# AppleHolic/pytorch_sound

Hardware: AMD Instinct MI355X
Metric: audio-sec/s STFT+mel+fwd/bwd (higher is better)
Workload: dtype bf16; 1 GPU; configs[1]: Conv1d separator (4 x ResBlock1, C=256, on 513-bin magnitude), 22.05 kHz, STFT 1024/256, 80 mel, batch 32 x 2 s per GPU, Adam, bf16 autocast; global_batch=32, parallelism=dp1, model_params=5520386

## Files before the change

### include/psnd.h

```cpp
#ifndef PSND_H
#define PSND_H

#include <stdint.h>
#include <stddef.h>

#ifdef __cplusplus
extern "C" {
#endif

#define PSND_OK 0
#define PSND_E_ARG (-1)
#define PSND_E_SHAPE (-2)
#define PSND_E_HIP (-3)
#define PSND_E_UNSUPPORTED (-4)

#define PSND_FRAMING_CENTER 0
#define PSND_FRAMING_HIFIGAN 1
#define PSND_FRAMING_NONE 2

int psnd_version(void);
const char *psnd_last_error(void);
#ifdef PSND_LAB
void psnd_env_refresh(void);
#endif

void *psnd_event_create(void);
int psnd_event_destroy(void *ev);
int psnd_event_record_external(void *ev, void *stream);
int psnd_stream_wait_event(void *stream, void *ev);
int psnd_event_external_supported(void);

int64_t psnd_frame_count(int64_t T, int n_fft, int hop, int framing);
int64_t psnd_frame_sample_index(int64_t f, int m, int64_t T, int n_fft, int hop, int framing);

size_t psnd_stft_plan_bytes(int n_fft);
int psnd_stft_plan_build(int n_fft, const float *window_host, void *plan_host);

int psnd_stft_fwd(const float *wav, int64_t N, int64_t T, int n_fft, int hop, int framing,
                  const void *plan, float mag_eps,
                  float *mag, float *phase, float *re, float *im, void *stream);

int psnd_stft_mag_nfk(const float *wav, int64_t N, int64_t T, int n_fft, int hop, int framing,
                      const void *plan, float mag_eps, float *mag_nfk, void *stream);

int psnd_stft_bwd(const float *wav, int64_t N, int64_t T, int n_fft, int hop, int framing,
                  const void *plan, float mag_eps,
                  const float *gmag, const float *gre, const float *gim,
                  float *gwav, void *stream);

int psnd_polar_bwd(const float *gmag, const float *gphase, const float *mag, const float *phase, int64_t n,
                   float *gre, float *gim, void *stream);

int psnd_istft(const float *mag, const float *phase, int64_t N, int64_t F, int n_fft, int hop,
               const void *plan, float eps, float *out, void *stream);

size_t psnd_stft_mr_plan_bytes(int n_fft);
int psnd_stft_mr_plan_build(int n_fft, const float *window_host, void *plan_host);
int psnd_stft_mr_fwd(const float *wav, int64_t N, int64_t T, int n_fft, int hop, int framing, const void *plan, size_t plan_bytes,
                     float mag_eps, float *mag, float *phase, float *re, float *im, void *stream);
size_t psnd_stft_mr_bwd_scratch_bytes(int64_t N, int64_t T, int n_fft, int hop, int framing);
int psnd_stft_mr_bwd(const float *wav, int64_t N, int64_t T, int n_fft, int hop, int framing, const void *plan, size_t plan_bytes,
                     float mag_eps, const float *gmag, const float *gre, const float *gim, void *scratch, size_t scratch_bytes,
                     float *gwav, void *stream);
size_t psnd_istft_mr_scratch_bytes(int64_t N, int64_t F, int n_fft);
int psnd_istft_mr(const float *mag, const float *phase, int64_t N, int64_t F, int n_fft, int hop, const void *plan, size_t plan_bytes,
                  float eps, void *scratch, size_t scratch_bytes, float *out, void *stream);

#define PSND_LOG_NONE 0
#define PSND_LOG_E 1
#define PSND_LOG_10 2
size_t psnd_mel_plan_bytes(int M, int K);
int psnd_mel_plan_build(int M, int K, const float *mel_filter_host, void *plan_host);
int psnd_mel_fwd(const float *mag, int64_t N, int64_t F, int M, int K, const void *mel_plan,
                 int log_kind, float log_offset, float pre_clamp_min, float clamp_lo, float clamp_hi,
                 float *out, float *mel_lin, void *stream);
int psnd_mel_bwd(const float *gout, const float *mel_lin, int64_t N, int64_t F, int M, int K,
                 const void *mel_plan, int log_kind, float log_offset, float pre_clamp_min,
                 float clamp_lo, float clamp_hi, float *gmag, void *stream);

int psnd_logmel_fwd(const float *wav, int64_t N, int64_t T, int n_fft, int hop, int framing, const void *stft_plan,
                    float mag_eps, int M, const void *mel_plan, int log_kind, float log_offset, float pre_clamp_min,
                    float clamp_lo, float clamp_hi, float *out, void *stream);

int psnd_conv1d_cl(const void *A, const void *A2, const void *AM, float a2_slope, const void *W, const float *bias,
                   const void *res, const void *mask_src, int64_t N, int Lp, int L, int HP, int Ca, int Cb, int k,
                   int off0, int dstep, float act_slope, float mask_slope, void *out_raw, void *out_act,
                   void *a_eff_out, void *stream);
int psnd_conv1d_cl_wgrad_splits(int64_t N, int Lp, int Ca, int Cb, int k);
int psnd_conv1d_cl_pair_supported(int C, int k, int off1, int dstep1, int off2, int dstep2);
int psnd_conv1d_cl_pair(const void *A, const void *W1, const float *bias1, const void *M1, float m1_slope, float act1_slope,
                        void *mid_out, const void *W2, const float *bias2, const void *M2, float m2_slope, const void *res,
                        int64_t N, int Lp, int L, int HP, int C, int k, int off1, int dstep1, int off2, int dstep2,
                        float act2_slope, void *out_raw, void *out_act, void *stream);
typedef struct psnd_wgrad_desc {
    const void *g, *xa;
    float *gw_part, *gbias_part;
    int off0, dstep;
    int Ca, Cb, k, splits;
} psnd_wgrad_desc;
int psnd_conv1d_cl_wgrad_multi_splits(int64_t N, int Lp, int Ca, int Cb, int k, int n_convs);
int psnd_conv1d_cl_wgrad_multi(const psnd_wgrad_desc *d, int n, int64_t N, int Lp, void *stream);
typedef struct psnd_chain_pair {
    const void *W1;
    const float *bias1;
    float act1_slope;
    void *mid_out;
    const void *W2;
    const float *bias2;
    int off1, dstep1, off2, dstep2;
    float act2_slope;
    void *out_raw, *out_act;
    const void *M1, *M2;
    float m1_slope, m2_slope;
} psnd_chain_pair;
int psnd_conv1d_cl_chain_rows(int C, int k, int n_pairs, const int *taps);
int psnd_conv1d_cl_chain_plan(int C, int k, int n_pairs, const int *taps, int64_t R, int *mr_out);
int psnd_conv1d_cl_chain(const void *A, const void *res, const psnd_chain_pair *pairs, int n_pairs, int64_t N, int Lp, int L, int HP,
                         int C, int k, void *stream);
void psnd_conv_chain_stats(long long *out2);
int psnd_to_cl_nfk(const float *x_nfk, int64_t N, int K, int64_t F, int Lp, int HP, int Cp, int preop, void *out, void *stream);
int64_t psnd_mask_head_l1_blocks_nfk(int64_t N, int64_t F, int K);
int psnd_mask_head_l1_fwd_nfk(const void *y, const float *mag_nfk, const float *ref_nfk, int64_t N, int K, int64_t F, int Lp, int HP, int Cp,
                              float *est_nfk, double *part, void *stream);
int psnd_mask_head_l1_bwd_nfk(const float *gest_nfk, const float *mag_nfk, const void *y, const float *est_nfk, const float *ref_nfk,
                              const float *g, float coef, int64_t N, int K, int64_t F, int Lp, int HP, int Cp, void *gy, void *stream);
int psnd_mel_fwd_nfk(const float *mag_nfk, int64_t N, int64_t F, int M, int K, const void *mel_plan, int log_kind, float log_offset,
                     float pre_clamp_min, float clamp_lo, float clamp_hi, float *out, float *mel_lin, void *stream);
int psnd_mel_bwd_nfk(const float *gout, const float *mel_lin, int64_t N, int64_t F, int M, int K, const void *mel_plan, int log_kind,
                     float log_offset, float pre_clamp_min, float clamp_lo, float clamp_hi, float *gmag_nfk, void *stream);
int psnd_mel_l1_fwd_nfk(const float *mag_nfk, int64_t N, int64_t F, int M, int K, const void *mel_plan, int log_kind, float log_offset,
                        float pre_clamp_min, float clamp_lo, float clamp_hi, const float *ref, float *mel_lin, double *part, void *stream);
int psnd_mel_l1_bwd_nfk(const float *ref, const float *mel_lin, const float *g, float coef, int64_t N, int64_t F, int M, int K,
                        const void *mel_plan, int log_kind, float log_offset, float pre_clamp_min, float clamp_lo, float clamp_hi,
                        float *gmag_nfk, void *stream);
int64_t psnd_mask_head_l1_blocks(int64_t N, int64_t T, int Cp);
int psnd_mask_head_l1_fwd(const void *y, const float *mag, const float *ref, int64_t N, int C, int64_t T, int Lp, int HP, int Cp,
                          float *est, double *part, void *stream);
int psnd_mask_head_l1_bwd(const float *gest, const float *mag, const void *y, const float *est, const float *ref, const float *g,
                          float coef, int64_t N, int C, int64_t T, int Lp, int HP, int Cp, void *gy, void *stream);
int64_t psnd_mel_l1_blocks(int64_t N, int64_t F, int M);
int psnd_mel_l1_fwd(const float *mag, int64_t N, int64_t F, int M, int K, const void *mel_plan, int log_kind, float log_offset,
                    float pre_clamp_min, float clamp_lo, float clamp_hi, const float *ref, float *mel_lin, double *part, void *stream);
int psnd_mel_l1_bwd(const float *ref, const float *mel_lin, const float *g, float coef, int64_t N, int64_t F, int M, int K,
                    const void *mel_plan, int log_kind, float log_offset, float pre_clamp_min, float clamp_lo, float clamp_hi,
                    float *gmag, void *stream);
int psnd_nan_flag(const float *x, int64_t n, float *flag, void *stream);
int psnd_l1_loss_combine(const double *const *parts, const int64_t *nb, const double *scale, int terms, float *out, float *nan_flag, void *stream);
int psnd_conv_stats(int64_t *out4, int reset);
int psnd_conv_pair_stats(int64_t *out4, int reset);
int psnd_conv1d_cl_wgrad(const void *G1, const void *G2, const void *GM, float g2_slope, const void *xa, int64_t N,
                         int Lp, int Ca, int Cb, int k, int off0, int dstep, float *gw_part, float *gbias_part,
                         void *g_out, void *stream);
int psnd_conv1d_prep(const float *v, const float *g, const float *bias, int Cout, int Cin, int k, int Cb, int Ca,
                     void *wf, void *wb, float *bias_padded, void *stream);
int psnd_convtr1d_prep(const float *v, const float *g, const float *bias, int Cin, int Cout, int K, int stride, int Cr, int Cip,
                       void *wf, void *wb, float *bias_rep, void *stream);
int psnd_convtr1d_prep_multi(const void *descs_dev, int n, int total_blocks, void *stream);
int psnd_convtr1d_cl_fwd(const void *xa, const void *wf, const float *bias_rep, int64_t N, int Lp, int L, int HP, int Cip, int Cr,
                         int stride, int padding, int LpO, int HPO, float act_slope, void *out_raw, void *out_act, void *stream);
int psnd_convtr1d_cl_wgrad_splits(int64_t N, int Lp, int Cip, int Cr, int stride);
int psnd_convtr1d_cl_bwd(const void *g_raw, const void *g_act, const void *act, float act_slope, const void *wb, const void *xa,
                         int64_t N, int Lp, int L, int HP, int Cip, int Cr, int stride, int padding, int LpO, int HPO, void *gx,
                         void *g_eff, float *gw_part, void *stream);
int psnd_convtr1d_wnorm_bwd(const float *gw_part, int splits, const float *v, const float *g, int Cin, int Cout, int K, int stride,
                            int Cr, int Cip, float *gv, float *gg, void *stream);
int psnd_cl_mean_act_fwd(const void *a, const void *b, const void *c, const void *d, int count, float slope, void *out, int64_t n,
                         void *stream);
int psnd_cl_mean_act_bwd(const void *g, const void *y, int count, float slope, void *gin, int64_t n, void *stream);
int psnd_cl_sum2(const void *const *a, int na, void *out_a, const void *const *b, int nb, void *out_b, int64_t n, void *stream);
int psnd_cl_colsum_splits(int64_t rows, int C);
int psnd_cl_colsum(const void *g, int64_t rows, int C, int Lp, int lo, int hi, float *part, float *out, void *stream);
int psnd_conv1d_prep_multi(const void *descs_dev, int n, int total_blocks, int max_row, int which, void *stream);
#define PSND_WNORM_MAX 32
typedef struct psnd_wnorm_desc {
    const float *gw_part, *gbias_part;
    const float *v, *g;
    float *gv, *gg, *gbias;
    int splits, Cout, Cin, k, Cb, Ca;
} psnd_wnorm_desc;
int psnd_conv1d_wnorm_bwd_multi(const psnd_wnorm_desc *descs, int n, void *stream);
int psnd_conv1d_cl_bwd(const void *G1, const void *G2, const void *GM, float g2_slope, const void *wb, const void *xa,
                       int64_t N, int Lp, int L, int HP, int Ca, int Cb, int k, int pad, int dil, void *gx, void *g_out,
                       const void *gx_mask, float gx_mask_slope, const void *gx_res, float *gw_part, float *gbias_part,
                       void *stream);
int psnd_conv1d_cl_pair_bwd_supported(int C, int k, int pad2, int dil2, int pad1, int dil1);
int psnd_conv1d_cl_pair_bwd_splits(int64_t N, int Lp, int C, int k);
int psnd_conv1d_cl_pair_bwd(const void *G, const void *wb2, const void *M1, float m1_slope, void *g_mid, const void *wb1, const void *M2,
                            float m2_slope, const void *res, int64_t N, int Lp, int L, int HP, int C, int k, int pad2, int dil2,
                            int pad1, int dil1, void *gx, const void *xa_a, float *gw_a, float *gb_a, const void *G_b,
                            const void *xa_b, int off_b, int dstep_b, float *gw_b, float *gb_b, void *stream);
int psnd_conv1d_wnorm_bwd(const float *gw_part, const float *gbias_part, int splits, const float *v, const float *g,
                          int Cout, int Cin, int k, int Cb, int Ca, float *gv, float *gg, float *gbias, void *stream);
int psnd_to_cl(const float *x, int64_t N, int C, int64_t T, int Lp, int HP, int Cp, int preop, void *out, void *stream);
int psnd_from_cl_tanh(const void *x, int64_t N, int C, int64_t T, int Lp, int HP, int Cp, float *out, void *stream);
int psnd_to_cl_tanh_bwd(const float *g, const float *out_fwd, int64_t N, int C, int64_t T, int Lp, int HP, int Cp, void *gx, void *stream);
int psnd_from_cl(const void *x, int64_t N, int C, int64_t T, int Lp, int HP, int Cp, float *out, void *stream);
int psnd_mask_head_fwd(const void *y, const float *mag, int64_t N, int C, int64_t T, int Lp, int HP, int Cp, float *est,
                       void *stream);
int psnd_mask_head_bwd(const float *gest, const float *mag, const void *y, int64_t N, int C, int64_t T, int Lp, int HP, int Cp,
                       void *gy, void *stream);

int psnd_linear1x1_fwd(const float *x, const float *w, const float *bias, int64_t N, int Cin, int Cout, int64_t T, int relu, int bf16,
                       float *y, void *stream);
int64_t psnd_linear1x1_wgrad_slabs(int64_t N, int Cin, int Cout, int64_t T);
int psnd_linear1x1_bwd(const float *gy, const float *ymask, const float *x, const float *w, int64_t N, int Cin, int Cout, int64_t T,
                       int bf16, float *gx, float *gw, float *gw_part, float *gbias, void *stream);
int psnd_linear1x1_bwd_acc(const float *gy, const float *ymask, const float *x, const float *w, int64_t N, int Cin, int Cout, int64_t T,
                           int bf16, const float *gx_addend, float *gx, float *gw, float *gw_part, float *gbias, void *stream);
int psnd_linear1x1_bwd_ex(const void *gy, const float *ymask, const void *x, const float *w, int64_t N, int Cin, int Cout, int64_t T, int bf16,
                          int io_h, int64_t ld_h, const float *gx_addend, const void *gx_mask, void *gx, float *gw, float *gw_part, float *gbias,
                          void *stream);
int psnd_linear1x1_fwd_ex(const void *x, const float *w, const float *bias, int64_t N, int Cin, int Cout, int64_t T, int relu, int bf16, int io_h,
                          int64_t ld_h, void *y, void *stream);
int psnd_mha_fwd(const float *kvq, const unsigned char *mask, int64_t N, int H, int C, int64_t T, float *out, float *att, float *stats,
                 int bf16, void *stream);
int psnd_mha_bwd(const float *kvq, const unsigned char *mask, const float *out, const float *att, const float *stats, const float *gout,
                 const float *gatt, int64_t N, int H, int C, int64_t T, float *delta, float *gkvq, int bf16, void *stream);
int psnd_mha_bwd_parts(const float *kvq, const unsigned char *mask, const float *out, const float *att, const float *stats, const float *gout,
                       const float *gatt, int64_t N, int H, int C, int64_t T, float *delta, float *gkvq, int bf16, int parts, void *stream);

#define PSND_GN_WS_DOUBLES(C) (2 * (size_t)(C))
int psnd_posenc(const float *x, const float *pe, float scale, int64_t N, int C, int64_t T, int64_t pe_len, float *y, void *stream);
int psnd_groupnorm1_fwd(const float *x, const float *res, const float *gamma, const float *beta, int64_t N, int C,
                        int64_t T, float eps, int relu, float *y, float *stats, double *ws, void *stream);
int psnd_groupnorm1_bwd(const float *gy, const float *x, const float *res, const float *gamma, const float *y,
                        const float *stats, int64_t N, int C, int64_t T, int relu, float *gx, float *ggamma,
                        float *gbeta, double *ws, void *stream);
int psnd_groupnorm1_drop_fwd(const float *x, const float *res, const float *gamma, const float *beta, int64_t N, int C,
                             int64_t T, float eps, int relu, float *y, float *stats, double *ws, const uint64_t *key,
                             uint32_t thr, float scale, void *stream);
int psnd_groupnorm1_drop_bwd(const float *gy, const float *x, const float *res, const float *gamma, const float *y,
                             const float *stats, int64_t N, int C, int64_t T, int relu, float *gx, float *gres, float *ggamma,
                             float *gbeta, double *ws, const uint64_t *key, uint32_t thr, float scale, void *stream);
int psnd_rng_seed(uint64_t *state, uint64_t seed, uint64_t call, void *stream);
int psnd_rng_next(uint64_t *state, uint64_t *key_out, void *stream);
int psnd_softmax_keys_fwd(float *scores, const uint8_t *mask, int64_t B, int64_t T, float scale, void *stream);
int psnd_softmax_keys_bwd(const float *att, const float *gatt, int64_t B, int64_t T, float scale, float *gscores,
                          void *stream);

int psnd_preemphasis_fwd(const float *x, int64_t N, int64_t T, float coef, float *y, void *stream);
int psnd_preemphasis_bwd(const float *gy, int64_t N, int64_t T, float coef, float *gx, void *stream);
int64_t psnd_stft_loss_blocks(int64_t KF);
int psnd_stft_loss_partial(const float *p_mag, const float *t_mag, int64_t N, int64_t KF, float eps, double *part,
                           void *stream);
int psnd_stft_loss_final(const double *const *parts, const int64_t *KF, int L, int64_t N, float *norms, float *out3,
                         void *stream);
int psnd_stft_loss_bwd(const float *p_mag, const float *t_mag, int64_t N, int64_t KF, float eps, const float *norms,
                       const float *g3, int L, float *gp, float *gt, void *stream);
int64_t psnd_stft_fwd_msl_blocks(int64_t T, int n_fft, int hop);
int psnd_stft_fwd_msl(const float *wav, int64_t N, int64_t T, int n_fft, int hop, const void *plan, float mag_eps,
                      const float *t_mag, float eps, double *part, void *stream);
int psnd_stft_loss_final_blocks(const double *const *parts, const int64_t *KF, const int64_t *blocks, int L, int64_t N,
                                float *norms, float *out3, void *stream);
int psnd_stft_bwd_msl_supported(int n_fft, int hop);
int psnd_stft_bwd_msl(const float *wav, int64_t N, int64_t T, int n_fft, int hop, int framing, const void *plan,
                      float mag_eps, const float *t_mag, const float *norms, const float *g3, int L, float eps,
                      int accumulate, float *gwav, void *stream);

#define PSND_IPREEMPH_SPAN 8192
#define PSND_IPREEMPH_WARM_MAX 2048
#define PSND_IPREEMPH_SEQ (-1)
#define PSND_IPREEMPH_AUTO (-2)
int psnd_ipreemph_fwd(const float *x, int64_t N, int64_t T, const float *w_ih, const float *w_hh, int warm, float *y,
                      void *stream);
int psnd_ipreemph_bwd(const float *gy, const float *y, const float *x, int64_t N, int64_t T, const float *w_ih,
                      const float *w_hh, int warm, float *gx, double *partial, float *gw, void *stream);
int psnd_volnorm_fwd(const float *wav, int64_t B, int64_t L, int window, int hop, float inv_gain, float *out,
                     int64_t out_len, float *std, void *stream);
int psnd_volnorm_reverse(const float *wav, int64_t B, int64_t L, int window, int hop, float gain, const float *std,
                         float *out, int64_t out_len, void *stream);

int psnd_im2col_f32(const float *x, int64_t N, int C, int64_t T, int k, int dil, int pad, int stride, int up, int64_t To, float slope,
                    float *col, void *stream);
int psnd_col2im_f32(const float *gcol, const float *x, int64_t N, int C, int64_t T, int k, int dil, int pad, int stride, int up, int64_t To,
                    float slope, float *gx, void *stream);

int psnd_pad_collate(const float *flat, const int64_t *offs, const int64_t *lens, int64_t N, int64_t Tmax, float *out,
                     float *mask, void *stream);

int64_t psnd_frame_mask_frames(int64_t T, int win, int hop);
int psnd_frame_mask(const float *mask, int64_t N, int64_t T, int win, int hop, float *out, void *stream);

int psnd_grad_pack_bf16(const float *src, void *dst, int64_t n, float scale, void *stream);
int psnd_grad_unpack_bf16(const void *src, float *dst, int64_t n, float scale, void *stream);
int64_t psnd_adam_chunk(void);
int64_t psnd_adam_table_bytes(void);
int psnd_adam_step(const void *table, int n_tensors, const int *chunk_tensor, const int64_t *chunk_off, int64_t n_chunks,
                   double lr, double beta1, double beta2, double eps, double weight_decay, int decoupled,
                   const float *found_inf, const float *grad_scale, float *corr, float clip_value, const float *clip_coef,
                   void *stream);
int psnd_adam_step_logged(const void *table, int n_tensors, const int *chunk_tensor, const int64_t *chunk_off, int64_t n_chunks,
                          double lr, double beta1, double beta2, double eps, double weight_decay, int decoupled,
                          const float *found_inf, const float *grad_scale, float *corr, float clip_value, const float *clip_coef,
                          int *flag_log, int log_slot, int log_seq, void *stream);
int psnd_grad_sumsq(const void *table, int n_tensors, const int *chunk_tensor, const int64_t *chunk_off, int64_t n_chunks,
                    float clip_value, const float *grad_scale, int accumulate, float max_norm, double *partial, double *sumsq,
                    float *coef, void *stream);

int psnd_pqmf_analysis(const float *x, const float *filt, int64_t B, int64_t T, int subbands, int taps, int flip, float scale,
                       float *out, void *stream);
int psnd_pqmf_synthesis(const float *x, const float *filt, int64_t B, int64_t M, int64_t T_out, int subbands, int taps, int flip,
                        float scale, float *y, void *stream);

int psnd_lstft_analysis(const float *x, const float *basis, const float *window, int64_t N, int64_t Lx, int C, int n, int hop, float *spec,
                        float *mag, float *phase, void *stream);
int psnd_lstft_mag_bwd(const float *spec, const float *mag, const float *gmag, int64_t N, int C, int64_t F, float *gspec, void *stream);
int psnd_lstft_synthesis(const float *g, const float *basis, const float *window, const float *mult, int64_t N, int C, int64_t F, int n,
                         int hop, int64_t Ly, float *y, void *stream);
int64_t psnd_lstft_wgrad_slabs(int64_t N, int C, int n, int64_t F);
int psnd_lstft_basis_grad(const float *g, const float *x, const float *window, int64_t N, int64_t Lx, int C, int n, int hop, int64_t F,
                          float *gb_part, float *gb, void *stream);

int64_t psnd_l1_loss_blocks(int64_t n);
int64_t psnd_masked_l1_blocks(int64_t n);
int psnd_masked_l1_fwd(const float *a, const float *b, const float *frame_weight, int64_t N, int C, int64_t T, double *part, float *out,
                       float *inv_den, void *stream);
int psnd_masked_l1_bwd(const float *a, const float *b, const float *frame_weight, int64_t N, int C, int64_t T, const float *g,
                       const float *inv_den, float *ga, float *gb, void *stream);
int psnd_l1_loss_fwd(const float *a, const float *b, int64_t n, double *part, float *out, void *stream);
int psnd_l1_loss_bwd(const float *a, const float *b, int64_t n, const float *g, float *ga, float *gb, void *stream);
int psnd_l1_loss_sum_fwd(const float *const *a, const float *const *b, const int64_t *n, const double *w, int terms, double *part,
                         float *out, void *stream);
int psnd_l1_loss_bwd_w(const float *a, const float *b, int64_t n, const float *g, double weight, float *ga, float *gb, void *stream);

#ifdef __cplusplus
// ... 4 lines not shown
```

### pytorch_sound_amd/_lib.py

```python
import ctypes
import os
import numpy as np

_HERE = os.path.dirname(os.path.abspath(__file__))
LIB_PATH = os.environ.get('PSND_LIB', os.path.join(_HERE, 'libpsnd_hip.so'))

PSND_OK = 0
FRAMING_CENTER = 0
FRAMING_HIFIGAN = 1
FRAMING_NONE = 2
LOG_NONE, LOG_E, LOG_10 = 0, 1, 2

_c = ctypes
_P = _c.c_void_p
_I64 = _c.c_int64
_INT = _c.c_int
_F = _c.c_float
_D = _c.c_double
_U32 = _c.c_uint32
_U64 = _c.c_uint64

SIGNATURES = {
    'psnd_version': (_INT, []),
    'psnd_last_error': (_c.c_char_p, []),
    'psnd_event_create': (_P, []),
    'psnd_event_destroy': (_INT, [_P]),
    'psnd_event_record_external': (_INT, [_P, _P]),
    'psnd_stream_wait_event': (_INT, [_P, _P]),
    'psnd_event_external_supported': (_INT, []),
    'psnd_frame_count': (_I64, [_I64, _INT, _INT, _INT]),
    'psnd_frame_sample_index': (_I64, [_I64, _INT, _I64, _INT, _INT, _INT]),
    'psnd_stft_plan_bytes': (_c.c_size_t, [_INT]),
    'psnd_stft_plan_build': (_INT, [_INT, _P, _P]),
    'psnd_stft_fwd': (_INT, [_P, _I64, _I64, _INT, _INT, _INT, _P, _F, _P, _P, _P, _P, _P]),
    'psnd_stft_mag_nfk': (_INT, [_P, _I64, _I64, _INT, _INT, _INT, _P, _F, _P, _P]),
    'psnd_stft_bwd': (_INT, [_P, _I64, _I64, _INT, _INT, _INT, _P, _F, _P, _P, _P, _P, _P]),
    'psnd_istft': (_INT, [_P, _P, _I64, _I64, _INT, _INT, _P, _F, _P, _P]),
    'psnd_stft_mr_plan_bytes': (_c.c_size_t, [_INT]),
    'psnd_stft_mr_plan_build': (_INT, [_INT, _P, _P]),
    'psnd_stft_mr_fwd': (_INT, [_P, _I64, _I64, _INT, _INT, _INT, _P, _c.c_size_t, _F, _P, _P, _P, _P, _P]),
    'psnd_stft_mr_bwd_scratch_bytes': (_c.c_size_t, [_I64, _I64, _INT, _INT, _INT]),
    'psnd_stft_mr_bwd': (_INT, [_P, _I64, _I64, _INT, _INT, _INT, _P, _c.c_size_t, _F, _P, _P, _P, _P, _c.c_size_t, _P, _P]),
    'psnd_istft_mr_scratch_bytes': (_c.c_size_t, [_I64, _I64, _INT]),
    'psnd_istft_mr': (_INT, [_P, _P, _I64, _I64, _INT, _INT, _P, _c.c_size_t, _F, _P, _c.c_size_t, _P, _P]),
    'psnd_mel_plan_bytes': (_c.c_size_t, [_INT, _INT]),
    'psnd_mel_plan_build': (_INT, [_INT, _INT, _P, _P]),
    'psnd_mel_fwd': (_INT, [_P, _I64, _I64, _INT, _INT, _P, _INT, _F, _F, _F, _F, _P, _P, _P]),
    'psnd_mel_bwd': (_INT, [_P, _P, _I64, _I64, _INT, _INT, _P, _INT, _F, _F, _F, _F, _P, _P]),
    'psnd_logmel_fwd': (_INT, [_P, _I64, _I64, _INT, _INT, _INT, _P, _F, _INT, _P, _INT, _F, _F, _F, _F, _P, _P]),
    'psnd_conv1d_cl': (_INT, [_P, _P, _P, _F, _P, _P, _P, _P, _I64, _INT, _INT, _INT, _INT, _INT, _INT, _INT, _INT, _F, _F, _P, _P, _P, _P]),
    'psnd_conv1d_cl_pair_supported': (_INT, [_INT, _INT, _INT, _INT, _INT, _INT]),
    'psnd_conv1d_cl_pair': (_INT, [_P, _P, _P, _P, _F, _F, _P, _P, _P, _P, _F, _P, _I64, _INT, _INT, _INT, _INT, _INT, _INT, _INT, _INT, _INT, _F, _P, _P, _P]),
    'psnd_conv1d_cl_wgrad': (_INT, [_P, _P, _P, _F, _P, _I64, _INT, _INT, _INT, _INT, _INT, _INT, _P, _P, _P, _P]),
    'psnd_conv1d_prep': (_INT, [_P, _P, _P, _INT, _INT, _INT, _INT, _INT, _P, _P, _P, _P]),
    'psnd_conv1d_wnorm_bwd': (_INT, [_P, _P, _INT, _P, _P, _INT, _INT, _INT, _INT, _INT, _P, _P, _P, _P]),
    'psnd_conv1d_cl_bwd': (_INT, [_P, _P, _P, _F, _P, _P, _I64, _INT, _INT, _INT, _INT, _INT, _INT, _INT, _INT, _P, _P, _P, _F, _P, _P, _P, _P]),
    'psnd_conv1d_cl_wgrad_multi_splits': (_INT, [_I64, _INT, _INT, _INT, _INT, _INT]),
    'psnd_conv1d_cl_wgrad_multi': (_INT, [_P, _INT, _I64, _INT, _P]),
    'psnd_nan_flag': (_INT, [_P, _I64, _P, _P]),
    'psnd_conv1d_cl_chain_rows': (_INT, [_INT, _INT, _INT, _P]),
    'psnd_conv1d_cl_chain_plan': (_INT, [_INT, _INT, _INT, _P, _I64, _P]),
    'psnd_conv1d_cl_chain': (_INT, [_P, _P, _P, _INT, _I64, _INT, _INT, _INT, _INT, _INT, _P]),
    'psnd_conv_chain_stats': (None, [_P]),
    'psnd_conv1d_cl_pair_bwd_supported': (_INT, [_INT, _INT, _INT, _INT, _INT, _INT]),
    'psnd_conv1d_cl_pair_bwd_splits': (_INT, [_I64, _INT, _INT, _INT]),
    'psnd_conv1d_cl_pair_bwd': (_INT, [_P, _P, _P, _F, _P, _P, _P, _F, _P, _I64, _INT, _INT, _INT, _INT, _INT, _INT, _INT, _INT, _INT, _P, _P, _P, _P,
                                       _P, _P, _INT, _INT, _P, _P, _P]),
    'psnd_conv1d_wnorm_bwd_multi': (_INT, [_P, _INT, _P]),
    'psnd_conv1d_prep_multi': (_INT, [_P, _INT, _INT, _INT, _INT, _P]),
    'psnd_conv1d_cl_wgrad_splits': (_INT, [_I64, _INT, _INT, _INT, _INT]),
    'psnd_mask_head_l1_blocks': (_I64, [_I64, _I64, _INT]),
    'psnd_masked_l1_blocks': (_I64, [_I64]),
    'psnd_masked_l1_fwd': (_INT, [_P, _P, _P, _I64, _INT, _I64, _P, _P, _P, _P]),
    'psnd_masked_l1_bwd': (_INT, [_P, _P, _P, _I64, _INT, _I64, _P, _P, _P, _P, _P]),
    'psnd_to_cl_nfk': (_INT, [_P, _I64, _INT, _I64, _INT, _INT, _INT, _INT, _P, _P]),
    'psnd_mask_head_l1_blocks_nfk': (_I64, [_I64, _I64, _INT]),
    'psnd_mask_head_l1_fwd_nfk': (_INT, [_P, _P, _P, _I64, _INT, _I64, _INT, _INT, _INT, _P, _P, _P]),
    'psnd_mask_head_l1_bwd_nfk': (_INT, [_P, _P, _P, _P, _P, _P, _F, _I64, _INT, _I64, _INT, _INT, _INT, _P, _P]),
    'psnd_mel_fwd_nfk': (_INT, [_P, _I64, _I64, _INT, _INT, _P, _INT, _F, _F, _F, _F, _P, _P, _P]),
    'psnd_mel_bwd_nfk': (_INT, [_P, _P, _I64, _I64, _INT, _INT, _P, _INT, _F, _F, _F, _F, _P, _P]),
    'psnd_mel_l1_fwd_nfk': (_INT, [_P, _I64, _I64, _INT, _INT, _P, _INT, _F, _F, _F, _F, _P, _P, _P, _P]),
    'psnd_mel_l1_bwd_nfk': (_INT, [_P, _P, _P, _F, _I64, _I64, _INT, _INT, _P, _INT, _F, _F, _F, _F, _P, _P]),
    'psnd_mask_head_l1_fwd': (_INT, [_P, _P, _P, _I64, _INT, _I64, _INT, _INT, _INT, _P, _P, _P]),
    'psnd_mask_head_l1_bwd': (_INT, [_P, _P, _P, _P, _P, _P, _F, _I64, _INT, _I64, _INT, _INT, _INT, _P, _P]),
    'psnd_mel_l1_blocks': (_I64, [_I64, _I64, _INT]),
    'psnd_mel_l1_fwd': (_INT, [_P, _I64, _I64, _INT, _INT, _P, _INT, _F, _F, _F, _F, _P, _P, _P, _P]),
    'psnd_mel_l1_bwd': (_INT, [_P, _P, _P, _F, _I64, _I64, _INT, _INT, _P, _INT, _F, _F, _F, _F, _P, _P]),
    'psnd_l1_loss_combine': (_INT, [_P, _P, _P, _INT, _P, _P, _P]),
    'psnd_conv_stats': (_INT, [_P, _INT]),
    'psnd_conv_pair_stats': (_INT, [_P, _INT]),
    'psnd_convtr1d_prep_multi': (_INT, [_P, _INT, _INT, _P]),
    'psnd_convtr1d_prep': (_INT, [_P, _P, _P, _INT, _INT, _INT, _INT, _INT, _INT, _P, _P, _P, _P]),
    'psnd_convtr1d_cl_fwd': (_INT, [_P, _P, _P, _I64, _INT, _INT, _INT, _INT, _INT, _INT, _INT, _INT, _INT, _F, _P, _P, _P]),
    'psnd_convtr1d_cl_wgrad_splits': (_INT, [_I64, _INT, _INT, _INT, _INT]),
    'psnd_convtr1d_cl_bwd': (_INT, [_P, _P, _P, _F, _P, _P, _I64, _INT, _INT, _INT, _INT, _INT, _INT, _INT, _INT, _INT, _P, _P, _P, _P]),
    'psnd_convtr1d_wnorm_bwd': (_INT, [_P, _INT, _P, _P, _INT, _INT, _INT, _INT, _INT, _INT, _P, _P, _P]),
    'psnd_cl_mean_act_fwd': (_INT, [_P, _P, _P, _P, _INT, _F, _P, _I64, _P]),
    'psnd_cl_mean_act_bwd': (_INT, [_P, _P, _INT, _F, _P, _I64, _P]),
    'psnd_cl_sum2': (_INT, [_P, _INT, _P, _P, _INT, _P, _I64, _P]),
    'psnd_grad_pack_bf16': (_INT, [_P, _P, _I64, _F, _P]),
    'psnd_grad_unpack_bf16': (_INT, [_P, _P, _I64, _F, _P]),
    'psnd_cl_colsum_splits': (_INT, [_I64, _INT]),
    'psnd_cl_colsum': (_INT, [_P, _I64, _INT, _INT, _INT, _INT, _P, _P, _P]),
    'psnd_posenc': (_INT, [_P, _P, _F, _I64, _INT, _I64, _I64, _P, _P]),
    'psnd_groupnorm1_fwd': (_INT, [_P, _P, _P, _P, _I64, _INT, _I64, _F, _INT, _P, _P, _P, _P]),
    'psnd_groupnorm1_bwd': (_INT, [_P, _P, _P, _P, _P, _P, _I64, _INT, _I64, _INT, _P, _P, _P, _P, _P]),
    'psnd_groupnorm1_drop_fwd': (_INT, [_P, _P, _P, _P, _I64, _INT, _I64, _F, _INT, _P, _P, _P, _P, _U32, _F, _P]),
    'psnd_groupnorm1_drop_bwd': (_INT, [_P, _P, _P, _P, _P, _P, _I64, _INT, _I64, _INT, _P, _P, _P, _P, _P, _P, _U32, _F, _P]),
    'psnd_rng_seed': (_INT, [_P, _U64, _U64, _P]),
    'psnd_rng_next': (_INT, [_P, _P, _P]),
    'psnd_linear1x1_fwd': (_INT, [_P, _P, _P, _I64, _INT, _INT, _I64, _INT, _INT, _P, _P]),
    'psnd_linear1x1_wgrad_slabs': (_I64, [_I64, _INT, _INT, _I64]),
    'psnd_linear1x1_bwd': (_INT, [_P, _P, _P, _P, _I64, _INT, _INT, _I64, _INT, _P, _P, _P, _P, _P]),
    'psnd_linear1x1_bwd_acc': (_INT, [_P, _P, _P, _P, _I64, _INT, _INT, _I64, _INT, _P, _P, _P, _P, _P, _P]),
    'psnd_linear1x1_bwd_ex': (_INT, [_P, _P, _P, _P, _I64, _INT, _INT, _I64, _INT, _INT, _I64, _P, _P, _P, _P, _P, _P, _P]),
    'psnd_linear1x1_fwd_ex': (_INT, [_P, _P, _P, _I64, _INT, _INT, _I64, _INT, _INT, _INT, _I64, _P, _P]),
    'psnd_mha_fwd': (_INT, [_P, _P, _I64, _INT, _INT, _I64, _P, _P, _P, _INT, _P]),
    'psnd_mha_bwd': (_INT, [_P, _P, _P, _P, _P, _P, _P, _I64, _INT, _INT, _I64, _P, _P, _INT, _P]),
    'psnd_mha_bwd_parts': (_INT, [_P, _P, _P, _P, _P, _P, _P, _I64, _INT, _INT, _I64, _P, _P, _INT, _INT, _P]),
    'psnd_softmax_keys_fwd': (_INT, [_P, _P, _I64, _I64, _F, _P]),
    'psnd_softmax_keys_bwd': (_INT, [_P, _P, _I64, _I64, _F, _P, _P]),
    'psnd_polar_bwd': (_INT, [_P, _P, _P, _P, _I64, _P, _P, _P]),
    'psnd_preemphasis_fwd': (_INT, [_P, _I64, _I64, _F, _P, _P]),
    'psnd_preemphasis_bwd': (_INT, [_P, _I64, _I64, _F, _P, _P]),
    'psnd_ipreemph_fwd': (_INT, [_P, _I64, _I64, _P, _P, _INT, _P, _P]),
    'psnd_ipreemph_bwd': (_INT, [_P, _P, _P, _I64, _I64, _P, _P, _INT, _P, _P, _P, _P]),
    'psnd_volnorm_fwd': (_INT, [_P, _I64, _I64, _INT, _INT, _F, _P, _I64, _P, _P]),
    'psnd_volnorm_reverse': (_INT, [_P, _I64, _I64, _INT, _INT, _F, _P, _P, _I64, _P]),
    'psnd_stft_loss_blocks': (_I64, [_I64]),
    'psnd_stft_loss_partial': (_INT, [_P, _P, _I64, _I64, _F, _P, _P]),
    'psnd_stft_loss_final': (_INT, [_P, _P, _INT, _I64, _P, _P, _P]),
    'psnd_stft_loss_bwd': (_INT, [_P, _P, _I64, _I64, _F, _P, _P, _INT, _P, _P, _P]),
    'psnd_stft_bwd_msl_supported': (_INT, [_INT, _INT]),
    'psnd_stft_fwd_msl_blocks': (_I64, [_I64, _INT, _INT]),
    'psnd_stft_fwd_msl': (_INT, [_P, _I64, _I64, _INT, _INT, _P, _F, _P, _F, _P, _P]),
    'psnd_stft_loss_final_blocks': (_INT, [_P, _P, _P, _INT, _I64, _P, _P, _P]),
    'psnd_stft_bwd_msl': (_INT, [_P, _I64, _I64, _INT, _INT, _INT, _P, _F, _P, _P, _P, _INT, _F, _INT, _P, _P]),
    'psnd_frame_mask_frames': (_I64, [_I64, _INT, _INT]),
    'psnd_frame_mask': (_INT, [_P, _I64, _I64, _INT, _INT, _P, _P]),
    'psnd_pad_collate': (_INT, [_P, _P, _P, _I64, _I64, _P, _P, _P]),
    'psnd_im2col_f32': (_INT, [_P, _I64, _INT, _I64, _INT, _INT, _INT, _INT, _INT, _I64, _F, _P, _P]),
    'psnd_col2im_f32': (_INT, [_P, _P, _I64, _INT, _I64, _INT, _INT, _INT, _INT, _INT, _I64, _F, _P, _P]),
    'psnd_adam_chunk': (_I64, []),
    'psnd_adam_table_bytes': (_I64, []),
    'psnd_adam_step': (_INT, [_P, _INT, _P, _P, _I64, _D, _D, _D, _D, _D, _INT, _P, _P, _P, _F, _P, _P]),
    'psnd_adam_step_logged': (_INT, [_P, _INT, _P, _P, _I64, _D, _D, _D, _D, _D, _INT, _P, _P, _P, _F, _P, _P, _INT, _INT, _P]),
    'psnd_grad_sumsq': (_INT, [_P, _INT, _P, _P, _I64, _F, _P, _INT, _F, _P, _P, _P, _P]),
    'psnd_mask_head_fwd': (_INT, [_P, _P, _I64, _INT, _I64, _INT, _INT, _INT, _P, _P]),
    'psnd_mask_head_bwd': (_INT, [_P, _P, _P, _I64, _INT, _I64, _INT, _INT, _INT, _P, _P]),
    'psnd_pqmf_analysis': (_INT, [_P, _P, _I64, _I64, _INT, _INT, _INT, _F, _P, _P]),
    'psnd_pqmf_synthesis': (_INT, [_P, _P, _I64, _I64, _I64, _INT, _INT, _INT, _F, _P, _P]),
    'psnd_lstft_analysis': (_INT, [_P, _P, _P, _I64, _I64, _INT, _INT, _INT, _P, _P, _P, _P]),
    'psnd_lstft_mag_bwd': (_INT, [_P, _P, _P, _I64, _INT, _I64, _P, _P]),
    'psnd_lstft_synthesis': (_INT, [_P, _P, _P, _P, _I64, _INT, _I64, _INT, _INT, _I64, _P, _P]),
    'psnd_lstft_wgrad_slabs': (_I64, [_I64, _INT, _INT, _I64]),
    'psnd_lstft_basis_grad': (_INT, [_P, _P, _P, _I64, _I64, _INT, _INT, _INT, _I64, _P, _P, _P]),
    'psnd_l1_loss_blocks': (_I64, [_I64]),
    'psnd_l1_loss_fwd': (_INT, [_P, _P, _I64, _P, _P, _P]),
    'psnd_l1_loss_bwd': (_INT, [_P, _P, _I64, _P, _P, _P, _P]),
    'psnd_l1_loss_sum_fwd': (_INT, [_P, _P, _P, _P, _INT, _P, _P, _P]),
    'psnd_l1_loss_bwd_w': (_INT, [_P, _P, _I64, _P, _D, _P, _P, _P]),
    'psnd_to_cl': (_INT, [_P, _I64, _INT, _I64, _INT, _INT, _INT, _INT, _P, _P]),
    'psnd_from_cl': (_INT, [_P, _I64, _INT, _I64, _INT, _INT, _INT, _P, _P]),
    'psnd_from_cl_tanh': (_INT, [_P, _I64, _INT, _I64, _INT, _INT, _INT, _P, _P]),
    'psnd_to_cl_tanh_bwd': (_INT, [_P, _P, _I64, _INT, _I64, _INT, _INT, _INT, _P, _P]),
}

_lib = None


class PsndError(RuntimeError):
    pass


class WgradDesc(ctypes.Structure):
    _fields_ = [('g', _P), ('xa', _P), ('gw_part', _P), ('gbias_part', _P), ('off0', _INT), ('dstep', _INT),
                ('Ca', _INT), ('Cb', _INT), ('k', _INT), ('splits', _INT)]


class ChainPair(ctypes.Structure):
    _fields_ = [('W1', _P), ('bias1', _P), ('act1_slope', _F), ('mid_out', _P), ('W2', _P), ('bias2', _P),
                ('off1', _INT), ('dstep1', _INT), ('off2', _INT), ('dstep2', _INT), ('act2_slope', _F), ('out_raw', _P), ('out_act', _P),
                ('M1', _P), ('M2', _P), ('m1_slope', _F), ('m2_slope', _F)]


def lib():
    global _lib
    if _lib is None:
        import torch
        if not os.path.exists(LIB_PATH):
            raise PsndError('libpsnd_hip.so not found at %s - run `python -m pytorch_sound_amd._build` '
                            '(there is no CPU / eager fallback)' % LIB_PATH)
        _lib = _load(LIB_PATH)
    return _lib


def _load(path):
    h = ctypes.CDLL(path)
    for name, (res, args) in SIGNATURES.items():
        fn = getattr(h, name)
        fn.restype = res
        fn.argtypes = args
    for name, (res, args) in LAB_SIGNATURES.items():
        fn = getattr(h, name, None)
        if fn is not None:
            fn.restype = res
            fn.argtypes = args
    return h


LAB_LIB_PATH = os.path.join(_HERE, 'libpsnd_hip_lab.so')
LAB_SIGNATURES = {'psnd_env_refresh': (None, [])}


def is_lab() -> bool:
    return hasattr(lib(), 'psnd_env_refresh')


def refresh_switches():
    if _lib is not None and hasattr(_lib, 'psnd_env_refresh'):
        _lib.psnd_env_refresh()

# ... 84 lines not shown
```

### pytorch_sound_amd/cl.py

```python
import ctypes
import os
from pytorch_sound_amd import _switches as _sw
import weakref

import torch

from . import _lib
from ._lib import lib, check, ptr, stream_ptr

ALIGN_C = 32


def round_up(x, m):
    return (x + m - 1) // m * m


class CLShape:

    def __init__(self, N, L, HP):
        self.N, self.L, self.HP = int(N), int(L), int(HP)
        self.Lp = round_up(self.L + 2 * self.HP, 8)

    @property
    def R(self):
# ... 33 lines not shown
        return gx, None, None


def from_cl_raw(buf, C, T, shape):
    _need(buf, torch.bfloat16)
    N, Lp, Cp = buf.shape
    out = torch.empty((N, C, T), dtype=torch.float32, device=buf.device)
    with torch.cuda.device(buf.device):
        check(lib().psnd_from_cl(ptr(buf), N, C, T, Lp, shape.HP, Cp, ptr(out), stream_ptr(buf.device)), 'psnd_from_cl')
    return out


class FromCL(torch.autograd.Function):
    @staticmethod
    def forward(ctx, buf, C, T, shape):
        ctx.shape, ctx.Cp = shape, buf.shape[2]
        return from_cl_raw(buf.contiguous(), C, T, shape)

    @staticmethod
    def backward(ctx, g):
        g = g.contiguous()
        N, C, T = g.shape
        out = torch.empty((N, ctx.shape.Lp, ctx.Cp), dtype=torch.bfloat16, device=g.device)
        with torch.cuda.device(g.device):
            check(lib().psnd_to_cl(ptr(g), N, C, T, ctx.shape.Lp, ctx.shape.HP, ctx.Cp, 0, ptr(out), stream_ptr(g.device)),
                  'psnd_to_cl')
        return out, None, None, None


class FromCLTanh(torch.autograd.Function):

    @staticmethod
    def forward(ctx, buf, C, T, shape):
        buf = buf.contiguous()
        _need(buf, torch.bfloat16)
        N, Lp, Cp = buf.shape
        out = torch.empty((N, C, T), dtype=torch.float32, device=buf.device)
        with torch.cuda.device(buf.device):
            check(lib().psnd_from_cl_tanh(ptr(buf), N, C, T, Lp, shape.HP, Cp, ptr(out), stream_ptr(buf.device)), 'psnd_from_cl_tanh')
        ctx.shape, ctx.Cp = shape, Cp
        ctx.save_for_backward(out)
        return out

    @staticmethod
    def backward(ctx, g):
        (out,) = ctx.saved_tensors
        g = g.contiguous().float()
        N, C, T = g.shape
        gx = torch.empty((N, ctx.shape.Lp, ctx.Cp), dtype=torch.bfloat16, device=g.device)
        with torch.cuda.device(g.device):
            check(lib().psnd_to_cl_tanh_bwd(ptr(g), ptr(out), N, C, T, ctx.shape.Lp, ctx.shape.HP, ctx.Cp, ptr(gx), stream_ptr(g.device)),
                  'psnd_to_cl_tanh_bwd')
        return gx, None, None, None


class MaskHeadCL(torch.autograd.Function):

    @staticmethod
    def forward(ctx, y, mag, shape):
        _need(y, torch.bfloat16)
        _need(mag, torch.float32)
        y, mag = y.contiguous(), mag.contiguous()
        N, C, T = mag.shape
        est = torch.empty_like(mag)
        with torch.cuda.device(y.device):
            check(lib().psnd_mask_head_fwd(ptr(y), ptr(mag), N, C, T, shape.Lp, shape.HP, y.shape[2], ptr(est), stream_ptr(y.device)),
                  'psnd_mask_head_fwd')
        ctx.shape = shape
        ctx.save_for_backward(y, mag)
        return est

    @staticmethod
    def backward(ctx, g):
        y, mag = ctx.saved_tensors
        g = g.contiguous().float()
        N, C, T = mag.shape
        gy = torch.empty_like(y)
        with torch.cuda.device(y.device):
            check(lib().psnd_mask_head_bwd(ptr(g), ptr(mag), ptr(y), N, C, T, ctx.shape.Lp, ctx.shape.HP, y.shape[2], ptr(gy),
                                           stream_ptr(y.device)), 'psnd_mask_head_bwd')
        return gy, None, None


LAST_LOSS_NAN_FLAG = [None]
NAN_FLAG_DEST = [None]


def _nan_flag_tensor(dev):
    dest = NAN_FLAG_DEST[0]
    if dest is not None and dest.device == dev and dest.dtype == torch.float32 and dest.numel() == 1:
        return dest.view(())
    return torch.empty((), dtype=torch.float32, device=dev)


class MaskHeadSpectralL1CL(torch.autograd.Function):

    @staticmethod
    def forward(ctx, y, mag, mag_ref, mel_ref, mel_plan, shape, M, log_kind, log_offset, pre_clamp_min, clamp_lo, clamp_hi, w1, w2):
        import ctypes
        from .kernels import _clamp_args
        ctx.set_materialize_grads(False)
        _need(y, torch.bfloat16)
        for t in (mag, mag_ref, mel_ref):
            _need(t, torch.float32)
        N, C, T = mag.shape
        if mag_ref.shape != mag.shape or tuple(mel_ref.shape) != (N, M, T):
            raise _lib.PsndError('mask_head_spectral_l1: mag_ref %s / mel_ref %s do not match mag %s and %d mel bands'
                                 % (tuple(mag_ref.shape), tuple(mel_ref.shape), tuple(mag.shape), M))
        dev = y.device
        lo, hi, pre = _clamp_args(clamp_lo, clamp_hi, pre_clamp_min)
        est = torch.empty_like(mag)
        lin = torch.empty((N, M, T), dtype=torch.float32, device=dev)
        nb1 = int(lib().psnd_mask_head_l1_blocks(N, T, y.shape[2]))
        nb2 = int(lib().psnd_mel_l1_blocks(N, T, M))
        part = torch.empty(nb1 + nb2, dtype=torch.float64, device=dev)
        out = torch.empty((), dtype=torch.float32, device=dev)
        st = stream_ptr(dev)
        with torch.cuda.device(dev):
            check(lib().psnd_mask_head_l1_fwd(ptr(y), ptr(mag), ptr(mag_ref), N, C, T, shape.Lp, shape.HP, y.shape[2], ptr(est),
                                              ptr(part), st), 'psnd_mask_head_l1_fwd')
            p2 = ctypes.c_void_p(part.data_ptr() + 8 * nb1)
            check(lib().psnd_mel_l1_fwd(ptr(est), N, T, M, C, ptr(mel_plan), log_kind, float(log_offset), pre, lo, hi, ptr(mel_ref),
                                        ptr(lin), p2, st), 'psnd_mel_l1_fwd')
            parts = (ctypes.c_void_p * 2)(part.data_ptr(), part.data_ptr() + 8 * nb1)
            nbs = (ctypes.c_int64 * 2)(nb1, nb2)
            sc = (ctypes.c_double * 2)(float(w1) / mag.numel(), float(w2) / mel_ref.numel())
            nan_flag = _nan_flag_tensor(dev)
            check(lib().psnd_l1_loss_combine(parts, nbs, sc, 2, ptr(out), ptr(nan_flag), st), 'psnd_l1_loss_combine')
        LAST_LOSS_NAN_FLAG[0] = nan_flag
        ctx.cfg = (shape, M, log_kind, float(log_offset), pre, lo, hi, float(w1) / mag.numel(), float(w2) / mel_ref.numel())
        ctx.save_for_backward(y, mag, mag_ref, mel_ref, mel_plan, est, lin)
        ctx.mark_non_differentiable(est)
        return out, est

    @staticmethod
    def backward(ctx, g, _gest):
        y, mag, mag_ref, mel_ref, mel_plan, est, lin = ctx.saved_tensors
        shape, M, log_kind, log_offset, pre, lo, hi, c1, c2 = ctx.cfg
        N, C, T = mag.shape
        if g is None:
            return (None,) * 14
        g = g.contiguous().float()
        gest = torch.empty_like(mag)
        gy = torch.empty_like(y)
        st = stream_ptr(y.device)
        with torch.cuda.device(y.device):
            check(lib().psnd_mel_l1_bwd(ptr(mel_ref), ptr(lin), ptr(g), c2, N, T, M, C, ptr(mel_plan), log_kind, log_offset, pre, lo, hi,
                                        ptr(gest), st), 'psnd_mel_l1_bwd')
            check(lib().psnd_mask_head_l1_bwd(ptr(gest), ptr(mag), ptr(y), ptr(est), ptr(mag_ref), ptr(g), c1, N, C, T, shape.Lp, shape.HP,
                                              y.shape[2], ptr(gy), st), 'psnd_mask_head_l1_bwd')
        return (gy,) + (None,) * 13


def to_cl_nfk(x_nfk, shape, preop=0):
    _need(x_nfk, torch.float32)
    if x_nfk.requires_grad and torch.is_grad_enabled():
        raise _lib.PsndError('to_cl_nfk carries no gradient (feature tensors are inputs); use ToCL on an (N, K, F) tensor')
    N, F, K = x_nfk.shape
    if F != shape.L or N != shape.N:
        raise _lib.PsndError('to_cl_nfk: tensor %s does not match the CL geometry (N=%d, L=%d)' % (tuple(x_nfk.shape), shape.N, shape.L))
    Cp = round_up(K, ALIGN_C)
    out = torch.empty((N, shape.Lp, Cp), dtype=torch.bfloat16, device=x_nfk.device)
    with torch.cuda.device(x_nfk.device):
        check(lib().psnd_to_cl_nfk(ptr(x_nfk), N, K, F, shape.Lp, shape.HP, Cp, int(preop), ptr(out), stream_ptr(x_nfk.device)),
              'psnd_to_cl_nfk')
    return out


class MaskHeadSpectralL1NFK(torch.autograd.Function):

    @staticmethod
    def forward(ctx, y, mag, mag_ref, mel_ref, mel_plan, shape, M, log_kind, log_offset, pre_clamp_min, clamp_lo, clamp_hi, w1, w2):
        from .kernels import _clamp_args
        ctx.set_materialize_grads(False)
        _need(y, torch.bfloat16)
        for t in (mag, mag_ref, mel_ref):
            _need(t, torch.float32)
        N, F, K = mag.shape
        if mag_ref.shape != mag.shape or tuple(mel_ref.shape) != (N, M, F):
            raise _lib.PsndError('mask_head_spectral_l1 (nfk): mag_ref %s / mel_ref %s do not match mag %s and %d mel bands'
                                 % (tuple(mag_ref.shape), tuple(mel_ref.shape), tuple(mag.shape), M))
        dev = y.device
        lo, hi, pre = _clamp_args(clamp_lo, clamp_hi, pre_clamp_min)
        est = torch.empty_like(mag)
        lin = torch.empty((N, M, F), dtype=torch.float32, device=dev)
        nb1 = int(lib().psnd_mask_head_l1_blocks_nfk(N, F, K))
        nb2 = int(lib().psnd_mel_l1_blocks(N, F, M))
        part = torch.empty(nb1 + nb2, dtype=torch.float64, device=dev)
        out = torch.empty((), dtype=torch.float32, device=dev)
        st = stream_ptr(dev)
        with torch.cuda.device(dev):
            check(lib().psnd_mask_head_l1_fwd_nfk(ptr(y), ptr(mag), ptr(mag_ref), N, K, F, shape.Lp, shape.HP, y.shape[2], ptr(est),
                                                  ptr(part), st), 'psnd_mask_head_l1_fwd_nfk')
            p2 = ctypes.c_void_p(part.data_ptr() + 8 * nb1)
            check(lib().psnd_mel_l1_fwd_nfk(ptr(est), N, F, M, K, ptr(mel_plan), log_kind, float(log_offset), pre, lo, hi, ptr(mel_ref),
                                            ptr(lin), p2, st), 'psnd_mel_l1_fwd_nfk')
            parts = (ctypes.c_void_p * 2)(part.data_ptr(), part.data_ptr() + 8 * nb1)
            nbs = (ctypes.c_int64 * 2)(nb1, nb2)
            sc = (ctypes.c_double * 2)(float(w1) / mag.numel(), float(w2) / mel_ref.numel())
            nan_flag = _nan_flag_tensor(dev)
            check(lib().psnd_l1_loss_combine(parts, nbs, sc, 2, ptr(out), ptr(nan_flag), st), 'psnd_l1_loss_combine')
        LAST_LOSS_NAN_FLAG[0] = nan_flag
        ctx.cfg = (shape, M, log_kind, float(log_offset), pre, lo, hi, float(w1) / mag.numel(), float(w2) / mel_ref.numel())
        ctx.save_for_backward(y, mag, mag_ref, mel_ref, mel_plan, est, lin)
        ctx.mark_non_differentiable(est)
        return out, est

    @staticmethod
    def backward(ctx, g, _gest):
        y, mag, mag_ref, mel_ref, mel_plan, est, lin = ctx.saved_tensors
        shape, M, log_kind, log_offset, pre, lo, hi, c1, c2 = ctx.cfg
        N, F, K = mag.shape
        if g is None:
            return (None,) * 14
        g = g.contiguous().float()
        gest = torch.empty_like(mag)
        gy = torch.empty_like(y)
        st = stream_ptr(y.device)
        with torch.cuda.device(y.device):
            check(lib().psnd_mel_l1_bwd_nfk(ptr(mel_ref), ptr(lin), ptr(g), c2, N, F, M, K, ptr(mel_plan), log_kind, log_offset, pre, lo, hi,
                                            ptr(gest), st), 'psnd_mel_l1_bwd_nfk')
            check(lib().psnd_mask_head_l1_bwd_nfk(ptr(gest), ptr(mag), ptr(y), ptr(est), ptr(mag_ref), ptr(g), c1, N, K, F, shape.Lp,
                                                  shape.HP, y.shape[2], ptr(gy), st), 'psnd_mask_head_l1_bwd_nfk')
        return (gy,) + (None,) * 13


def _launch_conv(A, A2, AM, a2_slope, W, bias, res, mask_src, shape, Ca, Cb, k, off0, dstep, act_slope, mask_slope,
                 want_raw, want_act, a_eff_out=None):
    dev = W.device
    raw = torch.empty((shape.N, shape.Lp, Cb), dtype=torch.bfloat16, device=dev) if want_raw else None
    act = torch.empty((shape.N, shape.Lp, Cb), dtype=torch.bfloat16, device=dev) if want_act else None
    with torch.cuda.device(dev):
        check(lib().psnd_conv1d_cl(ptr(A), ptr(A2), ptr(AM), float(a2_slope), ptr(W), ptr(bias), ptr(res), ptr(mask_src),
                                   shape.N, shape.Lp, shape.L, shape.HP, Ca, Cb, k, off0, dstep, float(act_slope),
                                   float(mask_slope), ptr(raw), ptr(act), ptr(a_eff_out), stream_ptr(dev)), 'psnd_conv1d_cl')
    return raw, act


_JOIN_PENDING = {}


def _join_side_at_end_of_backward(dev, side):
    target = torch.cuda.current_stream(dev)
    pending = _JOIN_PENDING.setdefault(dev.index, [])
    if not any(t == target and sd == side for t, sd in pending):
        pending.append((target, side))

    def join():
        for t, sd in _JOIN_PENDING.pop(dev.index, []):
            t.wait_stream(sd)

    torch.autograd.Variable._execution_engine.queue_callback(join)

_SECTION_STREAMS = {}
AUTO_SECTIONS = True
NODE_GRANULARITY = 'body'

GRAD_SINK = None

_PARAM_NOTES = {}
_PARAM_MULTI_TASK = {}
_PARAM_FORCED_MULTI = set()


def _graph_task_id():
    return torch._C._current_graph_task_id()


def _drop_notes(cid, pids):
    for pid in pids:
        live = _PARAM_NOTES.get(pid)
        if live is not None:
            live.discard(cid)
            if not live:
                del _PARAM_NOTES[pid]


def note_param_use(ctx, *params):
    if not any(ctx.needs_input_grad):
        return
    pids = tuple(id(p) for p in params if p is not None)
    if not pids:
        return
    cid = id(ctx)
    in_backward = _graph_task_id() != -1
    for pid in pids:
        _PARAM_NOTES.setdefault(pid, set()).add(cid)
        if in_backward:
            _PARAM_FORCED_MULTI.add(pid)
    ctx._psnd_noted = pids
    weakref.finalize(ctx, _drop_notes, cid, pids)


def single_use(p) -> bool:
    if p is None:
        return True
    pid = id(p)
    if pid in _PARAM_FORCED_MULTI:
        return False
    task = _graph_task_id()
    if task != -1 and _PARAM_MULTI_TASK.get(pid) == task:
        return False
    n = len(_PARAM_NOTES.get(pid, ()))
    if n > 1 and task != -1:
        _PARAM_MULTI_TASK[pid] = task
    return n == 1


def consume_param_use(ctx):
    pids = getattr(ctx, '_psnd_noted', None)
    if pids:
        task = _graph_task_id()
        for pid in pids:
            if len(_PARAM_NOTES.get(pid, ())) > 1 and task != -1:
                _PARAM_MULTI_TASK[pid] = task
        _drop_notes(id(ctx), pids)


def reset_param_uses():
    _PARAM_NOTES.clear()
    _PARAM_MULTI_TASK.clear()
    _PARAM_FORCED_MULTI.clear()


HANDOVER_CHUNKS = 3


def _sections(dev, N, rows):
    import os
    e = _sw.lab('PSND_CL_SECTIONS', 'auto')
    n = 1 if e == 'auto' else int(e)
    if n <= 1 or N % n != 0 or N // n < 1 or (e == 'auto' and not AUTO_SECTIONS):
        return 1, []
    pool = _SECTION_STREAMS.setdefault(dev.index, [])
    while len(pool) < n - 1:
        pool.append(torch.cuda.Stream(device=dev))
    return n, pool[:n - 1]


def _run_sections(dev, nsec, sides, fn):
    if nsec == 1:
        fn(0)
        return
    main = torch.cuda.current_stream(dev)
    for sd in sides:
        sd.wait_stream(main)
    fn(0)
    for h, sd in enumerate(sides, 1):
        with torch.cuda.stream(sd):
            fn(h)
    for sd in sides:
        main.wait_stream(sd)


BRANCH_PARAM_GRADS = _sw.lab('PSND_BRANCH_PARAM_GRADS', '1') == '1'
_BRANCH_STREAMS = {}
_PARAM_STREAM = {}


def param_stream(dev):
    s = _PARAM_STREAM.get(dev.index)
    if s is None:
        s = _PARAM_STREAM[dev.index] = torch.cuda.Stream(device=dev)
    return s



def branch_streams(dev, n):
    pool = _BRANCH_STREAMS.setdefault(dev.index, [])
    while len(pool) < n:
        pool.append(torch.cuda.Stream(device=dev))
    return pool[:n]


_WGRAD_STREAMS = {}

# ... 208 lines not shown
            if GRAD_SINK is not None:
                GRAD_SINK.note_producer(ctx.params, side)
        main = torch.cuda.current_stream(dev)

        def param_side(st):
            check(lib().psnd_convtr1d_cl_bwd(ptr(g_raw), ptr(g_act), ptr(act if g_act is not None else None), slope, ptr(wb), ptr(xa),
                                             shape.N, shape.Lp, shape.L, shape.HP, Cip, Cr, stride, padding, out_shape.Lp, out_shape.HP,
                                             None, ptr(g_eff), ptr(gw), st), 'psnd_convtr1d_cl_bwd')
            check(lib().psnd_convtr1d_wnorm_bwd(ptr(gw), S, ptr(v32), ptr(g32), Cin, Cout, K, stride, Cr, Cip, ptr(gv), ptr(gg), st),
                  'psnd_convtr1d_wnorm_bwd')
            if ctx.has_bias:
                gsrc = (g_eff if g_eff is not None else g_raw).view(-1, Cr)
                if Cr > 256:
                    return torch.sum(gsrc, 0, dtype=torch.float32)[:Cout]
                rows = gsrc.shape[0]
                part = torch.empty(lib().psnd_cl_colsum_splits(rows, Cr) * Cr, dtype=torch.float32, device=dev)
                gb_full = torch.empty(Cr, dtype=torch.float32, device=dev)
                win = (out_shape.Lp, out_shape.HP, out_shape.HP + out_shape.L) if (g_eff is not None and clip_rows) else (0, 0, 0)
                check(lib().psnd_cl_colsum(ptr(gsrc), rows, Cr, win[0], win[1], win[2], ptr(part), ptr(gb_full), st), 'psnd_cl_colsum')
                return gb_full[:Cout]
            return None

        with torch.cuda.device(dev):
            check(lib().psnd_convtr1d_cl_bwd(ptr(g_raw), ptr(g_act), ptr(act if g_act is not None else None), slope, ptr(wb), ptr(xa),
                                             shape.N, shape.Lp, shape.L, shape.HP, Cip, Cr, stride, padding, out_shape.Lp, out_shape.HP,
                                             ptr(gx), ptr(g_eff), None, stream_ptr(dev)), 'psnd_convtr1d_cl_bwd')
            if side is None:
                g_bias = param_side(stream_ptr(dev))
            else:
                side.wait_stream(main)
                with torch.cuda.stream(side):
                    gw = torch.empty_like(gw)
                    gv, gg = torch.empty_like(gv), torch.empty_like(gg)
                    g_bias = param_side(stream_ptr(dev))
                for t in (g_raw, g_act, g_eff, act, xa, v32, g32, wb):
                    if t is not None:
                        t.record_stream(side)
                _join_side_at_end_of_backward(dev, side)
        consume_param_use(ctx)
        return gx, gv, gg, g_bias, None, None, None, None, None, None


def prep_all_convtr(owner, ups):
    import struct
    key = tuple((u.weight_v.data_ptr(), u.weight_g.data_ptr(), 0 if u.bias is None else u.bias.data_ptr(), tuple(u.weight_v.shape), u.stride)
                for u in ups)
    cache = getattr(owner, '_cl_prep_convtr_cache', None)
    if cache is None or cache['key'] != key:
        dev = ups[0].weight_v.device
        packs, recs, blk0 = {}, [], 0
        for u in ups:
            Cin, Cout, K = u.weight_v.shape
            Cip, Cr = round_up(Cin, ALIGN_C), round_up(Cout, ALIGN_C)
            wf = torch.zeros(2 * u.stride * Cr * Cip, dtype=torch.bfloat16, device=dev)
            wb = torch.zeros(2 * u.stride * Cr * Cip, dtype=torch.bfloat16, device=dev)
            bp = torch.zeros(u.stride * Cr, dtype=torch.float32, device=dev)
            packs[id(u)] = (wf, wb, bp)
            recs.append(struct.pack('<6Q8i', u.weight_v.data_ptr(), u.weight_g.data_ptr(), 0 if u.bias is None else u.bias.data_ptr(),
                                    wf.data_ptr(), wb.data_ptr(), bp.data_ptr(), Cin, Cout, K, u.stride, Cr, Cip, blk0, 0))
            blk0 += Cin
        table = torch.frombuffer(bytearray(b''.join(recs)), dtype=torch.uint8).to(dev)
        cache = {'key': key, 'packs': packs, 'table': table, 'n': len(ups), 'blocks': blk0, 'dev': dev}
        owner._cl_prep_convtr_cache = cache
    for u in ups:
        if not (u.weight_v.is_contiguous() and u.weight_g.is_contiguous() and u.weight_v.dtype == torch.float32):
            raise _lib.PsndError('prep_all_convtr: fp32 contiguous weight_v / weight_g expected')
    with torch.cuda.device(cache['dev']):
        check(lib().psnd_convtr1d_prep_multi(ptr(cache['table']), cache['n'], cache['blocks'], stream_ptr(cache['dev'])),
              'psnd_convtr1d_prep_multi')
    return cache['packs']


class FanOutCL(torch.autograd.Function):

    @staticmethod
    def forward(ctx, x_raw, x_act, count):
        ctx.set_materialize_grads(False)
        ctx.count = count
        ctx.meta = (x_raw.shape, x_raw.device)
        outs = []
        for _ in range(count):
            outs += [x_raw.detach(), x_act.detach()]
        return tuple(outs)

    @staticmethod
    def backward(ctx, *gs):
        g_raw = [g.contiguous() for g in gs[0::2] if g is not None]
        g_act = [g.contiguous() for g in gs[1::2] if g is not None]
        shape, dev = ctx.meta

        def single(lst):
            return lst[0] if len(lst) == 1 else None

        if len(g_raw) <= 1 and len(g_act) <= 1:
            return single(g_raw), single(g_act), None
        out_r = single(g_raw) if len(g_raw) <= 1 else torch.empty(shape, dtype=torch.bfloat16, device=dev)
        out_a = single(g_act) if len(g_act) <= 1 else torch.empty(shape, dtype=torch.bfloat16, device=dev)
        for g in g_raw + g_act:
            _need(g, torch.bfloat16)
        ra = g_raw if len(g_raw) > 1 else []
        aa = g_act if len(g_act) > 1 else []
        pa = (ctypes.c_void_p * max(1, len(ra)))(*[g.data_ptr() for g in ra])
        pb = (ctypes.c_void_p * max(1, len(aa)))(*[g.data_ptr() for g in aa])
        n = (ra or aa)[0].numel()
        with torch.cuda.device(dev):
            check(lib().psnd_cl_sum2(pa, len(ra), ptr(out_r) if ra else None, pb, len(aa), ptr(out_a) if aa else None, n, stream_ptr(dev)),
                  'psnd_cl_sum2')
        return out_r, out_a, None


class MeanActCL(torch.autograd.Function):

    @staticmethod
    def forward(ctx, slope, *rs):
        n = len(rs)
        if not 1 <= n <= 4:
            raise _lib.PsndError('MeanActCL: 1..4 branches, got %d' % n)
        rs = [r.contiguous() for r in rs]
        for r in rs:
            _need(r, torch.bfloat16)
        out = torch.empty_like(rs[0])
        ps = [ptr(r) for r in rs] + [None] * (4 - n)
        with torch.cuda.device(out.device):
            check(lib().psnd_cl_mean_act_fwd(ps[0], ps[1], ps[2], ps[3], n, float(slope), ptr(out), out.numel(), stream_ptr(out.device)),
                  'psnd_cl_mean_act_fwd')
        ctx.n, ctx.slope = n, float(slope)
        ctx.save_for_backward(out)
        return out

    @staticmethod
    def backward(ctx, g):
        (out,) = ctx.saved_tensors
        g = g.contiguous()
        gin = torch.empty_like(out)
        with torch.cuda.device(out.device):
            check(lib().psnd_cl_mean_act_bwd(ptr(g), ptr(out), ctx.n, ctx.slope, ptr(gin), out.numel(), stream_ptr(out.device)),
                  'psnd_cl_mean_act_bwd')
        return (None,) + (gin,) * ctx.n


class PrepPacks(dict):
    deferred = None

    def write_backward_packs(self):
        cache = self.deferred
        if cache is None or cache['wb_done']:
            return
        cache['wb_done'] = True
        with torch.cuda.device(cache['dev']):
            check(lib().psnd_conv1d_prep_multi(ptr(cache['table']), cache['n'], cache['blocks'], cache['max_row'], 2, stream_ptr(cache['dev'])),
                  'psnd_conv1d_prep_multi')


def prep_all(owner, convs, defer_backward_packs=False):
    import struct
    import os
    if _sw.lab('PSND_NO_PREP_ALL') == '1':
        return None
    if any(c.weight_v.shape[1] * c.weight_v.shape[2] > 10240 for c in convs):
        return None
    key = tuple((c.weight_v.data_ptr(), c.weight_g.data_ptr(), 0 if c.bias is None else c.bias.data_ptr(),
                 tuple(c.weight_v.shape)) for c in convs)
    cache = getattr(owner, '_cl_prep_cache', None)
    if cache is None or cache['key'] != key:
        dev = convs[0].weight_v.device
        packs, recs, blk0, max_row = PrepPacks(), [], 0, 0
        for c in convs:
            Cout, Cin, k = c.weight_v.shape
            Ca, Cb = round_up(Cin, ALIGN_C), round_up(Cout, ALIGN_C)
            wf = torch.zeros((k, Cb, Ca), dtype=torch.bfloat16, device=dev)
            wb = torch.zeros((k, Ca, Cb), dtype=torch.bfloat16, device=dev)
            bp = torch.zeros(Cb, dtype=torch.float32, device=dev)
            packs[id(c)] = (wf, wb, bp)
            recs.append(struct.pack('<6Q6i', c.weight_v.data_ptr(), c.weight_g.data_ptr(),
                                    0 if c.bias is None else c.bias.data_ptr(), wf.data_ptr(), wb.data_ptr(), bp.data_ptr(),
                                    Cout, Cin, k, Cb, Ca, blk0))
            blk0 += (Cout + 7) // 8
            max_row = max(max_row, Cin * k)
        table = torch.frombuffer(bytearray(b''.join(recs)), dtype=torch.uint8).to(dev)
        cache = {'key': key, 'packs': packs, 'table': table, 'n': len(convs), 'blocks': blk0, 'max_row': max_row, 'dev': dev,
                 'wb_done': True}
        owner._cl_prep_cache = cache
    for c in convs:
        if not (c.weight_v.is_contiguous() and c.weight_g.is_contiguous() and c.weight_v.dtype == torch.float32):
            raise _lib.PsndError('prep_all: fp32 contiguous weight_v / weight_g expected')
    defer = bool(defer_backward_packs) and torch.is_grad_enabled() and _sw.lab('PSND_PREP_NO_DEFER') != '1'
    with torch.cuda.device(cache['dev']):
        check(lib().psnd_conv1d_prep_multi(ptr(cache['table']), cache['n'], cache['blocks'], cache['max_row'], 1 if defer else 3,
                                           stream_ptr(cache['dev'])), 'psnd_conv1d_prep_multi')
    cache['wb_done'] = not defer
    cache['packs'].deferred = cache if defer else None
    return cache['packs']


def fused_conv(xa, conv, shape, res=None, want_raw=False, want_act=True, act_slope=0.1, prep=None):
    return FusedConvCL.apply(xa, conv.weight_v, conv.weight_g, conv.bias, res, shape, conv.dilation, want_raw, want_act,
                             act_slope, None if prep is None else prep[id(conv)])


class ResBlockCL(torch.autograd.Function):

    @staticmethod
    def forward(ctx, x, xa, shape, roles, dils, last_act_slope, want_raw, packs, *params):
        ctx.set_materialize_grads(False)
        _need(xa, torch.bfloat16)
        dev = xa.device
        n = len(dils)
        ctx.pack_owner = getattr(packs, 'owner', None)
        steps, saved, plan = [], [], []
        cur_x, cur_xa, pending = x, xa, None
        for i in range(n):
            wv, wg, b = params[3 * i:3 * i + 3]
            Cout, Cin, k = wv.shape
            role = roles[i]
            src = pending if role == 'c2' else cur_xa
            Ca, Cb = src.shape[2], round_up(Cout, ALIGN_C)
            if Ca != round_up(Cin, ALIGN_C) or (role in ('c2', 'r2') and Cb != cur_x.shape[2]):
                raise _lib.PsndError('CL conv chain: %s conv %d -> %d channels on a %d-channel buffer' % (role, Cin, Cout, Ca))
            dil = dils[i]
            pad = (k * dil - dil) // 2
            v32, g32 = wv.detach().contiguous(), wg.detach().contiguous()
            if packs is not None and packs[i] is not None:
                wf, wb, bp = packs[i]
            else:
                wf = torch.empty((k, Cb, Ca), dtype=torch.bfloat16, device=dev)
                wb = torch.empty((k, Ca, Cb), dtype=torch.bfloat16, device=dev)
                bp = torch.empty(Cb, dtype=torch.float32, device=dev)
                b32 = None if b is None else b.detach().contiguous()
                with torch.cuda.device(dev):
                    check(lib().psnd_conv1d_prep(ptr(v32), ptr(g32), ptr(b32), Cout, Cin, k, Cb, Ca, ptr(wf), ptr(wb), ptr(bp),
                                                 stream_ptr(dev)), 'psnd_conv1d_prep')
            last = i == n - 1
            inp, slope, has_res = src, (last_act_slope if last else 0.1), role in ('c2', 'r2')
            mk = lambda: torch.empty((shape.N, shape.Lp, Cb), dtype=torch.bfloat16, device=dev)
            if role == 'c1':
                raw, act, res, oslope = None, mk(), None, slope
                pending = act
            elif role == 'tail':
                raw, act, res, oslope = mk(), None, None, 1.0
                cur_x, cur_xa = raw, None
            else:
                raw, act, res, oslope = (mk() if (not last) or want_raw else None), mk(), (cur_x if has_res else None), slope
                cur_x, cur_xa = raw, act
            if (role == 'c2' and _pair_enabled() and plan and plan[-1][0] == 'conv' and steps[-1][10] == 'c1' and plan[-1][5] == Ca == Cb
                    and plan[-1][7] == k and lib().psnd_conv1d_cl_pair_supported(Ca, k, plan[-1][8], plan[-1][9], -pad, dil)):
                _, inp1, wf1, bp1, _, _, _, _, off1, dil1, slope1, _, mid = plan.pop()
                plan.append(('pair', inp1, wf1, bp1, slope1, mid, wf, bp, res, Ca, k, off1, dil1, -pad, dil, oslope, raw, act))
            else:
                plan.append(('conv', inp, wf, bp, res, Ca, Cb, k, -pad, dil, oslope, raw, act))
            steps.append((Cout, Cin, k, Ca, Cb, dil, pad, slope, has_res, b is not None, role))
            saved += [inp, act if act is not None else inp, wb, v32, g32]
        nsec, sides = _sections(dev, shape.N, shape.N * shape.Lp)
        Nh = shape.N // nsec
        plan = _chain_pairs(plan, Nh * shape.Lp)

        def run(h):
            st = stream_ptr(dev)
            q = lambda t: ptr(_sec(t, h, nsec))
            for e in plan:
                if e[0] == 'chain':
                    _, inp1, res0, C, k, pairs = e
                    arr = (_lib.ChainPair * len(pairs))()
                    for d, (_, _, wf1, bp1, slope1, mid, wf2, bp2, _, _, _, off1, dil1, off2, dil2, oslope, raw, act) in zip(arr, pairs):
                        d.W1, d.bias1, d.act1_slope, d.mid_out = wf1.data_ptr(), bp1.data_ptr(), float(slope1), q(mid)
                        d.W2, d.bias2, d.off1, d.dstep1, d.off2, d.dstep2 = wf2.data_ptr(), bp2.data_ptr(), off1, dil1, off2, dil2
                        d.act2_slope, d.out_raw, d.out_act = float(oslope), (q(raw) if raw is pairs[-1][16] else None), q(act)
                    check(lib().psnd_conv1d_cl_chain(q(inp1), q(res0), ctypes.addressof(arr), len(pairs), Nh, shape.Lp, shape.L, shape.HP,
                                                     C, k, st), 'psnd_conv1d_cl_chain')
                    continue
                if e[0] == 'pair':
                    _, inp1, wf1, bp1, slope1, mid, wf2, bp2, res, C, k, off1, dil1, off2, dil2, oslope, raw, act = e
                    check(lib().psnd_conv1d_cl_pair(q(inp1), ptr(wf1), ptr(bp1), None, 1.0, float(slope1), q(mid), ptr(wf2), ptr(bp2),
                                                    None, 1.0, q(res), Nh, shape.Lp, shape.L, shape.HP, C, k, off1, dil1, off2, dil2,
                                                    float(oslope), q(raw), q(act), st), 'psnd_conv1d_cl_pair')
                    continue
                _, inp, wf, bp, res, Ca, Cb, k, off0, dil, oslope, raw, act = e
                check(lib().psnd_conv1d_cl(q(inp), None, None, 1.0, ptr(wf), ptr(bp), q(res), None,
                                           Nh, shape.Lp, shape.L, shape.HP, Ca, Cb, k, off0, dil, float(oslope), 1.0,
                                           q(raw), q(act), None, st), 'psnd_conv1d_cl')

        with torch.cuda.device(dev):
            _run_sections(dev, nsec, sides, run)
        ctx.steps, ctx.shape = steps, shape
        ctx.param_refs = params
        note_param_use(ctx, *params)
        ctx.save_for_backward(*saved)
        return cur_x, cur_xa

    @staticmethod
    def backward(ctx, g_raw, g_act):
        import os
        import struct
        import ctypes
        saved, steps, shape = ctx.saved_tensors, ctx.steps, ctx.shape
        dev = saved[0].device
        n = len(steps)
        if ctx.pack_owner is not None:
            ctx.pack_owner.write_backward_packs()
        g_raw = None if g_raw is None else g_raw.contiguous()
        g_act = None if g_act is None else g_act.contiguous()
        grads = [None] * (3 * n)
        descs, keep = [None] * n, []
        res_pending = None
        sink = GRAD_SINK if (GRAD_SINK is not None and GRAD_SINK.sink_active()) else None
        prefs = getattr(ctx, 'param_refs', None)
        early = {}

        def grad_out(i, v32, g32, Cb):
            gv = gg = gb = None
            if sink is not None and prefs is not None:
                pv, pg, pb = prefs[3 * i:3 * i + 3]
                gv, gg = sink.dest(pv, pv.numel()), sink.dest(pg, pg.numel())
                gb = sink.dest(pb, Cb) if pb is not None else None
                early[i] = [(0, pv) if gv is not None else None, (1, pg) if gg is not None else None,
                            (2, pb) if gb is not None else None]
            gv = torch.empty_like(v32) if gv is None else gv.view_as(v32)
            gg = torch.empty_like(g32) if gg is None else gg.view_as(g32)
            gb = torch.empty(Cb, dtype=torch.float32, device=dev) if gb is None else gb
            return gv, gg, gb

        nsec, sides = _sections(dev, shape.N, shape.N * shape.Lp)
        wstreams = _wgrad_streams(dev) if shape.N * shape.Lp <= 8192 else []
        if wstreams:
            nsec, sides = 1, []
        Nh = shape.N // nsec
        plan = []
        skip = -1
        batch = (nsec == 1 and not wstreams and _pair_enabled() and _sw.lab('PSND_CL_BWD_BATCH', '1') == '1'
                 and shape.N * shape.Lp <= 8192)
        wbatch = []
        own_launch = []
        flush_after = {}
        pair_bwd = (nsec == 1 and not wstreams and not batch and _pair_enabled() and _sw.lab('PSND_CL_PAIR_BWD', '1') != '0'
                    and shape.N * shape.Lp <= 8192)
        lag = None
        with torch.cuda.device(dev):
            g_comb = None
            res_pending = None
            def slabs(i, G1, G2, am, inp, S=None):
                Cout, Cin, k, Ca, Cb, dil, pad, slope = steps[i][:8]
                v32, g32 = saved[5 * i + 3], saved[5 * i + 4]
                if S is None:
                    S = lib().psnd_conv1d_cl_wgrad_splits(Nh, shape.Lp, Ca, Cb, k)
                gw = torch.empty((nsec * S, k, Cb, Ca), dtype=torch.float32, device=dev)
                gbp = torch.empty((nsec * S, Cb), dtype=torch.float32, device=dev)
# ... 341 lines not shown
```

### pytorch_sound_amd/csrc/psnd_conv.hip

```cpp
#include "psnd_common.h"
#include "psnd_conv_pair.h"
#include <stdlib.h>
#include <string.h>
#include <algorithm>
#include <atomic>

namespace {

typedef __attribute__((ext_vector_type(8))) short bf16x8;
typedef __attribute__((ext_vector_type(16))) float f32x16;
typedef unsigned short bf16_t;

__device__ __forceinline__ float bf2f(bf16_t v) { return __builtin_bit_cast(float, (unsigned)v << 16); }
__device__ __forceinline__ bf16_t f2bf(float f) {
    unsigned u = __builtin_bit_cast(unsigned, f);
    if ((u & 0x7fffffffu) > 0x7f800000u) return (bf16_t)((u >> 16) | 0x40);
    u += 0x7fffu + ((u >> 16) & 1u);
    return (bf16_t)(u >> 16);
}

typedef __bf16 hwbf16x2 __attribute__((ext_vector_type(2)));
typedef float f32x2_t __attribute__((ext_vector_type(2)));
__device__ __forceinline__ unsigned pack_bf16(float lo, float hi) {
    const f32x2_t v = {lo, hi};
    return __builtin_bit_cast(unsigned, __builtin_convertvector(v, hwbf16x2));
}

struct ConvParams {
    const bf16_t *A;
    const bf16_t *A2;
    const bf16_t *AM;
    const bf16_t *W;
    const float *bias;
    const bf16_t *res;
    const bf16_t *mask_src;
    bf16_t *out_raw;
    bf16_t *out_act;
    bf16_t *a_eff_out;
    long long R;
    int Lp, L, HP, Ca, Cb, k, off0, dstep, hm;
    float act_slope, mask_slope, a2_slope;
    int up_role, up_u, up_p, up_LpO, up_HPO, up_LO, up_Cr;
    int res_is_a_eff;
#ifdef PSND_TRACE
    long long *trace;
#endif
};
__device__ __forceinline__ long long up_row_base(int Lp, int HP, int u, int pp, int LpO, int HPO, long long r) {
    const long long n = r / Lp;
    const int l = (int)(r - n * Lp);
    const int b = HPO - pp + (l - HP) * u;
    return (b >= 0 && b + u <= LpO) ? n * (long long)LpO + b : -1;
}
#ifdef PSND_TRACE
#define PSND_CSTAMP(i_)                                                                                         \
    do {                                                                                                        \
        if ((threadIdx.x & 63) == 0 && p.trace)                                                                 \
            p.trace[(tblk * 4 + (threadIdx.x >> 6)) * 8 + (i_)] = __builtin_amdgcn_s_memtime(); \
    } while (0)
#else
#define PSND_CSTAMP(i_)
#endif

constexpr int BM = 64, BN = 64, RS = 40;

__device__ __forceinline__ uint4 load_combined(const bf16_t *G1, const bf16_t *G2, const bf16_t *M, float slope, size_t o) {
    uint4 v = make_uint4(0, 0, 0, 0);
    if (G1) v = *reinterpret_cast<const uint4 *>(G1 + o);
    if (G2) {
        const uint4 g2 = *reinterpret_cast<const uint4 *>(G2 + o);
        const uint4 m = *reinterpret_cast<const uint4 *>(M + o);
        const unsigned *pv = reinterpret_cast<const unsigned *>(&v), *pg = reinterpret_cast<const unsigned *>(&g2),
                       *pm = reinterpret_cast<const unsigned *>(&m);
        unsigned out[4];
#pragma unroll
        for (int i = 0; i < 4; ++i) {
            const float a0 = bf2f((bf16_t)(pv[i] & 0xffff)), a1 = bf2f((bf16_t)(pv[i] >> 16));
            const float b0 = bf2f((bf16_t)(pg[i] & 0xffff)), b1 = bf2f((bf16_t)(pg[i] >> 16));
            const float m0 = bf2f((bf16_t)(pm[i] & 0xffff)), m1 = bf2f((bf16_t)(pm[i] >> 16));
            const float r0 = a0 + b0 * (m0 > 0.f ? 1.f : slope), r1 = a1 + b1 * (m1 > 0.f ? 1.f : slope);
            out[i] = pack_bf16(r0, r1);
        }
        v = make_uint4(out[0], out[1], out[2], out[3]);
    }
    return v;
}

constexpr int KFRAG = 16;
#ifndef PSND_DB_PLAIN
#define PSND_DB_PLAIN 4
#endif
#ifndef PSND_DB_COMBINE
#define PSND_DB_COMBINE 2
#endif
__device__ __host__ __forceinline__ size_t pack_index(int , int j, int n, int c, int Nn, int Nc) {
    return ((((size_t)j * (Nn >> 5) + (n >> 5)) * (Nc >> 4) + (c >> 4)) * 64 + (((c & 15) >> 3) << 5) + (n & 31)) * 8 + (c & 7);
}

constexpr int MAXK = 16;
constexpr int KC = 32;
constexpr int PCS = KC / 8;
constexpr int NA = (BM + 2 * 25) * PCS / 256 + 1;

template <int KT, int D, bool COMBINE, int NBUF, int MT, int HMX = 25, bool UPM = false, int KCT = 32, int WNC = 2>
__device__ __forceinline__ void conv_cl_body(const ConvParams &p, const int bx, const int by, bf16_t *smem_c, const size_t tblk) {
    static_assert(KCT == 32, "only 32-channel stages are validated");
    static_assert(WNC == 1 || WNC == 2, "waves across the channels");
    constexpr int KC = KCT, PCS = KCT / 8, KS = KCT / 16;
    constexpr int RS = KC + 8;
    constexpr int BNt = 32 * WNC, BMt = 32 * (4 / WNC) * MT, NAt = (BMt + 2 * HMX) * PCS / 256 + 1;
    const int rowsA = BMt + 2 * p.hm;
    const int buf_elems = rowsA * RS;
    const int tid = threadIdx.x, wave = tid >> 6, lane = tid & 63;
    const int wm = WNC == 2 ? wave >> 1 : wave, wn = WNC == 2 ? wave & 1 : 0;
    const long long r0 = (long long)bx * BMt;
    const int n0 = by * BNt;
    const int li = lane & 31, kg = lane >> 5;

    f32x16 acc[MT];
#pragma unroll
    for (int m = 0; m < MT; ++m)
#pragma unroll
        for (int i = 0; i < 16; ++i) acc[m][i] = 0.f;
    PSND_CSTAMP(0);

    constexpr int TC = 3, NCH = (KT + TC - 1) / TC, UNITS = D * NCH;
    constexpr int DB = D == 1 ? (UNITS % 2 == 0 ? 2 : (UNITS % 3 == 0 ? 3 : 1))
                     : KCT == 64 ? (UNITS % 2 == 0 ? 2 : 1)
                     : KT <= 3 ? (COMBINE ? PSND_DB_COMBINE : PSND_DB_PLAIN) : (UNITS % 4 == 0 ? 4 : (UNITS % 3 == 0 ? 3 : 2));
    static_assert(UNITS % DB == 0, "B ring depth must divide the units of a ring turn (slots are static inside a turn)");
    uint4 ra[D][NAt], ra2[COMBINE ? D : 1][NAt], ram[COMBINE ? D : 1][NAt], rbf[DB][KS * TC];
    const int nA = rowsA * PCS;
    constexpr unsigned OOB = 0xffffffffu;
    const bool upA = UPM && p.up_role == 2;
    const unsigned a_bytes = upA ? (unsigned)((size_t)(p.R / p.Lp) * p.up_LpO * p.up_Cr * sizeof(bf16_t))
                                 : (unsigned)((size_t)p.R * p.Ca * sizeof(bf16_t));
    const unsigned w_bytes = (unsigned)((size_t)p.k * p.Cb * p.Ca * sizeof(bf16_t));
    const __amdgpu_buffer_rsrc_t rA = make_uniform_rsrc(p.A ? p.A : p.A2, (int)a_bytes);
    __amdgpu_buffer_rsrc_t rA2 = rA, rAM = rA;
    if constexpr (COMBINE) rA2 = make_uniform_rsrc(p.A2, (int)a_bytes), rAM = make_uniform_rsrc(p.AM, (int)a_bytes);
    const __amdgpu_buffer_rsrc_t rW = make_uniform_rsrc(p.W, (int)w_bytes);
    const __amdgpu_buffer_rsrc_t rG = make_uniform_rsrc(p.a_eff_out ? p.a_eff_out : p.W,
                                                        (COMBINE && p.a_eff_out && by == 0) ? (int)a_bytes : 0);
    const bool haveA = p.A != nullptr;
    unsigned aoff[NAt];
#pragma unroll
    for (int u = 0; u < NAt; ++u) {
        const int idx = tid + 256 * u;
        const int rr = idx / PCS, pc = idx % PCS;
        const long long r = r0 - p.hm + rr;
        if (!upA) {
            aoff[u] = (idx < nA && r >= 0 && r < p.R) ? (unsigned)(((size_t)r * p.Ca + 8 * pc) * sizeof(bf16_t)) : OOB;
        } else {
            const long long hb = (idx < nA && r >= 0 && r < p.R) ? up_row_base(p.Lp, p.HP, p.up_u, p.up_p, p.up_LpO, p.up_HPO, r) : -1;
// ... 694 lines not shown
                }
            }
        }
    } else {
        constexpr int EP = 68;
        float *sE = reinterpret_cast<float *>(sT);
        static_assert(64 * EP * 4 <= kWgradLdsBytes, "one tap's slab tile fits the chunk buffers");
        const bool vec = (p.Ca % 4 == 0);
#pragma unroll
        for (int j = 0; j < WK; ++j)
            if (j < nt) {
                if (j > 0) __syncthreads();
#pragma unroll
                for (int rg = 0; rg < 16; ++rg) sE[(wm * 32 + (rg & 3) + 8 * (rg >> 2) + 4 * kg) * EP + wn * 32 + li] = acc[j][rg];
                __syncthreads();
                float *dst = p.gw + (((size_t)split * p.k + t0 + j) * p.Cb) * p.Ca;
#pragma unroll
                for (int u = 0; u < 4; ++u) {
                    const int idx = tid + 256 * u, row = idx >> 4, c4 = 4 * (idx & 15);
                    const int co = co0 + row, ci = ci0 + c4;
                    if (co >= p.Cb || ci >= p.Ca) continue;
                    const f32x4 v = *reinterpret_cast<const f32x4 *>(sE + row * EP + c4);
                    if (vec && ci + 3 < p.Ca) {
                        *reinterpret_cast<f32x4 *>(dst + (size_t)co * p.Ca + ci) = v;
                    } else {
                        const float e[4] = {v.x, v.y, v.z, v.w};
                        for (int q = 0; q < 4 && ci + q < p.Ca; ++q) dst[(size_t)co * p.Ca + ci + q] = e[q];
                    }
                }
            }
    }
    __syncthreads();
    PSND_WSTAMP(3);
#ifdef PSND_TRACE
    __builtin_amdgcn_s_waitcnt(0);
    PSND_WSTAMP(4);
#endif
    if (do_bias && p.gbias) {
        float *sb = reinterpret_cast<float *>(sT);
#pragma unroll
        for (int e = 0; e < 8; ++e) {
            float v = bsum[e];
#pragma unroll
            for (int m = 32; m >= 8; m >>= 1) v += __shfl_xor(v, m, 64);
            if ((lane >> 3) == 0) sb[wave * 64 + 8 * cg + e] = v;
        }
        __syncthreads();
        if (tid < 64 && co0 + tid < p.Cb) p.gbias[(size_t)split * p.Cb + co0 + tid] = (sb[tid] + sb[64 + tid]) + (sb[128 + tid] + sb[192 + tid]);
    }
#endif
}
__global__ __launch_bounds__(256, PSND_WGRAD_WAVES) void conv_wgrad_kernel(WgradParams p) {
    extern __shared__ __attribute__((aligned(16))) bf16_t smem_dyn[];
    if (p.G2) conv_wgrad_body<true>(p, blockIdx.x, blockIdx.y, blockIdx.z, smem_dyn, ((size_t)blockIdx.z * gridDim.y + blockIdx.y) * gridDim.x + blockIdx.x);
    else conv_wgrad_body<false>(p, blockIdx.x, blockIdx.y, blockIdx.z, smem_dyn, ((size_t)blockIdx.z * gridDim.y + blockIdx.y) * gridDim.x + blockIdx.x);
}

constexpr int pair_wk(int KT, int HMX) { return HMX != 25 ? WKT : (KT >= 9 ? 6 : (KT >= 5 ? 4 : WKT)); }
template <int KT, int D, int NBUF, bool COMBINE, int MT, int HMX = 25, int KCT = 32, int WNC = 2, bool WN = false>
__global__ __launch_bounds__(256, (D == 1 ? 3 : PSND_CONV_OCC)) void conv_bwd_pair_kernel(ConvParams pc, WgradParams pw, int nw, int wgx, int wgy, int cgx) {
    extern __shared__ __attribute__((aligned(16))) bf16_t smem_dyn[];
    const int b = blockIdx.x;
    if (b < nw) {
        const int bx = b % wgx, r = b / wgx;
        conv_wgrad_body<COMBINE, WN, ((WN || D == 1) ? WKT : pair_wk(KT, HMX))>(pw, bx, r % wgy, r / wgy, smem_dyn, 0);
    } else {
        const int c = b - nw;
        conv_cl_body<KT, D, COMBINE, NBUF, MT, HMX, false, KCT, WNC>(pc, c % cgx, c / cgx, smem_dyn, 0);
    }
}


#ifndef PSND_PAIRBWD_MR
#define PSND_PAIRBWD_MR 1
#endif
#ifndef PSND_PAIRBWD_RU
#define PSND_PAIRBWD_RU 6
#endif
__global__ __launch_bounds__(256, 2) void conv_pair_bwd_kernel(pairk::PairParams pp, WgradParams wa, WgradParams wb_, int nwa, int nwb, int wgx,
                                                               int wgy) {
    extern __shared__ __attribute__((aligned(16))) bf16_t smem_dyn[];
    const int b = blockIdx.x;
    if (b < nwa) {
        const int bx = b % wgx, r = b / wgx;
        conv_wgrad_body<false>(wa, bx, r % wgy, r / wgy, smem_dyn, 0);
    } else if (b < nwa + nwb) {
        const int c = b - nwa, bx = c % wgx, r = c / wgx;
        conv_wgrad_body<false>(wb_, bx, r % wgy, r / wgy, smem_dyn, 0);
    } else {
        pairk::conv_pair_body<256, PSND_PAIRBWD_MR, true, 4, PSND_PAIRBWD_RU>(pp, b - nwa - nwb, smem_dyn);
    }
}

constexpr int WGRAD_MULTI_MAX = 32;
struct WgradMultiArgs {
    WgradParams base;
    int n, linear, ci_fastest;
    struct {
        const bf16_t *g, *xa;
        float *gw, *gb;
        int off0, dstep, Ca, Cb, k, rps, wgx, wgy, splits, tiles, lab0;
    } c[WGRAD_MULTI_MAX];
};
__global__ __launch_bounds__(256, 2) void conv_wgrad_multi_kernel(WgradMultiArgs a) {
    extern __shared__ __attribute__((aligned(16))) bf16_t smem_dyn[];
    const bool lin = a.linear != 0;
    const int label = lin ? 0 : (int)(blockIdx.x & 7), sh = lin ? 0 : 3;
    int t = (int)blockIdx.x >> sh, c = 0, split = 0;
    for (; c < a.n; ++c) {
        const int first = lin ? 0 : (label - a.c[c].lab0) & 7, S = a.c[c].splits, T = a.c[c].tiles;
        const int nb = first < S ? (((S - first - 1) >> sh) + 1) * T : 0;
        if (t < nb) {
            split = first + ((t / T) << sh), t = t % T;
            break;
        }
        t -= nb;
    }
    if (c == a.n) return;
    WgradParams w = a.base;
    w.G1 = a.c[c].g, w.xa = a.c[c].xa, w.gw = a.c[c].gw, w.gbias = a.c[c].gb, w.off0 = a.c[c].off0, w.dstep = a.c[c].dstep;
    w.Ca = a.c[c].Ca, w.Cb = a.c[c].Cb, w.k = a.c[c].k, w.rows_per_split = a.c[c].rps;
    const int wgx = a.c[c].wgx, wgy = a.c[c].wgy, txy = t % (wgx * wgy), tgrp = t / (wgx * wgy);
    const int bx = a.ci_fastest ? txy / wgy : txy % wgx, by = a.ci_fastest ? txy % wgy : txy / wgx;
    conv_wgrad_body<false>(w, bx, by, split * (a.c[c].tiles / (wgx * wgy)) + tgrp, smem_dyn, 0);
}

__global__ __launch_bounds__(256) void conv_prep_kernel(const float *v, const float *g, const float *bias, int Cout, int Cin, int k,
                                                        int Cb, int Ca, bf16_t *wf, bf16_t *wb, float *bp) {
    __shared__ float red[4];
    const int co = blockIdx.x, n = Cin * k;
    const float *vr = v + (size_t)co * n;
    float ss = 0.f;
    for (int i = threadIdx.x; i < n; i += 256) ss = __builtin_fmaf(vr[i], vr[i], ss);
    for (int m = 32; m >= 1; m >>= 1) ss += __shfl_xor(ss, m, 64);
    if ((threadIdx.x & 63) == 0) red[threadIdx.x >> 6] = ss;
    __syncthreads();
    const float scale = g[co] / __builtin_sqrtf(red[0] + red[1] + red[2] + red[3]);
    for (int i = threadIdx.x; i < n; i += 256) {
        const int ci = i / k, j = i - ci * k;
        const bf16_t w = f2bf(vr[i] * scale);
        wf[pack_index(k, j, co, ci, Cb, Ca)] = w;
        wb[pack_index(k, j, ci, co, Ca, Cb)] = w;
    }
    if (threadIdx.x == 0) bp[co] = bias ? bias[co] : 0.f;
}

struct PrepDesc {
    const float *v, *g, *bias;
    bf16_t *wf, *wb;
    float *bp;
    int Cout, Cin, k, Cb, Ca, blk0;
};
constexpr int PREP_ROWS = 8;
__global__ __launch_bounds__(256) void conv_prep_multi_kernel(const PrepDesc *descs, int n, int which) {
    extern __shared__ __attribute__((aligned(16))) bf16_t s_prep[];
    int lo = 0, hi = n - 1;
    while (lo < hi) {
        const int mid = (lo + hi + 1) >> 1;
        if (descs[mid].blk0 <= (int)blockIdx.x) lo = mid;
        else hi = mid - 1;
    }
    const PrepDesc d = descs[lo];
    const int co0 = (blockIdx.x - d.blk0) * PREP_ROWS, nn = d.Cin * d.k;
    if (co0 >= d.Cout) return;
    const int tid = threadIdx.x, lane = tid & 63, w = tid >> 6;
    constexpr int NR = 32;
    if (nn <= 64 * NR) {
        float x[2][NR];
        const float *vr0 = d.v + (size_t)(co0 + 2 * w) * nn;
#pragma unroll
        for (int rr = 0; rr < 2; ++rr) {
            const bool live = co0 + 2 * w + rr < d.Cout;
#pragma unroll
            for (int q = 0; q < NR; ++q) {
                const int i = 64 * q + lane;
                x[rr][q] = (live && i < nn) ? vr0[(size_t)rr * nn + i] : 0.f;
            }
        }
#pragma unroll
        for (int rr = 0; rr < 2; ++rr) {
            const int r = 2 * w + rr, co = co0 + r;
            bf16_t *srow = s_prep + (size_t)r * nn;
            float ss[4] = {0.f, 0.f, 0.f, 0.f};
#pragma unroll
            for (int q = 0; q < NR; ++q) ss[q & 3] = __builtin_fmaf(x[rr][q], x[rr][q], ss[q & 3]);
#pragma unroll
            for (int q = 0; q < 4; ++q)
                for (int m = 32; m >= 1; m >>= 1) ss[q] += __shfl_xor(ss[q], m, 64);
            const float scale = co < d.Cout ? d.g[co] / __builtin_sqrtf(ss[0] + ss[1] + ss[2] + ss[3]) : 0.f;
#pragma unroll
            for (int q = 0; q < NR; ++q) {
                const int i = 64 * q + lane;
                if (i < nn) srow[i] = f2bf(x[rr][q] * scale);
            }
            if (lane == 0 && (which & 1) && co < d.Cout) d.bp[co] = d.bias ? d.bias[co] : 0.f;
        }
    } else {
#pragma unroll
    for (int rr = 0; rr < 2; ++rr) {
        const int r = 2 * w + rr, co = co0 + r;
        bf16_t *srow = s_prep + (size_t)r * nn;
        if (co >= d.Cout) {
            for (int i = lane; i < nn; i += 64) srow[i] = 0;
            continue;
        }
        const float *vr = d.v + (size_t)co * nn;
        float ss[4] = {0.f, 0.f, 0.f, 0.f};
        for (int i0 = 0; i0 < nn; i0 += 256) {
#pragma unroll
            for (int q = 0; q < 4; ++q) {
                const int i = i0 + 64 * q + lane;
                const float x = i < nn ? vr[i] : 0.f;
                ss[q] = __builtin_fmaf(x, x, ss[q]);
            }
        }
#pragma unroll
        for (int q = 0; q < 4; ++q)
            for (int m = 32; m >= 1; m >>= 1) ss[q] += __shfl_xor(ss[q], m, 64);
        const float scale = d.g[co] / __builtin_sqrtf(ss[0] + ss[1] + ss[2] + ss[3]);
        for (int i = lane; i < nn; i += 64) srow[i] = f2bf(vr[i] * scale);
        if (lane == 0 && (which & 1)) d.bp[co] = d.bias ? d.bias[co] : 0.f;
    }
    }
    __syncthreads();
    const int k = d.k, Ca8 = d.Ca >> 3;
    if (which & 1)
    for (int q = tid; q < k * Ca8 * PREP_ROWS; q += 256) {
        const int r = q & (PREP_ROWS - 1), rest = q >> 3;
        const int o = rest % Ca8, j = rest / Ca8;
        const bf16_t *srow = s_prep + (size_t)r * nn + j;
        bf16x8 v;
#pragma unroll
        for (int e = 0; e < 8; ++e) {
            const int ci = 8 * o + e;
            v[e] = ci < d.Cin ? (short)srow[ci * k] : (short)0;
        }
        *reinterpret_cast<bf16x8 *>(d.wf + pack_index(k, j, co0 + r, 8 * o, d.Cb, d.Ca)) = v;
    }
    if (which & 2)
    for (int q = tid; q < k * d.Cin; q += 256) {
        const int ci = q % d.Cin, j = q / d.Cin;
        const bf16_t *sp = s_prep + ci * k + j;
        bf16x8 v;
#pragma unroll
        for (int e = 0; e < 8; ++e) v[e] = (short)sp[(size_t)e * nn];
        *reinterpret_cast<bf16x8 *>(d.wb + pack_index(k, j, ci, co0, d.Ca, d.Cb)) = v;
    }
}

template <bool MANY>
__device__ __forceinline__ void conv_finish_body(const float *gw_part, const float *gb_part, int splits, const float *v,
                                                 const float *g, int Cin, int k, int Cb, int Ca, float *gv,
                                                 float *gg, float *gbias, unsigned kmagic, unsigned cmagic, const int co, float *s_gw,
                                                 float *red) {
    const int n = Cin * k, BD = blockDim.x, tid = threadIdx.x;
    const int pitch = Cin + 1;
    if constexpr (!MANY) {
        if ((Cin & 3) == 0 && (Ca & 3) == 0 && splits <= 16) {
            const int cin4 = Cin >> 2, n4 = n >> 2;
            const size_t slab4 = (size_t)k * Cb * Ca;
            const float *vrow = v + (size_t)co * n;
            float bsum = 0.f;
            if (tid < 64 && gbias && gb_part)
                for (int sp = tid; sp < splits; sp += 64) bsum += gb_part[(size_t)sp * Cb + co];
            for (int q = tid; q < n4; q += BD) {
                const int j = q / cin4, c4 = q - j * cin4;
                const float *src = gw_part + ((size_t)j * Cb + co) * Ca + 4 * c4;
                f32x4 a = {0.f, 0.f, 0.f, 0.f};
                auto add_slabs = [&](auto nc) __attribute__((always_inline)) {
                    constexpr int NS = decltype(nc)::value;
                    f32x4 t[NS];
#pragma unroll
                    for (int u = 0; u < NS; ++u) t[u] = *reinterpret_cast<const f32x4 *>(src + (size_t)(u < splits ? u : splits - 1) * slab4);
#pragma unroll
                    for (int u = 0; u < NS; ++u) {
                        const f32x4 z = {0.f, 0.f, 0.f, 0.f};
                        a += u < splits ? t[u] : z;
                    }
                };
                if (splits <= 2) add_slabs(std::integral_constant<int, 2>{});
                else if (splits <= 4) add_slabs(std::integral_constant<int, 4>{});
                else if (splits <= 8) add_slabs(std::integral_constant<int, 8>{});
                else add_slabs(std::integral_constant<int, 16>{});
                float *dst = s_gw + j * pitch + 4 * c4;
                dst[0] = a.x, dst[1] = a.y, dst[2] = a.z, dst[3] = a.w;
            }
            __syncthreads();
            float ss4 = 0.f, dot4 = 0.f;
            for (int q = tid; q < n4; q += BD) {
                const f32x4 vv = *reinterpret_cast<const f32x4 *>(vrow + 4 * q);
#pragma unroll
                for (int e = 0; e < 4; ++e) {
                    const int i = 4 * q + e, ci = (int)__umulhi((unsigned)i, kmagic), j = i - ci * k;
                    ss4 = __builtin_fmaf(vv[e], vv[e], ss4);
                    dot4 = __builtin_fmaf(vv[e], s_gw[j * pitch + ci], dot4);
                }
            }
            for (int m = 32; m >= 1; m >>= 1) {
                ss4 += __shfl_xor(ss4, m, 64);
                dot4 += __shfl_xor(dot4, m, 64);
            }
            const int nw4 = BD >> 6;
            if ((tid & 63) == 0) red[tid >> 6] = ss4, red[16 + (tid >> 6)] = dot4;
            __syncthreads();
            float sst = 0.f, dott = 0.f;
            for (int w = 0; w < nw4; ++w) sst += red[w], dott += red[16 + w];
            const float inv = 1.f / __builtin_sqrtf(sst);
            const float dd = dott * inv;
            const float gs = g[co] * inv;
            for (int q = tid; q < n4; q += BD) {
                const f32x4 vv = *reinterpret_cast<const f32x4 *>(vrow + 4 * q);
                f32x4 o;
#pragma unroll
                for (int e = 0; e < 4; ++e) {
                    const int i = 4 * q + e, ci = (int)__umulhi((unsigned)i, kmagic), j = i - ci * k;
                    o[e] = gs * (s_gw[j * pitch + ci] - vv[e] * inv * dd);
                }
                *reinterpret_cast<f32x4 *>(gv + (size_t)co * n + 4 * q) = o;
            }
            if (tid == 0) gg[co] = dd;
            if (tid < 64 && gbias && gb_part) {
                float b = bsum;
                for (int m = 32; m >= 1; m >>= 1) b += __shfl_xor(b, m, 64);
                if (tid == 0) gbias[co] = b;
            }
            return;
        }
    }
    const size_t slab = (size_t)k * Cb * Ca;
    const float *vr = v + (size_t)co * n;
    float ss = 0.f, dot = 0.f;
    if constexpr (MANY) {
        int EP = 64;
        while (EP < n && EP < BD) EP <<= 1;
        const int NSG = BD / EP, e = tid & (EP - 1), sg = tid / EP;
        float *s_part = s_gw + pitch * k;
        for (int e0 = 0; e0 < n; e0 += EP) {
            const int ee = e0 + e;
            const bool ok = ee < n;
            const int j = (int)__umulhi((unsigned)ee, cmagic), c = ee - j * Cin;
            const float *src = gw_part + ((size_t)j * Cb + co) * Ca + c;
            float acc = 0.f;
            for (int sp0 = sg; sp0 < splits; sp0 += 8 * NSG) {
                float t[8];
#pragma unroll
                for (int u = 0; u < 8; ++u) t[u] = (ok && sp0 + u * NSG < splits) ? src[(size_t)(sp0 + u * NSG) * slab] : 0.f;
                acc += ((t[0] + t[1]) + (t[2] + t[3])) + ((t[4] + t[5]) + (t[6] + t[7]));
            }
            if (NSG > 1) {
                s_part[sg * EP + e] = acc;
                __syncthreads();
                if (sg == 0 && ok) {
                    float a2 = 0.f;
                    for (int q = 0; q < NSG; ++q) a2 += s_part[q * EP + e];
                    s_gw[j * pitch + c] = a2;
                }
                __syncthreads();
            } else if (ok) {
                s_gw[j * pitch + c] = acc;
            }
        }
    } else
    for (int e0 = tid; e0 < n; e0 += 4 * BD) {
        int jj[4], cc[4];
        float gsum[4] = {0.f, 0.f, 0.f, 0.f};
#pragma unroll
        for (int q = 0; q < 4; ++q) {
            const int e = e0 + BD * q;
            jj[q] = (int)__umulhi((unsigned)e, cmagic);
            cc[q] = e - jj[q] * Cin;
        }
        {
            float t[4][16];
#pragma unroll
            for (int q = 0; q < 4; ++q) {
                const float *src = gw_part + ((size_t)jj[q] * Cb + co) * Ca + cc[q];
#pragma unroll
                for (int u = 0; u < 16; ++u) t[q][u] = (e0 + BD * q < n && u < splits) ? src[(size_t)u * slab] : 0.f;
            }
#pragma unroll
            for (int q = 0; q < 4; ++q)
                gsum[q] += ((t[q][0] + t[q][1]) + (t[q][2] + t[q][3])) + ((t[q][4] + t[q][5]) + (t[q][6] + t[q][7])) +
                           (((t[q][8] + t[q][9]) + (t[q][10] + t[q][11])) + ((t[q][12] + t[q][13]) + (t[q][14] + t[q][15])));
        }
#pragma unroll
        for (int q = 0; q < 4; ++q)
            if (e0 + BD * q < n) s_gw[jj[q] * pitch + cc[q]] = gsum[q];
    }
    __syncthreads();
    for (int i = tid; i < n; i += BD) {
        const int ci = (int)__umulhi((unsigned)i, kmagic), j = i - ci * k;
        const float vv = vr[i];
        ss += vv * vv;
        dot += vv * s_gw[j * pitch + ci];
    }
    for (int m = 32; m >= 1; m >>= 1) {
        ss += __shfl_xor(ss, m, 64);
        dot += __shfl_xor(dot, m, 64);
    }
    const int nw = BD >> 6;
// ... 466 lines not shown
    fill(wa, G, xa_a, -pad2, dil2, gw_a, gb_a);
    fill(wb_, G_b, xa_b, off_b, dstep_b, gw_b, gb_b);
    pairk::PairParams pp;
    memset(&pp, 0, sizeof(pp));
    int tiles = 0;
    size_t lds = kWgradLdsBytes;
    if (have_pair) {
        pp.A = static_cast<const pairk::bf16_t *>(G), pp.W1 = static_cast<const pairk::bf16_t *>(wb2), pp.W2 = static_cast<const pairk::bf16_t *>(wb1);
        pp.bias1 = nullptr, pp.bias2 = nullptr;
        pp.M1 = static_cast<const pairk::bf16_t *>(M1), pp.M2 = static_cast<const pairk::bf16_t *>(M2), pp.res = static_cast<const pairk::bf16_t *>(res);
        pp.mid_out = static_cast<pairk::bf16_t *>(g_mid), pp.out_raw = static_cast<pairk::bf16_t *>(gx), pp.out_act = nullptr;
        pp.R = R, pp.Lp = Lp, pp.L = L, pp.HP = HP;
        pp.off1 = pad2, pp.dstep1 = -dil2, pp.h1 = pairk::reach3(pad2, -dil2);
        pp.off2 = pad1, pp.dstep2 = -dil1, pp.h2 = pairk::reach3(pad1, -dil1);
        pp.m1_slope = m1_slope, pp.m2_slope = m2_slope, pp.act1_slope = 1.f, pp.act2_slope = 1.f, pp.trace = nullptr;
        const int MRW = 32 * PSND_PAIRBWD_MR, TS = MRW - 2 * pp.h2;
        tiles = (int)((R + TS - 1) / TS);
        const size_t lp = (size_t)(MRW + 2 * pp.h1 + MRW + 2 * pp.h2) * (C + 8) * 2, lo = (size_t)MRW * (C + 8) * 4;
        if (lds < lp) lds = lp;
        if (lds < lo) lds = lo;
    }
    const int nwa = have_pair ? wgx * wgy * wgz : 0, nwb = have_b ? wgx * wgy * wgz : 0;
    hipLaunchKernelGGL(conv_pair_bwd_kernel, dim3((unsigned)(nwa + nwb + tiles)), dim3(256), lds, static_cast<hipStream_t>(stream), pp, wa, wb_, nwa,
                       nwb, wgx, wgy);
    PSND_CHECK_LAUNCH("conv1d_cl_pair_bwd");
    if (have_pair) g_conv_pair_stats[2]++;
    g_conv_pair_stats[3].store(splits);
    return PSND_OK;
}

extern "C" int psnd_conv1d_cl_bwd(const void *G1, const void *G2, const void *GM, float g2_slope, const void *wb, const void *xa,
                                  int64_t N, int Lp, int L, int HP, int Ca, int Cb, int k, int pad, int dil, void *gx, void *g_out,
                                  const void *gx_mask, float gx_mask_slope, const void *gx_res, float *gw_part, float *gbias_part,
                                  void *stream) {
    static const bool no_pair = PSND_ENV("PSND_NO_BWD_PAIR") != nullptr;
    if (gw_part && (k < WKT ? k - 1 : WKT - 1) * (dil < 0 ? -dil : dil) > WXR - 32)
        PSND_FAIL(PSND_E_UNSUPPORTED, "conv1d_cl_bwd: dilation %d: a tap group spans more than %d rows", dil, WXR - 32);
    int hm = 0;
    for (int j = 0; j < k; ++j) {
        const int o = pad - j * dil;
        hm = (o < 0 ? -o : o) > hm ? (o < 0 ? -o : o) : hm;
    }
    const size_t buf = sizeof(bf16_t) * 40 * (size_t)(BM + 2 * hm);
    const bool pairable = !no_pair && (G1 || G2) && (!G2 || GM) && gx && wb && xa && gw_part && k >= 1 && k <= 16 && (hm <= 25 || (hm <= 40 && k <= 7)) && hm <= HP && N > 0 &&
                          Ca % 32 == 0 && Cb % 32 == 0 && L > 0 && Lp >= L + 2 * HP &&
                          (size_t)N * Lp * (Ca > Cb ? Ca : Cb) * 2 < ((size_t)1 << 32) && (size_t)k * Cb * Ca * 2 < ((size_t)1 << 32);
    if (!pairable) {
        if (gw_part) {
            int rc = psnd_conv1d_cl_wgrad(G1, G2, GM, g2_slope, xa, N, Lp, Ca, Cb, k, -pad, dil, gw_part, gbias_part, nullptr, stream);
            if (rc != PSND_OK) return rc;
        }
        if (gx_res && gx_res == g_out) PSND_FAIL(PSND_E_UNSUPPORTED, "conv1d_cl_bwd: residual = combined gradient outside the paired launch");
        return psnd_conv1d_cl(G1, G2, GM, g2_slope, wb, nullptr, gx_res, gx_mask, N, Lp, L, HP, Cb, Ca, k, pad, -dil, 1.f, gx_mask_slope, gx,
                              nullptr, g_out, stream);
    }
    ConvParams pc;
    conv_params_plain(pc);
    pc.A = static_cast<const bf16_t *>(G1), pc.A2 = static_cast<const bf16_t *>(G2), pc.AM = static_cast<const bf16_t *>(GM);
    pc.a2_slope = g2_slope;
    pc.W = static_cast<const bf16_t *>(wb), pc.bias = nullptr;
    pc.res = static_cast<const bf16_t *>(gx_res), pc.mask_src = static_cast<const bf16_t *>(gx_mask);
    pc.out_raw = static_cast<bf16_t *>(gx), pc.out_act = nullptr, pc.a_eff_out = static_cast<bf16_t *>(g_out);
    if (gx_res && gx_res == g_out) {
        if (Ca != Cb) PSND_FAIL(PSND_E_SHAPE, "conv1d_cl_bwd: gx_res == g_out needs Ca == Cb");
        pc.res = nullptr, pc.res_is_a_eff = 1;
    }
    pc.R = N * (int64_t)Lp, pc.Lp = Lp, pc.L = L, pc.HP = HP, pc.Ca = Cb, pc.Cb = Ca, pc.k = k, pc.off0 = pad, pc.dstep = -dil, pc.hm = hm;
    pc.act_slope = 1.f, pc.mask_slope = gx_mask_slope;
    WgradParams pw;
    wgrad_params_plain(pw);
    pw.G1 = pc.A, pw.G2 = pc.A2, pw.GM = pc.AM;
    pw.xa = static_cast<const bf16_t *>(xa), pw.gw = gw_part, pw.gbias = gbias_part, pw.g_out = nullptr;
    pw.R = pc.R, pw.Ca = Ca, pw.Cb = Cb, pw.k = k, pw.off0 = -pad, pw.dstep = dil, pw.g2_slope = g2_slope;
    int64_t rps;
    const int splits = wgrad_splits(pw.R, Ca, Cb, k, &rps);
    pw.rows_per_split = (int)rps;
    const char *pe = PSND_ENV("PSND_PAIR_MT");
    const int pair_mt = pe ? atoi(pe) : 0;
    const bool can3 = !G2 && hm <= 25 && Ca > 32;
    const int mt = (pair_mt == 1 || pair_mt == 2 || (pair_mt == 3 && can3)) ? pair_mt : ((can3 && conv_row_tiles(pc.R, Ca, true) == 3) ? 3 : 2);
    const bool narrow = Ca <= 32 && mt == 2 && hm <= 25 && !G2 && (pc.R + 63) / 64 >= 1024 && !PSND_ENV("PSND_CONV_NO_NARROW");
    const int bm = narrow ? 256 : 64 * mt, bn = narrow ? 32 : BN;
    const int cgx = (int)((pc.R + bm - 1) / bm), cgy = (Ca + bn - 1) / bn;
    const bool wn = Ca <= 32 && Cb <= 32 && (pc.R + 63) / 64 >= 1024 && hm <= 25 && gw_part &&
                    ((k < 4 * WKT ? k : 4 * WKT) - 1) * (dil < 0 ? -dil : dil) <= WXRN - 32 && !PSND_ENV("PSND_CONV_NO_NARROW");
    const bool narrow1 = narrow && Cb <= 32;
    const int wk = wn ? 4 * WKT : (narrow1 ? WKT : pair_wk(k <= 3 ? 3 : (k <= 7 ? 7 : (k <= 11 ? 11 : 16)), hm > 25 ? 40 : 25));
    if (gw_part && !wn && ((k < wk ? k : wk) - 1) * (dil < 0 ? -dil : dil) > WXR - 32)
        PSND_FAIL(PSND_E_UNSUPPORTED, "conv1d_cl_bwd: dilation %d: a group of %d taps spans more than %d rows", dil, wk, WXR - 32);
    const int wgx = (Cb + 63) / 64, wgy = (Ca + 63) / 64, wgz = splits * ((k + wk - 1) / wk);
    const int nw = wgx * wgy * wgz;
    const int kct = 32;
    size_t lds = 2 * sizeof(bf16_t) * (kct + 8) * (size_t)(bm + 2 * hm);
    if (lds < sizeof(float) * bm * (bn + 8)) lds = sizeof(float) * bm * (bn + 8);
    if (lds < (size_t)kWgradLdsBytes) lds = kWgradLdsBytes;
    if (wn && lds < (size_t)kWgradNarrowLdsBytes) lds = kWgradNarrowLdsBytes;
    hipStream_t st = static_cast<hipStream_t>(stream);
#define PSND_PAIR_LAUNCH(KT_, D_, C_, H_)                                                                              \
    do {                                                                                                              \
        auto kern = mt == 2 ? conv_bwd_pair_kernel<KT_, (C_ ? 2 : (D_ > 4 ? 4 : D_)), 2, C_, 2, H_> : conv_bwd_pair_kernel<KT_, D_, 2, C_, 1, H_>;   \
        if constexpr (H_ == 25 && !C_) {                                                                              \
            if (mt == 3) kern = conv_bwd_pair_kernel<KT_, (D_ > 4 ? 4 : D_), 2, false, 3, H_>;                        \
        }                                                                                                             \
        if constexpr (H_ == 25) {                                                                                     \
            if (wn && mt == 2) kern = conv_bwd_pair_kernel<KT_, (C_ ? 2 : (D_ > 4 ? 4 : D_)), 2, C_, 2, H_, 32, 2, true>;   \
        }                                                                                                             \
        if constexpr (H_ == 25 && !C_) {                                                                              \
            if (narrow1 && wn) kern = conv_bwd_pair_kernel<KT_, 1, 2, false, 2, H_, 32, 1, true>;    \
            else if (narrow1) kern = conv_bwd_pair_kernel<KT_, 1, 2, false, 2, H_, 32, 1>;                            \
            else if (narrow) kern = conv_bwd_pair_kernel<KT_, (D_ > 4 ? 4 : D_), 2, false, 2, H_, 32, 1>;             \
        }                                                                                                             \
        if (lds > 64 * 1024) {                                                                                        \
            hipError_t e = hipFuncSetAttribute(reinterpret_cast<const void *>(kern),                                  \
                                               hipFuncAttributeMaxDynamicSharedMemorySize, (int)lds);                 \
            if (e != hipSuccess) PSND_FAIL(PSND_E_HIP, "conv1d_cl_bwd: set LDS size: %s", hipGetErrorString(e));      \
        }                                                                                                             \
        hipLaunchKernelGGL(kern, dim3((unsigned)(nw + cgx * cgy)), dim3(256), lds, st, pc, pw, nw, wgx, wgy, cgx);    \
    } while (0)
    if (hm > 25 && !G2) PSND_PAIR_LAUNCH(7, 3, false, 40);
    else if (hm > 25) PSND_PAIR_LAUNCH(7, 3, true, 40);
    else if (k <= 3 && !G2) PSND_PAIR_LAUNCH(3, 8, false, 25);
    else if (k <= 3) PSND_PAIR_LAUNCH(3, 4, true, 25);
    else if (k <= 7 && !G2) PSND_PAIR_LAUNCH(7, 3, false, 25);
    else if (k <= 7) PSND_PAIR_LAUNCH(7, 3, true, 25);
    else if (k <= 11 && !G2) PSND_PAIR_LAUNCH(11, 2, false, 25);
    else if (k <= 11) PSND_PAIR_LAUNCH(11, 2, true, 25);
    else if (!G2) PSND_PAIR_LAUNCH(16, 2, false, 25);
    else PSND_PAIR_LAUNCH(16, 2, true, 25);
#undef PSND_PAIR_LAUNCH
    PSND_CHECK_LAUNCH("conv1d_cl_bwd");
    g_conv_stats[mt == 2 ? 3 : 2]++;
    return PSND_OK;
}

extern "C" int psnd_conv1d_prep(const float *v, const float *g, const float *bias, int Cout, int Cin, int k, int Cb, int Ca,
                                void *wf, void *wb, float *bias_padded, void *stream) {
    if (!v || !g || !wf || !wb || !bias_padded) PSND_FAIL(PSND_E_ARG, "conv1d_prep: null pointer");
    if (Cb < Cout || Ca < Cin) PSND_FAIL(PSND_E_SHAPE, "conv1d_prep: padded sizes too small");
    hipStream_t s = static_cast<hipStream_t>(stream);
    const size_t nw = sizeof(bf16_t) * (size_t)k * Cb * Ca;
    hipError_t e = hipSuccess;
    if (Cb != Cout || Ca != Cin) {
        e = hipMemsetAsync(wf, 0, nw, s);
        if (e == hipSuccess) e = hipMemsetAsync(wb, 0, nw, s);
        if (e == hipSuccess) e = hipMemsetAsync(bias_padded, 0, sizeof(float) * Cb, s);
    }
    if (e != hipSuccess) PSND_FAIL(PSND_E_HIP, "conv1d_prep: memset: %s", hipGetErrorString(e));
    hipLaunchKernelGGL(conv_prep_kernel, dim3(Cout), dim3(256), 0, s, v, g, bias, Cout, Cin, k, Cb, Ca,
                       static_cast<bf16_t *>(wf), static_cast<bf16_t *>(wb), bias_padded);
    PSND_CHECK_LAUNCH("conv1d_prep");
    return PSND_OK;
}

extern "C" int psnd_conv1d_prep_multi(const void *descs_dev, int n, int total_blocks, int max_row, int which, void *stream) {
    if (!descs_dev || n <= 0 || total_blocks <= 0 || max_row <= 0 || which < 1 || which > 3) PSND_FAIL(PSND_E_ARG, "conv1d_prep_multi: bad arguments");
    const size_t lds = (size_t)PREP_ROWS * (size_t)max_row * sizeof(bf16_t);
    if (lds > 160 * 1024) PSND_FAIL(PSND_E_SHAPE, "conv1d_prep_multi: Cin * k = %d too large for the 8-row tile (use psnd_conv1d_prep)", max_row);
    if (lds > 48 * 1024) {
        hipError_t e = hipFuncSetAttribute(reinterpret_cast<const void *>(conv_prep_multi_kernel), hipFuncAttributeMaxDynamicSharedMemorySize, (int)lds);
        if (e != hipSuccess) PSND_FAIL(PSND_E_HIP, "conv1d_prep_multi: set LDS size: %s", hipGetErrorString(e));
    }
    hipLaunchKernelGGL(conv_prep_multi_kernel, dim3(total_blocks), dim3(256), lds, static_cast<hipStream_t>(stream),
                       static_cast<const PrepDesc *>(descs_dev), n, which);
    PSND_CHECK_LAUNCH("conv1d_prep_multi");
    return PSND_OK;
}

extern "C" int psnd_conv1d_wnorm_bwd(const float *gw_part, const float *gbias_part, int splits, const float *v, const float *g,
                                     int Cout, int Cin, int k, int Cb, int Ca, float *gv, float *gg, float *gbias, void *stream) {
    if (!gw_part || !v || !g || !gv || !gg || splits < 1) PSND_FAIL(PSND_E_ARG, "conv1d_wnorm_bwd: null pointer / splits");
    const size_t lds = sizeof(float) * (size_t)(Cin + 1) * k;
    if (lds > 60 * 1024) PSND_FAIL(PSND_E_SHAPE, "conv1d_wnorm_bwd: Cin*k=%d too large", Cin * k);
    const unsigned kmagic = (unsigned)((0x100000000ull + (unsigned)k - 1) / (unsigned)k);
    const unsigned cmagic = (unsigned)((0x100000000ull + (unsigned)Cin - 1) / (unsigned)Cin);
    const int threads = Cin * k >= 2048 ? 1024 : 256;
    if (splits > 16)
        hipLaunchKernelGGL(conv_finish_kernel<true>, dim3(Cout), dim3(1024), lds + 4096, static_cast<hipStream_t>(stream), gw_part,
                           gbias_part, splits, v, g, Cout, Cin, k, Cb, Ca, gv, gg, gbias, kmagic, cmagic);
    else
        hipLaunchKernelGGL(conv_finish_kernel<false>, dim3(Cout), dim3(threads), lds, static_cast<hipStream_t>(stream), gw_part,
                           gbias_part, splits, v, g, Cout, Cin, k, Cb, Ca, gv, gg, gbias, kmagic, cmagic);
    PSND_CHECK_LAUNCH("conv1d_wnorm_bwd");
    return PSND_OK;
}

extern "C" int psnd_conv1d_wnorm_bwd_multi(const psnd_wnorm_desc *descs, int n, void *stream) {
    if (!descs || n < 1 || n > PSND_WNORM_MAX) PSND_FAIL(PSND_E_ARG, "conv1d_wnorm_bwd_multi: %d descriptors (1..%d)", n, PSND_WNORM_MAX);
    FinishArgs a;
    a.n = n;
    size_t lds = 0;
    int total = 0, maxn = 0, maxsplits = 0;
    for (int i = 0; i < n; ++i) {
        const psnd_wnorm_desc &d = descs[i];
        if (!d.gw_part || !d.v || !d.g || !d.gv || !d.gg || d.splits < 1 || d.Cout < 1 || d.Cin < 1 || d.k < 1)
            PSND_FAIL(PSND_E_ARG, "conv1d_wnorm_bwd_multi: descriptor %d: null pointer / bad sizes", i);
        const size_t l = sizeof(float) * (size_t)(d.Cin + 1) * d.k;
        if (l > 60 * 1024) PSND_FAIL(PSND_E_SHAPE, "conv1d_wnorm_bwd_multi: Cin*k=%d too large", d.Cin * d.k);
        lds = l > lds ? l : lds;
        a.d[i] = d;
        a.kmagic[i] = (unsigned)((0x100000000ull + (unsigned)d.k - 1) / (unsigned)d.k);
        a.cmagic[i] = (unsigned)((0x100000000ull + (unsigned)d.Cin - 1) / (unsigned)d.Cin);
        a.blk0[i] = total;
        total += d.Cout;
        maxn = d.Cin * d.k > maxn ? d.Cin * d.k : maxn;
        maxsplits = d.splits > maxsplits ? d.splits : maxsplits;
    }
    a.blk0[n] = total;
    const int threads = maxn >= 2048 ? 1024 : 256;
    if (maxsplits > 16)
        hipLaunchKernelGGL(conv_finish_multi_kernel<true>, dim3(total), dim3(1024), lds + 4096, static_cast<hipStream_t>(stream), a);
    else
        hipLaunchKernelGGL(conv_finish_multi_kernel<false>, dim3(total), dim3(threads), lds, static_cast<hipStream_t>(stream), a);
    PSND_CHECK_LAUNCH("conv1d_wnorm_bwd_multi");
    return PSND_OK;
}

namespace {

__global__ __launch_bounds__(256) void convtr_prep_kernel(const float *v, const float *g, const float *bias, int Cin, int Cout, int K, int u,
                                                          int Cr, int Cip, bf16_t *wf, bf16_t *wb, float *bp) {
    __shared__ float red[4];
    const int ci = blockIdx.x, n = Cout * K;
    const float *vr = v + (size_t)ci * n;
    float ss = 0.f;
    for (int i = threadIdx.x; i < n; i += 256) ss += vr[i] * vr[i];
    for (int m = 32; m >= 1; m >>= 1) ss += __shfl_xor(ss, m, 64);
    if ((threadIdx.x & 63) == 0) red[threadIdx.x >> 6] = ss;
    __syncthreads();
    const float scale = g[ci] / __builtin_sqrtf(red[0] + red[1] + red[2] + red[3]);
    const int Nn = u * Cr;
    for (int i = threadIdx.x; i < n; i += 256) {
        const int co = i / K, jk = i - co * K;
        const int tap = jk / u, phi = jk - tap * u;
        const bf16_t w = f2bf(vr[i] * scale);
        wf[pack_index(2, tap, phi * Cr + co, ci, Nn, Cip)] = w;
        wb[pack_index(2, tap, ci, phi * Cr + co, Cip, Nn)] = w;
    }
    if (ci == 0)
        for (int i = threadIdx.x; i < Nn; i += 256) {
            const int co = i % Cr;
            bp[i] = (bias && co < Cout) ? bias[co] : 0.f;
        }
}

__global__ __launch_bounds__(1024) void convtr_finish_kernel(const float *gw_part, int splits, const float *v, const float *g, int Cin,
                                                             int Cout, int K, int u, int Cr, int Cip, float *gv, float *gg) {
    extern __shared__ float s_gw[];
    __shared__ float red[32];
    const int ci = blockIdx.x, n = Cout * K, Nn = u * Cr, BD = blockDim.x, tid = threadIdx.x;
    const size_t slab = (size_t)2 * Cip * Nn;
    const float *vr = v + (size_t)ci * n;
    float ss = 0.f, dot = 0.f;
    const int E = 2 * u * Cout;
    int EP = 64;
    while (EP < E && EP < BD) EP <<= 1;
    const int NSG = BD / EP, el = tid & (EP - 1), sg = tid / EP;
    float *s_part = s_gw + n;
    for (int e0 = 0; e0 < E; e0 += EP) {
        const int e = e0 + el;
        const bool ok = e < E;
        const int co = e % Cout, tp = e / Cout;
        const int tap = tp / u, phi = tp - tap * u;
        const float *src = gw_part + ((size_t)tap * Cip + ci) * Nn + phi * Cr + co;
        float a = 0.f;
        for (int sp0 = sg; sp0 < splits; sp0 += 8 * NSG) {
            float t[8];
#pragma unroll
            for (int q = 0; q < 8; ++q) t[q] = (ok && sp0 + q * NSG < splits) ? src[(size_t)(sp0 + q * NSG) * slab] : 0.f;
            a += ((t[0] + t[1]) + (t[2] + t[3])) + ((t[4] + t[5]) + (t[6] + t[7]));
        }
        if (NSG > 1) {
            s_part[sg * EP + el] = a;
            __syncthreads();
            if (sg == 0 && ok) {
                float a2 = 0.f;
                for (int q = 0; q < NSG; ++q) a2 += s_part[q * EP + el];
                s_gw[co * K + tp] = a2;
            }
            __syncthreads();
        } else if (ok) {
            s_gw[co * K + tp] = a;
        }
    }
    __syncthreads();
    for (int i = tid; i < n; i += BD) {
        const float vv = vr[i];
        ss += vv * vv;
        dot += vv * s_gw[i];
    }
    for (int m = 32; m >= 1; m >>= 1) {
        ss += __shfl_xor(ss, m, 64);
        dot += __shfl_xor(dot, m, 64);
    }
    const int nw = BD >> 6;
    if ((tid & 63) == 0) red[tid >> 6] = ss, red[16 + (tid >> 6)] = dot;
    __syncthreads();
    float sst = 0.f, dott = 0.f;
    for (int w = 0; w < nw; ++w) sst += red[w], dott += red[16 + w];
    const float inv = 1.f / __builtin_sqrtf(sst);
    const float d = dott * inv;
    const float gs = g[ci] * inv;
    for (int i = tid; i < n; i += BD) gv[(size_t)ci * n + i] = gs * (s_gw[i] - vr[i] * inv * d);
    if (tid == 0) gg[ci] = d;
}

__global__ __launch_bounds__(256) void cl_mean_act_kernel(const bf16_t *a, const bf16_t *b, const bf16_t *c, const bf16_t *d, int count,
                                                          float slope, bf16_t *out, size_t n8) {
    const size_t i = (size_t)blockIdx.x * 256 + threadIdx.x;
    if (i >= n8) return;
    const bf16_t *src[4] = {a, b, c, d};
    float acc[8] = {0.f, 0.f, 0.f, 0.f, 0.f, 0.f, 0.f, 0.f};
    for (int s = 0; s < count; ++s) {
        const uint4 q = reinterpret_cast<const uint4 *>(src[s])[i];
        const unsigned *pq = reinterpret_cast<const unsigned *>(&q);
#pragma unroll
        for (int e = 0; e < 4; ++e) acc[2 * e] += bf2f((bf16_t)(pq[e] & 0xffff)), acc[2 * e + 1] += bf2f((bf16_t)(pq[e] >> 16));
    }
    unsigned w[4];
// ... 322 lines not shown
```

### pytorch_sound_amd/csrc/psnd_core.hip

```cpp
#include "psnd_common.h"

static thread_local char g_err[512] = "";

void psnd_set_error(const char *fmt, ...) {
    va_list ap;
    va_start(ap, fmt);
    vsnprintf(g_err, sizeof(g_err), fmt, ap);
    va_end(ap);
}

extern "C" int psnd_version(void) { return 141; }

extern "C" const char *psnd_last_error(void) { return g_err; }

#ifdef PSND_LAB
std::atomic<int> g_psnd_env_gen{0};
extern "C" void psnd_env_refresh(void) { g_psnd_env_gen.fetch_add(1, std::memory_order_acq_rel); }
#endif

static inline int64_t pad_of(int n_fft, int hop, int framing) {
    if (framing == PSND_FRAMING_NONE) return 0;
    return framing == PSND_FRAMING_CENTER ? n_fft / 2 : (n_fft - hop) / 2;
}

extern "C" int64_t psnd_frame_count(int64_t T, int n_fft, int hop, int framing) {
    if (T <= 0 || n_fft <= 0 || hop <= 0) return 0;
    const int64_t L = T + 2 * pad_of(n_fft, hop, framing);
    if (L < n_fft) return 0;
    return (L - n_fft) / hop + 1;
}

extern "C" int64_t psnd_frame_sample_index(int64_t f, int m, int64_t T, int n_fft, int hop, int framing) {
    int64_t i = f * hop - pad_of(n_fft, hop, framing) + m;
    if (i < 0) i = -i;
    if (i >= T) i = 2 * (T - 1) - i;
    return i;
}

extern "C" void *psnd_event_create(void) {
    hipEvent_t ev = nullptr;
    if (hipEventCreateWithFlags(&ev, hipEventDisableTiming) != hipSuccess) {
        psnd_set_error("event_create: %s", hipGetErrorString(hipGetLastError()));
        return nullptr;
    }
    return ev;
}
extern "C" int psnd_event_destroy(void *ev) {
    if (!ev) return PSND_OK;
    if (hipEventDestroy(static_cast<hipEvent_t>(ev)) != hipSuccess) PSND_FAIL(PSND_E_HIP, "event_destroy: %s", hipGetErrorString(hipGetLastError()));
    return PSND_OK;
}
extern "C" int psnd_event_record_external(void *ev, void *stream) {
    if (!ev) PSND_FAIL(PSND_E_ARG, "event_record_external: null event");
    hipStream_t s = static_cast<hipStream_t>(stream);
    hipStreamCaptureStatus st = hipStreamCaptureStatusNone;
    if (hipStreamIsCapturing(s, &st) != hipSuccess) st = hipStreamCaptureStatusNone;
    const hipError_t e = st == hipStreamCaptureStatusActive ? hipEventRecordWithFlags(static_cast<hipEvent_t>(ev), s, hipEventRecordExternal)
                                                            : hipEventRecord(static_cast<hipEvent_t>(ev), s);
    if (e != hipSuccess) {
        (void)hipGetLastError();
        PSND_FAIL(PSND_E_HIP, "event_record_external: %s", hipGetErrorString(e));
    }
    return PSND_OK;
}
extern "C" int psnd_event_external_supported(void) {
    static int cached = -1;
    if (cached >= 0) return cached;
    int ok = 0;
    hipStream_t s = nullptr;
    hipEvent_t ev = nullptr;
    hipGraph_t g = nullptr;
    if (hipStreamCreateWithFlags(&s, hipStreamNonBlocking) == hipSuccess && hipEventCreateWithFlags(&ev, hipEventDisableTiming) == hipSuccess) {
        if (hipStreamBeginCapture(s, hipStreamCaptureModeThreadLocal) == hipSuccess) {
            const hipError_t e = hipEventRecordWithFlags(ev, s, hipEventRecordExternal);
            const hipError_t e2 = hipStreamEndCapture(s, &g);
            ok = (e == hipSuccess && e2 == hipSuccess) ? 1 : 0;
            if (g) (void)hipGraphDestroy(g);
        }
    }
    if (ev) (void)hipEventDestroy(ev);
    if (s) (void)hipStreamDestroy(s);
    (void)hipGetLastError();
    cached = ok;
    return ok;
}
extern "C" int psnd_stream_wait_event(void *stream, void *ev) {
    if (!ev) PSND_FAIL(PSND_E_ARG, "stream_wait_event: null event");
    const hipError_t e = hipStreamWaitEvent(static_cast<hipStream_t>(stream), static_cast<hipEvent_t>(ev), 0);
    if (e != hipSuccess) PSND_FAIL(PSND_E_HIP, "stream_wait_event: %s", hipGetErrorString(e));
    return PSND_OK;
}

__global__ __launch_bounds__(256) void polar_bwd_kernel(const float *__restrict__ gmag, const float *__restrict__ gphase,
                                                        const float *__restrict__ mag, const float *__restrict__ phase, long long n,
                                                        float *__restrict__ gre, float *__restrict__ gim) {
    const long long stride = (long long)gridDim.x * 256 * 4;
    for (long long i = ((long long)blockIdx.x * 256 + threadIdx.x) * 4; i < n; i += stride) {
        float gm[4] = {0.f, 0.f, 0.f, 0.f}, gp[4] = {0.f, 0.f, 0.f, 0.f}, m[4], ph[4], o_re[4], o_im[4];
        const int cnt = n - i >= 4 ? 4 : (int)(n - i);
        if (cnt == 4 && (n & 3) == 0) {
            *reinterpret_cast<float4 *>(m) = *reinterpret_cast<const float4 *>(mag + i);
            *reinterpret_cast<float4 *>(ph) = *reinterpret_cast<const float4 *>(phase + i);
            if (gmag) *reinterpret_cast<float4 *>(gm) = *reinterpret_cast<const float4 *>(gmag + i);
            if (gphase) *reinterpret_cast<float4 *>(gp) = *reinterpret_cast<const float4 *>(gphase + i);
        } else {
            for (int j = 0; j < cnt; ++j) {
                m[j] = mag[i + j], ph[j] = phase[i + j];
                if (gmag) gm[j] = gmag[i + j];
                if (gphase) gp[j] = gphase[i + j];
            }
        }
        for (int j = 0; j < 4; ++j) {
            float sn, cs;
            sn = sinf(ph[j]), cs = cosf(ph[j]);
            const float q = gphase ? gp[j] / m[j] : 0.f;
            o_re[j] = gm[j] * cs - q * sn;
            o_im[j] = gm[j] * sn + q * cs;
        }
        if (cnt == 4 && (n & 3) == 0) {
            *reinterpret_cast<float4 *>(gre + i) = *reinterpret_cast<float4 *>(o_re);
            *reinterpret_cast<float4 *>(gim + i) = *reinterpret_cast<float4 *>(o_im);
        } else {
            for (int j = 0; j < cnt; ++j) gre[i + j] = o_re[j], gim[i + j] = o_im[j];
        }
    }
}
extern "C" int psnd_polar_bwd(const float *gmag, const float *gphase, const float *mag, const float *phase, int64_t n, float *gre,
                              float *gim, void *stream) {
    if (!mag || !phase || !gre || !gim) PSND_FAIL(PSND_E_ARG, "polar_bwd: null mag/phase/gre/gim");
    if (!gmag && !gphase) PSND_FAIL(PSND_E_ARG, "polar_bwd: neither gmag nor gphase given");
    if (n < 0) PSND_FAIL(PSND_E_ARG, "polar_bwd: n=%lld", (long long)n);
    if (n == 0) return PSND_OK;
    long long blocks = (n + 1023) / 1024;
    if (blocks > 8192) blocks = 8192;
    hipLaunchKernelGGL(polar_bwd_kernel, dim3((unsigned)blocks), dim3(256), 0, static_cast<hipStream_t>(stream), gmag, gphase, mag, phase,
                       (long long)n, gre, gim);
    PSND_CHECK_LAUNCH("polar_bwd");
    return PSND_OK;
}
```

### pytorch_sound_amd/csrc/psnd_nfk.hip

```cpp
#include "psnd_common.h"

namespace {

typedef unsigned short bf16_t;
typedef __bf16 hwbf16x2 __attribute__((ext_vector_type(2)));

__device__ __forceinline__ float bf_lo(unsigned v) { return __builtin_bit_cast(float, v << 16); }
__device__ __forceinline__ float bf_hi(unsigned v) { return __builtin_bit_cast(float, v & 0xffff0000u); }
__device__ __forceinline__ unsigned pack_bf16(float lo, float hi) {
    const f32x2 v = {lo, hi};
    return __builtin_bit_cast(unsigned, __builtin_convertvector(v, hwbf16x2));
}

struct Row8 {
    float v[8];
};
__device__ __forceinline__ Row8 load8(__amdgpu_buffer_rsrc_t r, unsigned row_byte, int c0, int K, bool row_ok) {
    Row8 o;
    constexpr unsigned OOB = 0xffffffffu;
    if (c0 + 8 <= K) {
        const unsigned b = row_ok ? row_byte + 4u * (unsigned)c0 : OOB;
        const f32x4 a = __builtin_bit_cast(f32x4, __builtin_amdgcn_raw_buffer_load_b128(r, (int)b, 0, 0));
        const f32x4 c = __builtin_bit_cast(f32x4, __builtin_amdgcn_raw_buffer_load_b128(r, (int)(row_ok ? b + 16u : OOB), 0, 0));
        o.v[0] = a.x, o.v[1] = a.y, o.v[2] = a.z, o.v[3] = a.w, o.v[4] = c.x, o.v[5] = c.y, o.v[6] = c.z, o.v[7] = c.w;
    } else {
#pragma unroll
        for (int j = 0; j < 8; ++j)
            o.v[j] = __builtin_bit_cast(float, __builtin_amdgcn_raw_buffer_load_b32(r, (int)((row_ok && c0 + j < K) ? row_byte + 4u * (unsigned)(c0 + j) : OOB), 0, 0));
    }
    return o;
}
__device__ __forceinline__ void store8(__amdgpu_buffer_rsrc_t r, unsigned row_byte, int c0, int K, const float (&v)[8]) {
    if (c0 + 8 <= K) {
        __builtin_amdgcn_raw_buffer_store_b128(__builtin_bit_cast(u32x4, f32x4{v[0], v[1], v[2], v[3]}), r, (int)(row_byte + 4u * (unsigned)c0), 0, 0);
        __builtin_amdgcn_raw_buffer_store_b128(__builtin_bit_cast(u32x4, f32x4{v[4], v[5], v[6], v[7]}), r, (int)(row_byte + 4u * (unsigned)c0 + 16u), 0, 0);
    } else {
#pragma unroll
        for (int j = 0; j < 8; ++j)
            if (c0 + j < K) __builtin_amdgcn_raw_buffer_store_b32(__builtin_bit_cast(unsigned, v[j]), r, (int)(row_byte + 4u * (unsigned)(c0 + j)), 0, 0);
    }
}

struct NfkParams {
    const float *x;
    const float *ref;
    const float *est_in;
    const float *gest;
    const float *g;
    const bf16_t *y;
    bf16_t *out_cl;
    float *est;
    double *part;
    long long items;
    int N, F, K, Lp, HP, Cp, preop;
    unsigned tensor_bytes;
    float coef;
};

template <bool MASKBWD>
__global__ __launch_bounds__(256) void to_cl_nfk_kernel(NfkParams p) {
    const long long it = (long long)blockIdx.x * 256 + threadIdx.x;
    if (it >= p.items) return;
    const int cpr = p.Cp >> 3;
    const long long row = it / cpr;
    const int c0 = (int)(it - row * cpr) * 8;
    const int n = (int)(row / p.Lp), l = (int)(row - (long long)n * p.Lp), t = l - p.HP;
    const bool ok = t >= 0 && t < p.F;
    const unsigned rb = (unsigned)(((size_t)n * p.F + (size_t)(ok ? t : 0)) * p.K * 4);
    const int tb = (int)p.tensor_bytes;
    const __amdgpu_buffer_rsrc_t rx = make_uniform_rsrc(p.x, tb);
    float w[8];
    if constexpr (!MASKBWD) {
        const Row8 a = load8(rx, rb, c0, p.K, ok);
#pragma unroll
        for (int j = 0; j < 8; ++j) {
            float v = a.v[j];
            if (p.preop == 1) {
                const float u = 1.f + v;
                v = u == 1.f ? v : __logf(u) * __fdividef(v, u - 1.f);
            }
            w[j] = v;
        }
    } else {
        const __amdgpu_buffer_rsrc_t re = make_uniform_rsrc(p.est_in, tb), rr = make_uniform_rsrc(p.ref, tb);
        const __amdgpu_buffer_rsrc_t rg = make_uniform_rsrc(p.gest ? p.gest : p.x, p.gest ? tb : 0);
        const Row8 m = load8(rx, rb, c0, p.K, ok), e = load8(re, rb, c0, p.K, ok), r = load8(rr, rb, c0, p.K, ok), ge = load8(rg, rb, c0, p.K, ok);
        const u32x4 yq = *reinterpret_cast<const u32x4 *>(p.y + (size_t)row * p.Cp + c0);
        const float l1c = p.coef * p.g[0];
#pragma unroll
        for (int j = 0; j < 8; ++j) {
            const unsigned q = yq[j >> 1];
            const float yv = (j & 1) ? bf_hi(q) : bf_lo(q);
            const float sg = 1.f / (1.f + __expf(-yv));
            const float d = e.v[j] - r.v[j];
            const float gg = ge.v[j] + l1c * (d > 0.f ? 1.f : (d < 0.f ? -1.f : 0.f));
            w[j] = gg * m.v[j] * sg * (1.f - sg);
        }
    }
    const u32x4 o = {pack_bf16(w[0], w[1]), pack_bf16(w[2], w[3]), pack_bf16(w[4], w[5]), pack_bf16(w[6], w[7])};
    *reinterpret_cast<u32x4 *>(p.out_cl + (size_t)row * p.Cp + c0) = o;
}

__global__ __launch_bounds__(256) void mask_head_nfk_kernel(NfkParams p) {
    const long long it = (long long)blockIdx.x * 256 + threadIdx.x;
    const int cpr = (p.K + 7) >> 3;
    float acc = 0.f;
    if (it < p.items) {
        const long long row = it / cpr;
        const int c0 = (int)(it - row * cpr) * 8;
        const int n = (int)(row / p.F), t = (int)(row - (long long)n * p.F);
        const unsigned rb = (unsigned)((size_t)row * p.K * 4);
        const int tb = (int)p.tensor_bytes;
        const __amdgpu_buffer_rsrc_t rm = make_uniform_rsrc(p.x, tb), rr = make_uniform_rsrc(p.ref ? p.ref : p.x, p.ref ? tb : 0);
        const __amdgpu_buffer_rsrc_t ro = make_uniform_rsrc(p.est, tb);
        const Row8 m = load8(rm, rb, c0, p.K, true), r = load8(rr, rb, c0, p.K, true);
        const u32x4 yq = *reinterpret_cast<const u32x4 *>(p.y + ((size_t)n * p.Lp + p.HP + t) * p.Cp + c0);
        float v[8];
#pragma unroll
        for (int j = 0; j < 8; ++j) {
            const unsigned q = yq[j >> 1];
            const float yv = (j & 1) ? bf_hi(q) : bf_lo(q);
            v[j] = m.v[j] / (1.f + __expf(-yv));
            if (c0 + j < p.K) acc += __builtin_fabsf(v[j] - r.v[j]);
        }
        store8(ro, rb, c0, p.K, v);
    }
    if (p.part) {
        double d = (double)acc;
#pragma unroll
        for (int m = 32; m >= 1; m >>= 1) d += __shfl_xor(d, m, 64);
        __shared__ double red[4];
        if ((threadIdx.x & 63) == 0) red[threadIdx.x >> 6] = d;
        __syncthreads();
        if (threadIdx.x == 0) p.part[blockIdx.x] = red[0] + red[1] + red[2] + red[3];
    }
}

int check_shape(const char *what, int64_t N, int K, int64_t F, int Lp, int HP, int Cp) {
    if (N < 0 || K <= 0 || F <= 0 || HP < 0 || Lp < F + 2 * HP || Cp < ((K + 7) & ~7) || Cp % 8 != 0 || (size_t)N * (size_t)K * (size_t)F * 4 >= ((size_t)1 << 32) - 64 ||
        (size_t)Lp * Cp * 2 >= ((size_t)1 << 31) || N * (int64_t)Lp * (Cp / 8) >= ((int64_t)1 << 39))
        PSND_FAIL(PSND_E_SHAPE, "%s: N=%lld K=%d F=%lld Lp=%d HP=%d Cp=%d", what, (long long)N, K, (long long)F, Lp, HP, Cp);
    return PSND_OK;
}

}

extern "C" int psnd_to_cl_nfk(const float *x_nfk, int64_t N, int K, int64_t F, int Lp, int HP, int Cp, int preop, void *out, void *stream) {
    if (!x_nfk || !out) PSND_FAIL(PSND_E_ARG, "to_cl_nfk: null pointer");
    if (preop < 0 || preop > 1) PSND_FAIL(PSND_E_ARG, "to_cl_nfk: preop=%d", preop);
    if (int rc = check_shape("to_cl_nfk", N, K, F, Lp, HP, Cp)) return rc;
    if (N == 0) return PSND_OK;
    NfkParams p = {};
    p.x = x_nfk, p.out_cl = static_cast<bf16_t *>(out), p.N = (int)N, p.F = (int)F, p.K = K, p.Lp = Lp, p.HP = HP, p.Cp = Cp, p.preop = preop;
    p.items = N * (int64_t)Lp * (Cp / 8);
    p.tensor_bytes = (unsigned)((size_t)N * F * K * 4);
    hipLaunchKernelGGL(to_cl_nfk_kernel<false>, dim3((unsigned)((p.items + 255) / 256)), dim3(256), 0, static_cast<hipStream_t>(stream), p);
    PSND_CHECK_LAUNCH("to_cl_nfk");
    return PSND_OK;
}

extern "C" int64_t psnd_mask_head_l1_blocks_nfk(int64_t N, int64_t F, int K) {
    if (N <= 0 || F <= 0 || K <= 0) return 0;
    return (N * F * ((K + 7) / 8) + 255) / 256;
}

extern "C" int psnd_mask_head_l1_fwd_nfk(const void *y, const float *mag_nfk, const float *ref_nfk, int64_t N, int K, int64_t F, int Lp, int HP,
                                         int Cp, float *est_nfk, double *part, void *stream) {
    if (!y || !mag_nfk || !est_nfk) PSND_FAIL(PSND_E_ARG, "mask_head_l1_fwd_nfk: null pointer");
    if ((ref_nfk == nullptr) != (part == nullptr)) PSND_FAIL(PSND_E_ARG, "mask_head_l1_fwd_nfk: ref and part go together");
    if (int rc = check_shape("mask_head_l1_fwd_nfk", N, K, F, Lp, HP, Cp)) return rc;
    if (N == 0) return PSND_OK;
    NfkParams p = {};
    p.x = mag_nfk, p.ref = ref_nfk, p.y = static_cast<const bf16_t *>(y), p.est = est_nfk, p.part = part;
    p.N = (int)N, p.F = (int)F, p.K = K, p.Lp = Lp, p.HP = HP, p.Cp = Cp;
    p.items = N * F * ((K + 7) / 8);
    p.tensor_bytes = (unsigned)((size_t)N * F * K * 4);
    hipLaunchKernelGGL(mask_head_nfk_kernel, dim3((unsigned)((p.items + 255) / 256)), dim3(256), 0, static_cast<hipStream_t>(stream), p);
    PSND_CHECK_LAUNCH("mask_head_l1_fwd_nfk");
    return PSND_OK;
}

extern "C" int psnd_mask_head_l1_bwd_nfk(const float *gest_nfk, const float *mag_nfk, const void *y, const float *est_nfk, const float *ref_nfk,
                                         const float *g, float coef, int64_t N, int K, int64_t F, int Lp, int HP, int Cp, void *gy, void *stream) {
    if (!mag_nfk || !y || !est_nfk || !ref_nfk || !g || !gy) PSND_FAIL(PSND_E_ARG, "mask_head_l1_bwd_nfk: null pointer");
    if (int rc = check_shape("mask_head_l1_bwd_nfk", N, K, F, Lp, HP, Cp)) return rc;
    if (N == 0) return PSND_OK;
    NfkParams p = {};
    p.x = mag_nfk, p.ref = ref_nfk, p.est_in = est_nfk, p.gest = gest_nfk, p.g = g, p.coef = coef, p.y = static_cast<const bf16_t *>(y);
    p.out_cl = static_cast<bf16_t *>(gy), p.N = (int)N, p.F = (int)F, p.K = K, p.Lp = Lp, p.HP = HP, p.Cp = Cp;
    p.items = N * (int64_t)Lp * (Cp / 8);
    p.tensor_bytes = (unsigned)((size_t)N * F * K * 4);
    hipLaunchKernelGGL(to_cl_nfk_kernel<true>, dim3((unsigned)((p.items + 255) / 256)), dim3(256), 0, static_cast<hipStream_t>(stream), p);
    PSND_CHECK_LAUNCH("mask_head_l1_bwd_nfk");
    return PSND_OK;
}
```

### pytorch_sound_amd/models/separator.py

```python
import torch
import torch.nn as nn
import torch.nn.functional as F

from pytorch_sound_amd.models import register_model, register_model_architecture
from pytorch_sound_amd.models.vocoders.hifi_gan import WNConv1d, ResBlock1, LRELU_SLOPE, wants_bf16


@register_model('conv_separator')
class ConvSeparator(nn.Module):
    def __init__(self, spec_size: int = 513, channels: int = 256, num_blocks: int = 4, kernel_size: int = 3,
                 dilation=(1, 3, 5)):
        super().__init__()
        self.conv_pre = WNConv1d(spec_size, channels, 3, 1, 1)
        self.blocks = nn.ModuleList([ResBlock1(None, channels, kernel_size, tuple(dilation)) for _ in range(num_blocks)])
        self.conv_post = WNConv1d(channels, spec_size, 3, 1, 1, init_std=0.01)

    precision = 'auto'

    def forward(self, mag: torch.Tensor) -> torch.Tensor:
        from pytorch_sound_amd import deferred
        if mag.is_cuda and wants_bf16(self.precision, mag):
            node = deferred.nfk_of(mag) if deferred.ENABLED else None
            if node is not None:
                y, shape = self.logits_cl(node.nfk, 'nfk')
                return deferred.est(y, None, shape, node)
            return self.forward_cl(deferred.resolve(mag))
        mag = deferred.resolve(mag)
        if mag.is_cuda:
            with torch.autocast('cuda', enabled=False):
                return self._forward_plain(mag.float()).to(mag.dtype)
        return self._forward_plain(mag)

    def _forward_plain(self, mag):
        x = self.conv_pre(torch.log1p(mag))
        for block in self.blocks:
            x = block(x)
        mask = torch.sigmoid(self.conv_post(x, LRELU_SLOPE))
        return mask * mag


    def logits_cl(self, mag: torch.Tensor, layout: str = 'nkf'):
        from pytorch_sound_amd import cl
        if layout == 'nfk':
            N, T, C = mag.shape
        else:
            N, C, T = mag.shape
        halo = max(c.padding for b in self.blocks for c in list(b.convs1) + list(b.convs2))
        shape = cl.CLShape(N, T, max(halo, self.conv_pre.padding, self.conv_post.padding))
        convs = [self.conv_pre] + [c for b in self.blocks for c in list(b.convs1) + list(b.convs2)] + [self.conv_post]
        prep = cl.prep_all(self, convs, defer_backward_packs=True)
        x0 = cl.to_cl_nfk(mag.float(), shape, 1) if layout == 'nfk' else cl.ToCL.apply(mag.float(), shape, 1)
        return cl.conv_body_cl(self.conv_pre, list(self.blocks), self.conv_post, x0, shape, prep), shape

    def spectral_l1_loss(self, mag: torch.Tensor, mag_ref: torch.Tensor, mel_ref: torch.Tensor, mel_plan: torch.Tensor, n_mels: int,
                         w_mag: float = 1.0, w_mel: float = 0.5, log_offset: float = 1e-6, clamp_lo=None, clamp_hi=None, layout: str = 'nkf'):
        from pytorch_sound_amd import cl, kernels as K
        if not mag.is_cuda:
            raise RuntimeError('spectral_l1_loss is the fused HIP formulation; on the host compose the loss from forward()')
        if layout == 'nfk':
            y, shape = self.logits_cl(mag, 'nfk')
            loss, est = cl.MaskHeadSpectralL1NFK.apply(y, mag.float().contiguous(), mag_ref.float().contiguous(), mel_ref.float().contiguous(),
                                                       mel_plan, shape, n_mels, K.LOG_E, log_offset, None, clamp_lo, clamp_hi, w_mag, w_mel)
            loss.psnd_nan_flag = cl.LAST_LOSS_NAN_FLAG[0]
            return loss, est
        y, shape = self.logits_cl(mag)
        loss, est = cl.MaskHeadSpectralL1CL.apply(y, mag.float().contiguous(), mag_ref.float().contiguous(), mel_ref.float().contiguous(),
                                                  mel_plan, shape, n_mels, K.LOG_E, log_offset, None, clamp_lo, clamp_hi, w_mag, w_mel)
        loss.psnd_nan_flag = cl.LAST_LOSS_NAN_FLAG[0]
        return loss, est

    def forward_cl(self, mag: torch.Tensor) -> torch.Tensor:
        from pytorch_sound_amd import cl
        N, C, T = mag.shape
        halo = max(c.padding for b in self.blocks for c in list(b.convs1) + list(b.convs2))
        shape = cl.CLShape(N, T, max(halo, self.conv_pre.padding, self.conv_post.padding))
        convs = [self.conv_pre] + [c for b in self.blocks for c in list(b.convs1) + list(b.convs2)] + [self.conv_post]
        prep = cl.prep_all(self, convs, defer_backward_packs=True)
        x0 = cl.ToCL.apply(mag.float(), shape, 1)
        y = cl.conv_body_cl(self.conv_pre, list(self.blocks), self.conv_post, x0, shape, prep)
        if mag.dtype == torch.float32 and not mag.requires_grad:
            from pytorch_sound_amd import deferred
            if deferred.ENABLED:
                return deferred.est(y, mag.contiguous(), shape)
            return cl.MaskHeadCL.apply(y, mag, shape)
        logits = cl.FromCL.apply(y, C, T, shape)
        return torch.sigmoid(logits) * mag


@register_model_architecture('conv_separator', 'conv_separator_voicebank')
def conv_separator_voicebank():
    return {'spec_size': 513, 'channels': 256, 'num_blocks': 4, 'kernel_size': 3, 'dilation': (1, 3, 5)}
```

Measured before the change: 102,900 audio-s/s.

## Run weight-prep blocks alongside layout conversion and mask-head backward in one launch

Merges the conv weight-normalization prep kernel with the NFK-to-channels-last conversion kernel into a single launch. Leading workgroups run the prep and the remaining ones do the layout transform. The deferred backward weight packs are likewise launched together with the mask-head L1 backward kernel, tracked through a per-device pending-pack registry. This aims to cut kernel launches and let two small, independent kernels fill the GPU together. In exchange it adds shared-LDS sizing for the layout blocks and bookkeeping state that must stay consistent across forward and backward.

After: 104,300 audio-s/s, median of 6. 1.01x the previous value.

```diff
diff --git a/include/psnd.h b/include/psnd.h
--- a/include/psnd.h
+++ b/include/psnd.h
@@ -171,6 +171,12 @@
 int psnd_cl_colsum_splits(int64_t rows, int C);
 int psnd_cl_colsum(const void *g, int64_t rows, int C, int Lp, int lo, int hi, float *part, float *out, void *stream);
 int psnd_conv1d_prep_multi(const void *descs_dev, int n, int total_blocks, int max_row, int which, void *stream);
+int psnd_conv1d_prep_multi_to_cl_nfk(const void *descs_dev, int n, int total_blocks, int max_row, int which, const float *x_nfk, int64_t N,
+                                     int K, int64_t F, int Lp, int HP, int Cp, int preop, void *out, void *stream);
+int psnd_conv1d_prep_multi_mask_head_l1_bwd_nfk(const void *descs_dev, int n, int total_blocks, int max_row, int which, const float *gest_nfk,
+                                                const float *mag_nfk, const void *y, const float *est_nfk, const float *ref_nfk,
+                                                const float *g, float coef, int64_t N, int K, int64_t F, int Lp, int HP, int Cp, void *gy,
+                                                void *stream);
 #define PSND_WNORM_MAX 32
 typedef struct psnd_wnorm_desc {
     const float *gw_part, *gbias_part;
diff --git a/pytorch_sound_amd/_lib.py b/pytorch_sound_amd/_lib.py
--- a/pytorch_sound_amd/_lib.py
+++ b/pytorch_sound_amd/_lib.py
@@ -68,6 +68,9 @@
                                        _P, _P, _INT, _INT, _P, _P, _P]),
     'psnd_conv1d_wnorm_bwd_multi': (_INT, [_P, _INT, _P]),
     'psnd_conv1d_prep_multi': (_INT, [_P, _INT, _INT, _INT, _INT, _P]),
+    'psnd_conv1d_prep_multi_to_cl_nfk': (_INT, [_P, _INT, _INT, _INT, _INT, _P, _I64, _INT, _I64, _INT, _INT, _INT, _INT, _P, _P]),
+    'psnd_conv1d_prep_multi_mask_head_l1_bwd_nfk': (_INT, [_P, _INT, _INT, _INT, _INT, _P, _P, _P, _P, _P, _P, _F, _I64, _INT, _I64, _INT, _INT,
+                                                            _INT, _P, _P]),
     'psnd_conv1d_cl_wgrad_splits': (_INT, [_I64, _INT, _INT, _INT, _INT]),
     'psnd_mask_head_l1_blocks': (_I64, [_I64, _I64, _INT]),
     'psnd_masked_l1_blocks': (_I64, [_I64]),
diff --git a/pytorch_sound_amd/cl.py b/pytorch_sound_amd/cl.py
--- a/pytorch_sound_amd/cl.py
+++ b/pytorch_sound_amd/cl.py
@@ -209,7 +209,7 @@
         return (gy,) + (None,) * 13
 
 
-def to_cl_nfk(x_nfk, shape, preop=0):
+def _to_cl_nfk_out(x_nfk, shape):
     _need(x_nfk, torch.float32)
     if x_nfk.requires_grad and torch.is_grad_enabled():
         raise _lib.PsndError('to_cl_nfk carries no gradient (feature tensors are inputs); use ToCL on an (N, K, F) tensor')
@@ -217,7 +217,11 @@
     if F != shape.L or N != shape.N:
         raise _lib.PsndError('to_cl_nfk: tensor %s does not match the CL geometry (N=%d, L=%d)' % (tuple(x_nfk.shape), shape.N, shape.L))
     Cp = round_up(K, ALIGN_C)
-    out = torch.empty((N, shape.Lp, Cp), dtype=torch.bfloat16, device=x_nfk.device)
+    return N, F, K, Cp, torch.empty((N, shape.Lp, Cp), dtype=torch.bfloat16, device=x_nfk.device)
+
+
+def to_cl_nfk(x_nfk, shape, preop=0):
+    N, F, K, Cp, out = _to_cl_nfk_out(x_nfk, shape)
     with torch.cuda.device(x_nfk.device):
         check(lib().psnd_to_cl_nfk(ptr(x_nfk), N, K, F, shape.Lp, shape.HP, Cp, int(preop), ptr(out), stream_ptr(x_nfk.device)),
               'psnd_to_cl_nfk')
@@ -261,6 +265,7 @@
         ctx.cfg = (shape, M, log_kind, float(log_offset), pre, lo, hi, float(w1) / mag.numel(), float(w2) / mel_ref.numel())
         ctx.save_for_backward(y, mag, mag_ref, mel_ref, mel_plan, est, lin)
         ctx.mark_non_differentiable(est)
+        ctx.pending_packs = _PENDING_BACKWARD_PACKS.get(dev)
         return out, est
 
     @staticmethod
@@ -270,6 +275,7 @@
         N, F, K = mag.shape
         if g is None:
             return (None,) * 14
+        cache = _take_pending_backward_packs(y.device, ctx.pending_packs)
         g = g.contiguous().float()
         gest = torch.empty_like(mag)
         gy = torch.empty_like(y)
@@ -277,8 +283,15 @@
         with torch.cuda.device(y.device):
             check(lib().psnd_mel_l1_bwd_nfk(ptr(mel_ref), ptr(lin), ptr(g), c2, N, F, M, K, ptr(mel_plan), log_kind, log_offset, pre, lo, hi,
                                             ptr(gest), st), 'psnd_mel_l1_bwd_nfk')
-            check(lib().psnd_mask_head_l1_bwd_nfk(ptr(gest), ptr(mag), ptr(y), ptr(est), ptr(mag_ref), ptr(g), c1, N, K, F, shape.Lp,
-                                                  shape.HP, y.shape[2], ptr(gy), st), 'psnd_mask_head_l1_bwd_nfk')
+            if cache is not None:
+                cache['wb_done'] = True
+                check(lib().psnd_conv1d_prep_multi_mask_head_l1_bwd_nfk(ptr(cache['table']), cache['n'], cache['blocks'], cache['max_row'], 2,
+                                                                        ptr(gest), ptr(mag), ptr(y), ptr(est), ptr(mag_ref), ptr(g), c1, N, K, F,
+                                                                        shape.Lp, shape.HP, y.shape[2], ptr(gy), st),
+                      'psnd_conv1d_prep_multi_mask_head_l1_bwd_nfk')
+            else:
+                check(lib().psnd_mask_head_l1_bwd_nfk(ptr(gest), ptr(mag), ptr(y), ptr(est), ptr(mag_ref), ptr(g), c1, N, K, F, shape.Lp,
+                                                      shape.HP, y.shape[2], ptr(gy), st), 'psnd_mask_head_l1_bwd_nfk')
         return (gy,) + (None,) * 13
 
 
@@ -793,9 +806,26 @@
                   'psnd_conv1d_prep_multi')
 
 
-def prep_all(owner, convs, defer_backward_packs=False):
+_PENDING_BACKWARD_PACKS = {}
+
+
+def _prep_ride_enabled():
+    return _sw.lab('PSND_NO_PREP_RIDE') != '1'
+
+
+def _take_pending_backward_packs(dev, entry):
+    if entry is None or _PENDING_BACKWARD_PACKS.get(dev) is not entry:
+        return None
+    del _PENDING_BACKWARD_PACKS[dev]
+    packs = entry[1]()
+    cache = None if packs is None else packs.deferred
+    if cache is None or cache['wb_done'] or cache['key'] != entry[0] or not _prep_ride_enabled():
+        return None
+    return cache
+
+
+def _prep_cache(owner, convs):
     import struct
-    import os
     if _sw.lab('PSND_NO_PREP_ALL') == '1':
         return None
     if any(c.weight_v.shape[1] * c.weight_v.shape[2] > 10240 for c in convs):
@@ -825,13 +855,48 @@
     for c in convs:
         if not (c.weight_v.is_contiguous() and c.weight_g.is_contiguous() and c.weight_v.dtype == torch.float32):
             raise _lib.PsndError('prep_all: fp32 contiguous weight_v / weight_g expected')
-    defer = bool(defer_backward_packs) and torch.is_grad_enabled() and _sw.lab('PSND_PREP_NO_DEFER') != '1'
+    return cache
+
+
+def _prep_defer(defer_backward_packs):
+    return bool(defer_backward_packs) and torch.is_grad_enabled() and _sw.lab('PSND_PREP_NO_DEFER') != '1'
+
+
+def _prep_launched(cache, defer):
+    cache['wb_done'] = not defer
+    cache['packs'].deferred = cache if defer else None
+    _PENDING_BACKWARD_PACKS.pop(cache['dev'], None)
+    if defer:
+        _PENDING_BACKWARD_PACKS[cache['dev']] = (cache['key'], weakref.ref(cache['packs']))
+    return cache['packs']
+
+
+def prep_all(owner, convs, defer_backward_packs=False):
+    _PENDING_BACKWARD_PACKS.pop(convs[0].weight_v.device, None)
+    cache = _prep_cache(owner, convs)
+    if cache is None:
+        return None
+    defer = _prep_defer(defer_backward_packs)
     with torch.cuda.device(cache['dev']):
         check(lib().psnd_conv1d_prep_multi(ptr(cache['table']), cache['n'], cache['blocks'], cache['max_row'], 1 if defer else 3,
                                            stream_ptr(cache['dev'])), 'psnd_conv1d_prep_multi')
-    cache['wb_done'] = not defer
-    cache['packs'].deferred = cache if defer else None
-    return cache['packs']
+    return _prep_launched(cache, defer)
+
+
+def prep_all_to_cl_nfk(owner, convs, x_nfk, shape, preop=0, defer_backward_packs=False):
+    if not _prep_ride_enabled():
+        return prep_all(owner, convs, defer_backward_packs), to_cl_nfk(x_nfk, shape, preop)
+    _PENDING_BACKWARD_PACKS.pop(convs[0].weight_v.device, None)
+    cache = _prep_cache(owner, convs)
+    if cache is None or cache['dev'] != x_nfk.device:
+        return (None if cache is None else prep_all(owner, convs, defer_backward_packs)), to_cl_nfk(x_nfk, shape, preop)
+    N, F, K, Cp, out = _to_cl_nfk_out(x_nfk, shape)
+    defer = _prep_defer(defer_backward_packs)
+    with torch.cuda.device(cache['dev']):
+        check(lib().psnd_conv1d_prep_multi_to_cl_nfk(ptr(cache['table']), cache['n'], cache['blocks'], cache['max_row'], 1 if defer else 3,
+                                                     ptr(x_nfk), N, K, F, shape.Lp, shape.HP, Cp, int(preop), ptr(out),
+                                                     stream_ptr(cache['dev'])), 'psnd_conv1d_prep_multi_to_cl_nfk')
+    return _prep_launched(cache, defer), out
 
 
 def fused_conv(xa, conv, shape, res=None, want_raw=False, want_act=True, act_slope=0.1, prep=None):
diff --git a/pytorch_sound_amd/csrc/psnd_conv.hip b/pytorch_sound_amd/csrc/psnd_conv.hip
--- a/pytorch_sound_amd/csrc/psnd_conv.hip
+++ b/pytorch_sound_amd/csrc/psnd_conv.hip
@@ -1,5 +1,6 @@
 #include "psnd_common.h"
 #include "psnd_conv_pair.h"
+#include "psnd_nfk_body.h"
 #include <stdlib.h>
 #include <string.h>
 #include <algorithm>
@@ -1000,16 +1001,15 @@
     int Cout, Cin, k, Cb, Ca, blk0;
 };
 constexpr int PREP_ROWS = 8;
-__global__ __launch_bounds__(256) void conv_prep_multi_kernel(const PrepDesc *descs, int n, int which) {
-    extern __shared__ __attribute__((aligned(16))) bf16_t s_prep[];
+__device__ __forceinline__ void conv_prep_multi_body(const PrepDesc *descs, int n, int which, const unsigned block, bf16_t *s_prep) {
     int lo = 0, hi = n - 1;
     while (lo < hi) {
         const int mid = (lo + hi + 1) >> 1;
-        if (descs[mid].blk0 <= (int)blockIdx.x) lo = mid;
+        if (descs[mid].blk0 <= (int)block) lo = mid;
         else hi = mid - 1;
     }
     const PrepDesc d = descs[lo];
-    const int co0 = (blockIdx.x - d.blk0) * PREP_ROWS, nn = d.Cin * d.k;
+    const int co0 = (block - d.blk0) * PREP_ROWS, nn = d.Cin * d.k;
     if (co0 >= d.Cout) return;
     const int tid = threadIdx.x, lane = tid & 63, w = tid >> 6;
     constexpr int NR = 32;
@@ -1094,6 +1094,17 @@
         for (int e = 0; e < 8; ++e) v[e] = (short)sp[(size_t)e * nn];
         *reinterpret_cast<bf16x8 *>(d.wb + pack_index(k, j, ci, co0, d.Ca, d.Cb)) = v;
     }
+}
+__global__ __launch_bounds__(256) void conv_prep_multi_kernel(const PrepDesc *descs, int n, int which) {
+    extern __shared__ __attribute__((aligned(16))) bf16_t s_prep[];
+    conv_prep_multi_body(descs, n, which, blockIdx.x, s_prep);
+}
+
+template <bool MASKBWD>
+__global__ __launch_bounds__(256) void conv_prep_ride_kernel(const PrepDesc *descs, int n, int which, unsigned prep_blocks, nfkk::NfkParams p) {
+    extern __shared__ __attribute__((aligned(16))) bf16_t s_prep[];
+    if (blockIdx.x < prep_blocks) conv_prep_multi_body(descs, n, which, blockIdx.x, s_prep);
+    else nfkk::to_cl_nfk_body<MASKBWD>(p, blockIdx.x - prep_blocks);
 }
 
 template <bool MANY>
@@ -1866,18 +1877,59 @@
     return PSND_OK;
 }
 
+static int prep_multi_lds(const char *what, const void *kernel, const void *descs_dev, int n, int total_blocks, int max_row, int which, size_t *lds) {
+    if (!descs_dev || n <= 0 || total_blocks <= 0 || max_row <= 0 || which < 1 || which > 3) PSND_FAIL(PSND_E_ARG, "%s: bad arguments", what);
+    *lds = (size_t)PREP_ROWS * (size_t)max_row * sizeof(bf16_t);
+    if (*lds > 160 * 1024) PSND_FAIL(PSND_E_SHAPE, "%s: Cin * k = %d too large for the 8-row tile (use psnd_conv1d_prep)", what, max_row);
+    if (*lds > 48 * 1024) {
+        hipError_t e = hipFuncSetAttribute(kernel, hipFuncAttributeMaxDynamicSharedMemorySize, (int)*lds);
+        if (e != hipSuccess) PSND_FAIL(PSND_E_HIP, "%s: set LDS size: %s", what, hipGetErrorString(e));
+    }
+    return PSND_OK;
+}
+
 extern "C" int psnd_conv1d_prep_multi(const void *descs_dev, int n, int total_blocks, int max_row, int which, void *stream) {
-    if (!descs_dev || n <= 0 || total_blocks <= 0 || max_row <= 0 || which < 1 || which > 3) PSND_FAIL(PSND_E_ARG, "conv1d_prep_multi: bad arguments");
-    const size_t lds = (size_t)PREP_ROWS * (size_t)max_row * sizeof(bf16_t);
-    if (lds > 160 * 1024) PSND_FAIL(PSND_E_SHAPE, "conv1d_prep_multi: Cin * k = %d too large for the 8-row tile (use psnd_conv1d_prep)", max_row);
-    if (lds > 48 * 1024) {
-        hipError_t e = hipFuncSetAttribute(reinterpret_cast<const void *>(conv_prep_multi_kernel), hipFuncAttributeMaxDynamicSharedMemorySize, (int)lds);
-        if (e != hipSuccess) PSND_FAIL(PSND_E_HIP, "conv1d_prep_multi: set LDS size: %s", hipGetErrorString(e));
-    }
+    size_t lds = 0;
+    if (int rc = prep_multi_lds("conv1d_prep_multi", reinterpret_cast<const void *>(conv_prep_multi_kernel), descs_dev, n, total_blocks, max_row, which, &lds)) return rc;
     hipLaunchKernelGGL(conv_prep_multi_kernel, dim3(total_blocks), dim3(256), lds, static_cast<hipStream_t>(stream),
                        static_cast<const PrepDesc *>(descs_dev), n, which);
     PSND_CHECK_LAUNCH("conv1d_prep_multi");
     return PSND_OK;
+}
+
+template <bool MASKBWD>
+static int launch_prep_ride(const char *what, const void *descs_dev, int n, int total_blocks, int which, size_t lds, const nfkk::NfkParams &p,
+                            bool empty, void *stream) {
+    const long long lay = empty ? 0 : (p.items + 255) / 256;
+    if ((long long)total_blocks + lay >= (1ll << 31)) PSND_FAIL(PSND_E_SHAPE, "%s: %lld + %d workgroups", what, lay, total_blocks);
+    hipLaunchKernelGGL(conv_prep_ride_kernel<MASKBWD>, dim3((unsigned)(total_blocks + lay)), dim3(256), lds, static_cast<hipStream_t>(stream),
+                       static_cast<const PrepDesc *>(descs_dev), n, which, (unsigned)total_blocks, p);
+    PSND_CHECK_LAUNCH(what);
+    return PSND_OK;
+}
+
+extern "C" int psnd_conv1d_prep_multi_to_cl_nfk(const void *descs_dev, int n, int total_blocks, int max_row, int which, const float *x_nfk,
+                                                int64_t N, int K, int64_t F, int Lp, int HP, int Cp, int preop, void *out, void *stream) {
+    const char *what = "conv1d_prep_multi_to_cl_nfk";
+    size_t lds = 0;
+    if (int rc = prep_multi_lds(what, reinterpret_cast<const void *>(conv_prep_ride_kernel<false>), descs_dev, n, total_blocks, max_row, which, &lds)) return rc;
+    nfkk::NfkParams p;
+    bool empty = false;
+    if (int rc = nfkk::to_cl_params(what, x_nfk, N, K, F, Lp, HP, Cp, preop, out, p, &empty)) return rc;
+    return launch_prep_ride<false>(what, descs_dev, n, total_blocks, which, lds, p, empty, stream);
+}
+
+extern "C" int psnd_conv1d_prep_multi_mask_head_l1_bwd_nfk(const void *descs_dev, int n, int total_blocks, int max_row, int which,
+                                                           const float *gest_nfk, const float *mag_nfk, const void *y, const float *est_nfk,
+                                                           const float *ref_nfk, const float *g, float coef, int64_t N, int K, int64_t F, int Lp,
+                                                           int HP, int Cp, void *gy, void *stream) {
+    const char *what = "conv1d_prep_multi_mask_head_l1_bwd_nfk";
+    size_t lds = 0;
+    if (int rc = prep_multi_lds(what, reinterpret_cast<const void *>(conv_prep_ride_kernel<true>), descs_dev, n, total_blocks, max_row, which, &lds)) return rc;
+    nfkk::NfkParams p;
+    bool empty = false;
+    if (int rc = nfkk::mask_bwd_params(what, gest_nfk, mag_nfk, y, est_nfk, ref_nfk, g, coef, N, K, F, Lp, HP, Cp, gy, p, &empty)) return rc;
+    return launch_prep_ride<true>(what, descs_dev, n, total_blocks, which, lds, p, empty, stream);
 }
 
 extern "C" int psnd_conv1d_wnorm_bwd(const float *gw_part, const float *gbias_part, int splits, const float *v, const float *g,
diff --git a/pytorch_sound_amd/csrc/psnd_core.hip b/pytorch_sound_amd/csrc/psnd_core.hip
--- a/pytorch_sound_amd/csrc/psnd_core.hip
+++ b/pytorch_sound_amd/csrc/psnd_core.hip
@@ -9,7 +9,7 @@
     va_end(ap);
 }
 
-extern "C" int psnd_version(void) { return 141; }
+extern "C" int psnd_version(void) { return 142; }
 
 extern "C" const char *psnd_last_error(void) { return g_err; }
 
diff --git a/pytorch_sound_amd/csrc/psnd_nfk.hip b/pytorch_sound_amd/csrc/psnd_nfk.hip
--- a/pytorch_sound_amd/csrc/psnd_nfk.hip
+++ b/pytorch_sound_amd/csrc/psnd_nfk.hip
@@ -1,104 +1,11 @@
-#include "psnd_common.h"
+#include "psnd_nfk_body.h"
 
 namespace {
-
-typedef unsigned short bf16_t;
-typedef __bf16 hwbf16x2 __attribute__((ext_vector_type(2)));
-
-__device__ __forceinline__ float bf_lo(unsigned v) { return __builtin_bit_cast(float, v << 16); }
-__device__ __forceinline__ float bf_hi(unsigned v) { return __builtin_bit_cast(float, v & 0xffff0000u); }
-__device__ __forceinline__ unsigned pack_bf16(float lo, float hi) {
-    const f32x2 v = {lo, hi};
-    return __builtin_bit_cast(unsigned, __builtin_convertvector(v, hwbf16x2));
-}
-
-struct Row8 {
-    float v[8];
-};
-__device__ __forceinline__ Row8 load8(__amdgpu_buffer_rsrc_t r, unsigned row_byte, int c0, int K, bool row_ok) {
-    Row8 o;
-    constexpr unsigned OOB = 0xffffffffu;
-    if (c0 + 8 <= K) {
-        const unsigned b = row_ok ? row_byte + 4u * (unsigned)c0 : OOB;
-        const f32x4 a = __builtin_bit_cast(f32x4, __builtin_amdgcn_raw_buffer_load_b128(r, (int)b, 0, 0));
-        const f32x4 c = __builtin_bit_cast(f32x4, __builtin_amdgcn_raw_buffer_load_b128(r, (int)(row_ok ? b + 16u : OOB), 0, 0));
-        o.v[0] = a.x, o.v[1] = a.y, o.v[2] = a.z, o.v[3] = a.w, o.v[4] = c.x, o.v[5] = c.y, o.v[6] = c.z, o.v[7] = c.w;
-    } else {
-#pragma unroll
-        for (int j = 0; j < 8; ++j)
-            o.v[j] = __builtin_bit_cast(float, __builtin_amdgcn_raw_buffer_load_b32(r, (int)((row_ok && c0 + j < K) ? row_byte + 4u * (unsigned)(c0 + j) : OOB), 0, 0));
-    }
-    return o;
-}
-__device__ __forceinline__ void store8(__amdgpu_buffer_rsrc_t r, unsigned row_byte, int c0, int K, const float (&v)[8]) {
-    if (c0 + 8 <= K) {
-        __builtin_amdgcn_raw_buffer_store_b128(__builtin_bit_cast(u32x4, f32x4{v[0], v[1], v[2], v[3]}), r, (int)(row_byte + 4u * (unsigned)c0), 0, 0);
-        __builtin_amdgcn_raw_buffer_store_b128(__builtin_bit_cast(u32x4, f32x4{v[4], v[5], v[6], v[7]}), r, (int)(row_byte + 4u * (unsigned)c0 + 16u), 0, 0);
-    } else {
-#pragma unroll
-        for (int j = 0; j < 8; ++j)
-            if (c0 + j < K) __builtin_amdgcn_raw_buffer_store_b32(__builtin_bit_cast(unsigned, v[j]), r, (int)(row_byte + 4u * (unsigned)(c0 + j)), 0, 0);
-    }
-}
-
-struct NfkParams {
-    const float *x;
-    const float *ref;
-    const float *est_in;
-    const float *gest;
-    const float *g;
-    const bf16_t *y;
-    bf16_t *out_cl;
-    float *est;
-    double *part;
-    long long items;
-    int N, F, K, Lp, HP, Cp, preop;
-    unsigned tensor_bytes;
-    float coef;
-};
+using namespace nfkk;
 
 template <bool MASKBWD>
 __global__ __launch_bounds__(256) void to_cl_nfk_kernel(NfkParams p) {
-    const long long it = (long long)blockIdx.x * 256 + threadIdx.x;
-    if (it >= p.items) return;
-    const int cpr = p.Cp >> 3;
-    const long long row = it / cpr;
-    const int c0 = (int)(it - row * cpr) * 8;
-    const int n = (int)(row / p.Lp), l = (int)(row - (long long)n * p.Lp), t = l - p.HP;
-    const bool ok = t >= 0 && t < p.F;
-    const unsigned rb = (unsigned)(((size_t)n * p.F + (size_t)(ok ? t : 0)) * p.K * 4);
-    const int tb = (int)p.tensor_bytes;
-    const __amdgpu_buffer_rsrc_t rx = make_uniform_rsrc(p.x, tb);
-    float w[8];
-    if constexpr (!MASKBWD) {
-        const Row8 a = load8(rx, rb, c0, p.K, ok);
-#pragma unroll
-        for (int j = 0; j < 8; ++j) {
-            float v = a.v[j];
-            if (p.preop == 1) {
-                const float u = 1.f + v;
-                v = u == 1.f ? v : __logf(u) * __fdividef(v, u - 1.f);
-            }
-            w[j] = v;
-        }
-    } else {
-        const __amdgpu_buffer_rsrc_t re = make_uniform_rsrc(p.est_in, tb), rr = make_uniform_rsrc(p.ref, tb);
-        const __amdgpu_buffer_rsrc_t rg = make_uniform_rsrc(p.gest ? p.gest : p.x, p.gest ? tb : 0);
-        const Row8 m = load8(rx, rb, c0, p.K, ok), e = load8(re, rb, c0, p.K, ok), r = load8(rr, rb, c0, p.K, ok), ge = load8(rg, rb, c0, p.K, ok);
-        const u32x4 yq = *reinterpret_cast<const u32x4 *>(p.y + (size_t)row * p.Cp + c0);
-        const float l1c = p.coef * p.g[0];
-#pragma unroll
-        for (int j = 0; j < 8; ++j) {
-            const unsigned q = yq[j >> 1];
-            const float yv = (j & 1) ? bf_hi(q) : bf_lo(q);
-            const float sg = 1.f / (1.f + __expf(-yv));
-            const float d = e.v[j] - r.v[j];
-            const float gg = ge.v[j] + l1c * (d > 0.f ? 1.f : (d < 0.f ? -1.f : 0.f));
-            w[j] = gg * m.v[j] * sg * (1.f - sg);
-        }
-    }
-    const u32x4 o = {pack_bf16(w[0], w[1]), pack_bf16(w[2], w[3]), pack_bf16(w[4], w[5]), pack_bf16(w[6], w[7])};
-    *reinterpret_cast<u32x4 *>(p.out_cl + (size_t)row * p.Cp + c0) = o;
+    to_cl_nfk_body<MASKBWD>(p, blockIdx.x);
 }
 
 __global__ __launch_bounds__(256) void mask_head_nfk_kernel(NfkParams p) {
@@ -136,24 +43,13 @@
     }
 }
 
-int check_shape(const char *what, int64_t N, int K, int64_t F, int Lp, int HP, int Cp) {
-    if (N < 0 || K <= 0 || F <= 0 || HP < 0 || Lp < F + 2 * HP || Cp < ((K + 7) & ~7) || Cp % 8 != 0 || (size_t)N * (size_t)K * (size_t)F * 4 >= ((size_t)1 << 32) - 64 ||
-        (size_t)Lp * Cp * 2 >= ((size_t)1 << 31) || N * (int64_t)Lp * (Cp / 8) >= ((int64_t)1 << 39))
-        PSND_FAIL(PSND_E_SHAPE, "%s: N=%lld K=%d F=%lld Lp=%d HP=%d Cp=%d", what, (long long)N, K, (long long)F, Lp, HP, Cp);
-    return PSND_OK;
-}
-
 }
 
 extern "C" int psnd_to_cl_nfk(const float *x_nfk, int64_t N, int K, int64_t F, int Lp, int HP, int Cp, int preop, void *out, void *stream) {
-    if (!x_nfk || !out) PSND_FAIL(PSND_E_ARG, "to_cl_nfk: null pointer");
-    if (preop < 0 || preop > 1) PSND_FAIL(PSND_E_ARG, "to_cl_nfk: preop=%d", preop);
-    if (int rc = check_shape("to_cl_nfk", N, K, F, Lp, HP, Cp)) return rc;
-    if (N == 0) return PSND_OK;
-    NfkParams p = {};
-    p.x = x_nfk, p.out_cl = static_cast<bf16_t *>(out), p.N = (int)N, p.F = (int)F, p.K = K, p.Lp = Lp, p.HP = HP, p.Cp = Cp, p.preop = preop;
-    p.items = N * (int64_t)Lp * (Cp / 8);
-    p.tensor_bytes = (unsigned)((size_t)N * F * K * 4);
+    NfkParams p;
+    bool empty = false;
+    if (int rc = to_cl_params("to_cl_nfk", x_nfk, N, K, F, Lp, HP, Cp, preop, out, p, &empty)) return rc;
+    if (empty) return PSND_OK;
     hipLaunchKernelGGL(to_cl_nfk_kernel<false>, dim3((unsigned)((p.items + 255) / 256)), dim3(256), 0, static_cast<hipStream_t>(stream), p);
     PSND_CHECK_LAUNCH("to_cl_nfk");
     return PSND_OK;
@@ -182,14 +78,10 @@
 
 extern "C" int psnd_mask_head_l1_bwd_nfk(const float *gest_nfk, const float *mag_nfk, const void *y, const float *est_nfk, const float *ref_nfk,
                                          const float *g, float coef, int64_t N, int K, int64_t F, int Lp, int HP, int Cp, void *gy, void *stream) {
-    if (!mag_nfk || !y || !est_nfk || !ref_nfk || !g || !gy) PSND_FAIL(PSND_E_ARG, "mask_head_l1_bwd_nfk: null pointer");
-    if (int rc = check_shape("mask_head_l1_bwd_nfk", N, K, F, Lp, HP, Cp)) return rc;
-    if (N == 0) return PSND_OK;
-    NfkParams p = {};
-    p.x = mag_nfk, p.ref = ref_nfk, p.est_in = est_nfk, p.gest = gest_nfk, p.g = g, p.coef = coef, p.y = static_cast<const bf16_t *>(y);
-    p.out_cl = static_cast<bf16_t *>(gy), p.N = (int)N, p.F = (int)F, p.K = K, p.Lp = Lp, p.HP = HP, p.Cp = Cp;
-    p.items = N * (int64_t)Lp * (Cp / 8);
-    p.tensor_bytes = (unsigned)((size_t)N * F * K * 4);
+    NfkParams p;
+    bool empty = false;
+    if (int rc = mask_bwd_params("mask_head_l1_bwd_nfk", gest_nfk, mag_nfk, y, est_nfk, ref_nfk, g, coef, N, K, F, Lp, HP, Cp, gy, p, &empty)) return rc;
+    if (empty) return PSND_OK;
     hipLaunchKernelGGL(to_cl_nfk_kernel<true>, dim3((unsigned)((p.items + 255) / 256)), dim3(256), 0, static_cast<hipStream_t>(stream), p);
     PSND_CHECK_LAUNCH("mask_head_l1_bwd_nfk");
     return PSND_OK;
diff --git a/pytorch_sound_amd/csrc/psnd_nfk_body.h b/pytorch_sound_amd/csrc/psnd_nfk_body.h
--- /dev/null
+++ b/pytorch_sound_amd/csrc/psnd_nfk_body.h
@@ -0,0 +1,139 @@
+#pragma once
+#include "psnd_common.h"
+
+namespace {
+namespace nfkk {
+typedef unsigned short bf16_t;
+typedef __bf16 hwbf16x2 __attribute__((ext_vector_type(2)));
+
+__device__ __forceinline__ float bf_lo(unsigned v) { return __builtin_bit_cast(float, v << 16); }
+__device__ __forceinline__ float bf_hi(unsigned v) { return __builtin_bit_cast(float, v & 0xffff0000u); }
+__device__ __forceinline__ unsigned pack_bf16(float lo, float hi) {
+    const f32x2 v = {lo, hi};
+    return __builtin_bit_cast(unsigned, __builtin_convertvector(v, hwbf16x2));
+}
+
+struct Row8 {
+    float v[8];
+};
+__device__ __forceinline__ Row8 load8(__amdgpu_buffer_rsrc_t r, unsigned row_byte, int c0, int K, bool row_ok) {
+    Row8 o;
+    constexpr unsigned OOB = 0xffffffffu;
+    if (c0 + 8 <= K) {
+        const unsigned b = row_ok ? row_byte + 4u * (unsigned)c0 : OOB;
+        const f32x4 a = __builtin_bit_cast(f32x4, __builtin_amdgcn_raw_buffer_load_b128(r, (int)b, 0, 0));
+        const f32x4 c = __builtin_bit_cast(f32x4, __builtin_amdgcn_raw_buffer_load_b128(r, (int)(row_ok ? b + 16u : OOB), 0, 0));
+        o.v[0] = a.x, o.v[1] = a.y, o.v[2] = a.z, o.v[3] = a.w, o.v[4] = c.x, o.v[5] = c.y, o.v[6] = c.z, o.v[7] = c.w;
+    } else {
+#pragma unroll
+        for (int j = 0; j < 8; ++j)
+            o.v[j] = __builtin_bit_cast(float, __builtin_amdgcn_raw_buffer_load_b32(r, (int)((row_ok && c0 + j < K) ? row_byte + 4u * (unsigned)(c0 + j) : OOB), 0, 0));
+    }
+    return o;
+}
+__device__ __forceinline__ void store8(__amdgpu_buffer_rsrc_t r, unsigned row_byte, int c0, int K, const float (&v)[8]) {
+    if (c0 + 8 <= K) {
+        __builtin_amdgcn_raw_buffer_store_b128(__builtin_bit_cast(u32x4, f32x4{v[0], v[1], v[2], v[3]}), r, (int)(row_byte + 4u * (unsigned)c0), 0, 0);
+        __builtin_amdgcn_raw_buffer_store_b128(__builtin_bit_cast(u32x4, f32x4{v[4], v[5], v[6], v[7]}), r, (int)(row_byte + 4u * (unsigned)c0 + 16u), 0, 0);
+    } else {
+#pragma unroll
+        for (int j = 0; j < 8; ++j)
+            if (c0 + j < K) __builtin_amdgcn_raw_buffer_store_b32(__builtin_bit_cast(unsigned, v[j]), r, (int)(row_byte + 4u * (unsigned)(c0 + j)), 0, 0);
+    }
+}
+
+struct NfkParams {
+    const float *x;
+    const float *ref;
+    const float *est_in;
+    const float *gest;
+    const float *g;
+    const bf16_t *y;
+    bf16_t *out_cl;
+    float *est;
+    double *part;
+    long long items;
+    int N, F, K, Lp, HP, Cp, preop;
+    unsigned tensor_bytes;
+    float coef;
+};
+
+template <bool MASKBWD>
+__device__ __forceinline__ void to_cl_nfk_body(const NfkParams &p, const unsigned block) {
+    const long long it = (long long)block * 256 + threadIdx.x;
+    if (it >= p.items) return;
+    const int cpr = p.Cp >> 3;
+    const long long row = it / cpr;
+    const int c0 = (int)(it - row * cpr) * 8;
+    const int n = (int)(row / p.Lp), l = (int)(row - (long long)n * p.Lp), t = l - p.HP;
+    const bool ok = t >= 0 && t < p.F;
+    const unsigned rb = (unsigned)(((size_t)n * p.F + (size_t)(ok ? t : 0)) * p.K * 4);
+    const int tb = (int)p.tensor_bytes;
+    const __amdgpu_buffer_rsrc_t rx = make_uniform_rsrc(p.x, tb);
+    float w[8];
+    if constexpr (!MASKBWD) {
+        const Row8 a = load8(rx, rb, c0, p.K, ok);
+#pragma unroll
+        for (int j = 0; j < 8; ++j) {
+            float v = a.v[j];
+            if (p.preop == 1) {
+                const float u = 1.f + v;
+                v = u == 1.f ? v : __logf(u) * __fdividef(v, u - 1.f);
+            }
+            w[j] = v;
+        }
+    } else {
+        const __amdgpu_buffer_rsrc_t re = make_uniform_rsrc(p.est_in, tb), rr = make_uniform_rsrc(p.ref, tb);
+        const __amdgpu_buffer_rsrc_t rg = make_uniform_rsrc(p.gest ? p.gest : p.x, p.gest ? tb : 0);
+        const Row8 m = load8(rx, rb, c0, p.K, ok), e = load8(re, rb, c0, p.K, ok), r = load8(rr, rb, c0, p.K, ok), ge = load8(rg, rb, c0, p.K, ok);
+        const u32x4 yq = *reinterpret_cast<const u32x4 *>(p.y + (size_t)row * p.Cp + c0);
+        const float l1c = p.coef * p.g[0];
+#pragma unroll
+        for (int j = 0; j < 8; ++j) {
+            const unsigned q = yq[j >> 1];
+            const float yv = (j & 1) ? bf_hi(q) : bf_lo(q);
+            const float sg = 1.f / (1.f + __expf(-yv));
+            const float d = e.v[j] - r.v[j];
+            const float gg = ge.v[j] + l1c * (d > 0.f ? 1.f : (d < 0.f ? -1.f : 0.f));
+            w[j] = gg * m.v[j] * sg * (1.f - sg);
+        }
+    }
+    const u32x4 o = {pack_bf16(w[0], w[1]), pack_bf16(w[2], w[3]), pack_bf16(w[4], w[5]), pack_bf16(w[6], w[7])};
+    *reinterpret_cast<u32x4 *>(p.out_cl + (size_t)row * p.Cp + c0) = o;
+}
+
+int check_shape(const char *what, int64_t N, int K, int64_t F, int Lp, int HP, int Cp) {
+    if (N < 0 || K <= 0 || F <= 0 || HP < 0 || Lp < F + 2 * HP || Cp < ((K + 7) & ~7) || Cp % 8 != 0 || (size_t)N * (size_t)K * (size_t)F * 4 >= ((size_t)1 << 32) - 64 ||
+        (size_t)Lp * Cp * 2 >= ((size_t)1 << 31) || N * (int64_t)Lp * (Cp / 8) >= ((int64_t)1 << 39))
+        PSND_FAIL(PSND_E_SHAPE, "%s: N=%lld K=%d F=%lld Lp=%d HP=%d Cp=%d", what, (long long)N, K, (long long)F, Lp, HP, Cp);
+    return PSND_OK;
+}
+
+inline int to_cl_params(const char *what, const float *x_nfk, int64_t N, int K, int64_t F, int Lp, int HP, int Cp, int preop, void *out,
+                        NfkParams &p, bool *empty) {
+    if (!x_nfk || !out) PSND_FAIL(PSND_E_ARG, "%s: null pointer", what);
+    if (preop < 0 || preop > 1) PSND_FAIL(PSND_E_ARG, "%s: preop=%d", what, preop);
+    if (int rc = check_shape(what, N, K, F, Lp, HP, Cp)) return rc;
+    *empty = N == 0;
+    p = NfkParams{};
+    p.x = x_nfk, p.out_cl = static_cast<bf16_t *>(out), p.N = (int)N, p.F = (int)F, p.K = K, p.Lp = Lp, p.HP = HP, p.Cp = Cp, p.preop = preop;
+    p.items = N * (int64_t)Lp * (Cp / 8);
+    p.tensor_bytes = (unsigned)((size_t)N * F * K * 4);
+    return PSND_OK;
+}
+inline int mask_bwd_params(const char *what, const float *gest_nfk, const float *mag_nfk, const void *y, const float *est_nfk,
+                           const float *ref_nfk, const float *g, float coef, int64_t N, int K, int64_t F, int Lp, int HP, int Cp, void *gy,
+                           NfkParams &p, bool *empty) {
+    if (!mag_nfk || !y || !est_nfk || !ref_nfk || !g || !gy) PSND_FAIL(PSND_E_ARG, "%s: null pointer", what);
+    if (int rc = check_shape(what, N, K, F, Lp, HP, Cp)) return rc;
+    *empty = N == 0;
+    p = NfkParams{};
+    p.x = mag_nfk, p.ref = ref_nfk, p.est_in = est_nfk, p.gest = gest_nfk, p.g = g, p.coef = coef, p.y = static_cast<const bf16_t *>(y);
+    p.out_cl = static_cast<bf16_t *>(gy), p.N = (int)N, p.F = (int)F, p.K = K, p.Lp = Lp, p.HP = HP, p.Cp = Cp;
+    p.items = N * (int64_t)Lp * (Cp / 8);
+    p.tensor_bytes = (unsigned)((size_t)N * F * K * 4);
+    return PSND_OK;
+}
+
+}
+}
diff --git a/pytorch_sound_amd/models/separator.py b/pytorch_sound_amd/models/separator.py
--- a/pytorch_sound_amd/models/separator.py
+++ b/pytorch_sound_amd/models/separator.py
@@ -48,8 +48,11 @@
         halo = max(c.padding for b in self.blocks for c in list(b.convs1) + list(b.convs2))
         shape = cl.CLShape(N, T, max(halo, self.conv_pre.padding, self.conv_post.padding))
         convs = [self.conv_pre] + [c for b in self.blocks for c in list(b.convs1) + list(b.convs2)] + [self.conv_post]
-        prep = cl.prep_all(self, convs, defer_backward_packs=True)
-        x0 = cl.to_cl_nfk(mag.float(), shape, 1) if layout == 'nfk' else cl.ToCL.apply(mag.float(), shape, 1)
+        if layout == 'nfk':
+            prep, x0 = cl.prep_all_to_cl_nfk(self, convs, mag.float(), shape, 1, defer_backward_packs=True)
+        else:
+            prep = cl.prep_all(self, convs, defer_backward_packs=True)
+            x0 = cl.ToCL.apply(mag.float(), shape, 1)
         return cl.conv_body_cl(self.conv_pre, list(self.blocks), self.conv_post, x0, shape, prep), shape
 
     def spectral_l1_loss(self, mag: torch.Tensor, mag_ref: torch.Tensor, mel_ref: torch.Tensor, mel_plan: torch.Tensor, n_mels: int,
```
